# natir/yacrd

Measured on AMD Instinct MI355X. Metric: reads_per_sec_classified, higher is better.
Workload: dtype u32

## Files before the change

include/yacrd_engine_debug.h:

```cpp
#ifndef YACRD_ENGINE_DEBUG_H
#define YACRD_ENGINE_DEBUG_H

#include "yacrd_engine.h"

#define YACRD_F_FORCE_GENERAL 1u
#define YACRD_F_FORCE_LDS_SORT 2u
#define YACRD_F_WAVE_ONLY 8u
#define YACRD_F_NO_HALVES 16u
#define YACRD_F_NO_PREDICTION 64u
#define YACRD_F_NO_PREFILTER 256u
#define YACRD_F_COUNT_PREFILTERED 512u
#define YACRD_F_NO_DEFER 4096u
#define YACRD_F_ALWAYS_DEFER 8192u
#define YACRD_F_SCREEN_ITEMS_1 262144u
#define YACRD_F_SCREEN_ITEMS_2 524288u
#define YACRD_F_NO_FUSED_SCREEN 1048576u
#define YACRD_F_STREAM_SCREEN 65536u
#define YACRD_F_SCREEN_WIDE 2097152u

#ifdef __cplusplus
extern "C" {
#endif
int yacrd_debug_sort_pairs(yacrd_engine *e, uint64_t *keys, uint32_t *vals, uint64_t n, uint64_t key_bound);
uint64_t yacrd_debug_last_counters(const yacrd_engine *e, void *dst, uint64_t bytes);
int yacrd_debug_last_input_csr(yacrd_engine *e, uint64_t *n_reads, uint64_t *n_intervals, uint64_t *offsets, uint32_t *intervals,
                               uint32_t *lengths);
void yacrd_debug_peer_copy_counts(uint64_t out[3]);
void yacrd_debug_live_bytes(uint64_t out[2]);
#ifdef __cplusplus
}
#endif

#endif
```

yacrd_amd/__init__.py:

```python
from .engine import (
    Engine, EngineError, NeedsHostParser, Result, lib_path, load_library, build, partition_reads, run_partitioned, ingest_overlaps,
    NOT_BAD, CHIMERIC, NOT_COVERED, TYPE_NAMES, F_FORCE_GENERAL, F_FORCE_LDS_SORT, F_WAVE_ONLY, F_NO_HALVES, F_TIMING_FULL, F_NO_PREDICTION, F_NO_PREFILTER, F_COUNT_PREFILTERED, F_NO_TIMING, F_BLOCKING_WAIT, F_NO_DEFER, F_ALWAYS_DEFER, F_TIMING_SAMPLED, F_STREAM_SCREEN, F_SCREEN_ITEMS_1, F_SCREEN_ITEMS_2, F_NO_FUSED_SCREEN, F_SCREEN_WIDE, F_ONE_LAUNCH, run_device_batches, DeviceBatch,
    EXPORTED_SYMBOLS, CLASS_NAMES, CLASS_KERNELS, PinnedArray, Stream, StreamGroup, stream_device_of, HANDLE_ELSEWHERE, RecSink, OvlRec, OVL_REC_DTYPE, GzipWriter, ByteSink,
)
```

yacrd_amd/csrc/engine.hip:

```cpp
#include "engine_internal.h"

#include <time.h>

#include <algorithm>
#include <cstdio>
#include <cstdlib>
#include <cstring>
#include <string>
#include <thread>
#include <vector>

#include "device_common.h"
#include "plan_compact.h"
#include "sweep_big.h"
#include "sweep_wave.h"
#include "sweep_big_trim.h"
#include "sweep_general.h"
#include "sweep_lds.h"
#include "finish_compact.h"
#include "screen_wg.h"
#include "screen_stream.h"
#include "screen_big.h"
#include "one_batch.h"

// ... 85 lines not shown
            dl.shard_cap = (slabs / yk::kDeferShards + 1u) * (u32)yk::kMarkReads;
            HIP_TRY(e->dlist.reserve((size_t)yk::kDeferShards * dl.shard_cap * sizeof(u32)));
            dl.list = e->dlist.as<u32>();
            dl.count = reinterpret_cast<u32 *>(ca.scan_state + R.nb);
            if (e->compact_calls++)
                HIP_TRY(hipMemsetAsync(dl.count, 0, (size_t)yk::kDeferShards * yk::kDeferShardStride * sizeof(u32), e->stream));
            hipLaunchKernelGGL(yk::mark_list_kernel, dim3(slabs), dim3(yk::kMarkThreads), 0, e->stream, ca.sweep.counts, n_reads, dl);
            hipLaunchKernelGGL(yk::deferred_list_kernel, dim3((u32)e->num_cu * (u32)(YK_LIST_OCC * 256 / yk::kListThreads)), dim3(yk::kListThreads), 0,
                               e->stream, ca.sweep, dl);
        }
        hipLaunchKernelGGL(yk::scan_compact_kernel<4>, dim3((n_reads + 4 * yk::kScanThreads - 1) / (4 * yk::kScanThreads)), dim3(yk::kScanThreads), 0, e->stream, ca);
        return YACRD_OK;
    }
    hipLaunchKernelGGL(yk::finish_compact_kernel, dim3((n_reads + yk::kScanBlock - 1) / yk::kScanBlock), dim3(yk::kScanBlock), 0, e->stream, ca);
    return YACRD_OK;
}

int gather_reads(yacrd_engine *e, const u64 *d_off, const u32 *d_len, const u32 *d_list, u32 count,
                 hipStream_t stream, std::vector<yk::GatherOut> &out)
{
    HIP_TRY(e->gen_sizes.reserve((size_t)count * sizeof(yk::GatherOut)));
    hipLaunchKernelGGL(yk::gather_general_sizes_kernel, dim3((count + 255) / 256), dim3(256), 0,
                       stream, d_off, d_len, d_list, count, e->gen_sizes.as<yk::GatherOut>());
    out.resize(count);
    HIP_TRY(hipMemcpyAsync(out.data(), e->gen_sizes.p, (size_t)count * sizeof(yk::GatherOut),
                           hipMemcpyDeviceToHost, stream));
    HIP_TRY(hipStreamSynchronize(stream));
    for (const auto &g : out)
        if (g.n >= 0x7FFFFFFFull) return fail(YACRD_EINVAL, "a read has >= 2^31 - 1 intervals");
    return YACRD_OK;
}

int run_general_global(yacrd_engine *e, const u64 *d_off, const uint2 *d_iv, const u32 *d_len,
                       const u32 *d_list, u32 count, u32 cov, hipStream_t stream)
{
    std::vector<yk::GatherOut> info;
    int rc = gather_reads(e, d_off, d_len, d_list, count, stream, info);
    if (rc) return rc;
    HIP_TRY(e->gen_scratch_off.reserve((size_t)count * sizeof(u64)));
    std::vector<u64> offs(count);
    u64 tot = 0;
    for (u32 i = 0; i < count; i++) {
        offs[i] = tot;
        tot += 3 * info[i].n + 2;
    }
    HIP_TRY(e->gen_scratch.reserve((size_t)tot * sizeof(u64)));
    HIP_TRY(hipMemcpyAsync(e->gen_scratch_off.p, offs.data(), (size_t)count * sizeof(u64),
                           hipMemcpyHostToDevice, stream));
    HIP_TRY(hipStreamSynchronize(stream));
    yk::GeneralArgs ga;
    ga.off = d_off;
    ga.iv = d_iv;
    ga.len = d_len;
    ga.list = d_list;
    ga.scratch_off = e->gen_scratch_off.as<u64>();
    ga.scratch = e->gen_scratch.as<u64>();
    ga.cov = cov;
    ga.stage = e->stage.as<uint2>();
    ga.counts = e->counts.as<u32>();
    hipLaunchKernelGGL(yk::sweep_general_kernel, dim3(count), dim3(yk::kGenThreads), 0, stream, ga);
    return YACRD_OK;
}

int run_big_sort(yacrd_engine *e, const uint2 *d_iv, const std::vector<yk::GatherOut> &info, u32 cov,
                 hipStream_t stream, std::vector<u32> &redo)
{
    const u32 count = (u32)info.size();
    std::vector<yk::BigSeg> segs(count);
    std::vector<u32> chunk_seg;
    u64 key_off = 0;
    u32 max_P = 0;
    for (u32 i = 0; i < count; i++) {
        u64 P = yk::kBigC;
        while (P < 2 * info[i].n) P <<= 1;
        if (P > 0x80000000ull) return fail(YACRD_EINVAL, "a read has more than 2^30 intervals");
        yk::BigSeg &sg = segs[i];
        sg.key_off = key_off;
        sg.iv_off = info[i].iv_off;
        sg.P = (u32)P;
        sg.n = (u32)info[i].n;
        sg.len = info[i].len;
        sg.read = info[i].read;
        sg.chunk_off = (u32)chunk_seg.size();
        sg.pad = 0;
        for (u64 c = 0; c < P / yk::kBigC; c++) chunk_seg.push_back(i);
        key_off += P;
        max_P = std::max(max_P, (u32)P);
    }
    const size_t n_chunks = chunk_seg.size();
    if (n_chunks >= 0x7FFFFFFFull / (yk::kBigC / 2)) return fail(YACRD_EINVAL, "big path: too many keys");
    const size_t tab_bytes = (size_t)count * sizeof(yk::BigSeg) + n_chunks * sizeof(u32) +
                             9 * n_chunks * sizeof(u32) + (size_t)count * sizeof(u32) + 64;
    HIP_TRY(e->big_tab.reserve(tab_bytes));
    HIP_TRY(e->big_keys.reserve((size_t)key_off * sizeof(u32)));
    char *base = e->big_tab.as<char>();
    yk::BigArgs a;
    a.seg = reinterpret_cast<yk::BigSeg *>(base);
    u32 *w = reinterpret_cast<u32 *>(base + (size_t)count * sizeof(yk::BigSeg));
    a.chunk_seg = w;
    w += n_chunks;
    u32 **per_chunk[] = {&a.c_delta, &a.c_depth_in, &a.c_mf, &a.c_ml, &a.c_mf_in,
                         &a.c_ml_in, &a.c_cnt, &a.c_pos, &a.c_cand};
    for (u32 **pp : per_chunk) {
        *pp = w;
        w += n_chunks;
    }
    a.seg_bad = w;
    a.keys = e->big_keys.as<u32>();
    a.iv = d_iv;
    a.n_chunks = (u32)n_chunks;
    a.n_segs = count;
    a.cov = cov;
    a.stage = e->stage.as<uint2>();
    a.counts = e->counts.as<u32>();
    HIP_TRY(hipMemcpyAsync((void *)a.seg, segs.data(), (size_t)count * sizeof(yk::BigSeg),
                           hipMemcpyHostToDevice, stream));
    HIP_TRY(hipMemcpyAsync((void *)a.chunk_seg, chunk_seg.data(), n_chunks * sizeof(u32),
                           hipMemcpyHostToDevice, stream));
    HIP_TRY(hipMemsetAsync(a.seg_bad, 0, (size_t)count * sizeof(u32), stream));
    hipLaunchKernelGGL(yk::big_fill_kernel, dim3((u32)n_chunks), dim3(yk::kBigT), 0, stream, a);
    yk::launch_big(a, max_P, stream);
    std::vector<u32> bad(count);
    HIP_TRY(hipMemcpyAsync(bad.data(), a.seg_bad, (size_t)count * sizeof(u32), hipMemcpyDeviceToHost,
                           stream));
    HIP_TRY(hipStreamSynchronize(stream));
    HIP_TRY(hipGetLastError());
    for (u32 i = 0; i < count; i++)
        if (bad[i]) redo.push_back(info[i].read);
    return YACRD_OK;
}

int run_big(yacrd_engine *e, const u64 *d_off, const uint2 *d_iv, const u32 *d_len,
            const u32 *d_list, u32 count, u32 cov, hipStream_t stream)
{
    std::vector<yk::GatherOut> info;
    int rc = gather_reads(e, d_off, d_len, d_list, count, stream, info);
    if (rc) return rc;
    std::vector<u32> redo;

    if (!(e->flags & YACRD_F_NO_PREFILTER)) {
        std::vector<yk::BtSeg> bs(count);
        std::vector<u32> chunk_seg;
        for (u32 i = 0; i < count; i++) {
            yk::BtSeg &b = bs[i];
            b.iv_off = info[i].iv_off;
            b.n = (u32)info[i].n;
            b.len = info[i].len;
            b.read = info[i].read;
            b.chunk_off = (u32)chunk_seg.size();
            b.flags = 0;
            b.m_new = 0;
            b.n_zl = 0;
            b.pad = 0;
            for (u64 c = 0; c < (info[i].n + yk::kBtChunk - 1) / yk::kBtChunk; c++) chunk_seg.push_back(i);
        }
        const size_t n_chunks = chunk_seg.size();
        const size_t tab_words = (size_t)count * 3 * yk::kBtSeq;
        HIP_TRY(e->bt_tab.reserve((size_t)count * sizeof(yk::BtSeg) + n_chunks * sizeof(u32) + 64));
        HIP_TRY(e->bt_hist.reserve(tab_words * sizeof(u32)));
        HIP_TRY(e->bt_cur.reserve((2 * tab_words + (size_t)count * (3 * yk::kBtSeq / 32)) * sizeof(u32)));
        HIP_TRY(e->bt_keys.reserve((size_t)count * yk::kBtCap * sizeof(u32)));
        yk::BtArgs ba;
        ba.seg = e->bt_tab.as<yk::BtSeg>();
        ba.chunk_seg = reinterpret_cast<const u32 *>(e->bt_tab.as<char>() + (size_t)count * sizeof(yk::BtSeg));
        ba.iv = d_iv;
        ba.n_chunks = (u32)n_chunks;
        ba.n_segs = count;
        ba.cov = cov;
        ba.hist = e->bt_hist.as<u32>();
        ba.cur = e->bt_cur.as<u32>();
        ba.lim = e->bt_cur.as<u32>() + tab_words;
        ba.drop = e->bt_cur.as<u32>() + 2 * tab_words;
        ba.tkeys = e->bt_keys.as<u32>();
        ba.stage = e->stage.as<uint2>();
        ba.counts = e->counts.as<u32>();
        HIP_TRY(hipMemcpyAsync((void *)ba.seg, bs.data(), (size_t)count * sizeof(yk::BtSeg),
                               hipMemcpyHostToDevice, stream));
        HIP_TRY(hipMemcpyAsync((void *)ba.chunk_seg, chunk_seg.data(), n_chunks * sizeof(u32),
                               hipMemcpyHostToDevice, stream));
        HIP_TRY(hipMemsetAsync(ba.hist, 0, tab_words * sizeof(u32), stream));
        yk::Counters *ctr = e->ctrl2[e->ctrl_cur].as<yk::Counters>();
        u32 *rej = e->lists.as<u32>() + (size_t)(yk::CLS_COUNT + 2) * e->last_list_stride;
        hipLaunchKernelGGL(yk::bt_hist_kernel, dim3((u32)n_chunks), dim3(yk::kBtT), 0, stream, ba);
        hipLaunchKernelGGL(yk::bt_plan_kernel, dim3(count), dim3(yk::kBtT), 0, stream, ba);
        hipLaunchKernelGGL(yk::bt_scatter_kernel, dim3((u32)n_chunks), dim3(yk::kBtT), 0, stream, ba);
        hipLaunchKernelGGL(yk::bt_sweep_kernel, dim3(count), dim3(1024), 0, stream, ba, rej, &ctr->rej_big);
        HIP_TRY(hipMemcpyAsync(bs.data(), (void *)ba.seg, (size_t)count * sizeof(yk::BtSeg),
                               hipMemcpyDeviceToHost, stream));
        HIP_TRY(hipStreamSynchronize(stream));
        HIP_TRY(hipGetLastError());
        std::vector<yk::GatherOut> rest;
        for (u32 i = 0; i < count; i++) {
            if (bs[i].flags & yk::BT_TRIMMED) continue;
            if (bs[i].flags & yk::BT_BAD) redo.push_back(info[i].read);
            else rest.push_back(info[i]);
        }
        info.swap(rest);
        count = (u32)info.size();
    }
    if (count) {
        rc = run_big_sort(e, d_iv, info, cov, stream, redo);
        if (rc) return rc;
    }
    if (!redo.empty()) {
        HIP_TRY(e->big_redo.reserve(redo.size() * sizeof(u32)));
        HIP_TRY(hipMemcpyAsync(e->big_redo.p, redo.data(), redo.size() * sizeof(u32),
                               hipMemcpyHostToDevice, stream));
        HIP_TRY(hipStreamSynchronize(stream));
        rc = run_general_global(e, d_off, d_iv, d_len, e->big_redo.as<u32>(), (u32)redo.size(), cov, stream);
        if (rc) return rc;
    }
    return YACRD_OK;
}

int wait_for_stream(yacrd_engine *e)
{
    if (e->flags & YACRD_F_BLOCKING_WAIT) {
        HIP_TRY(hipEventRecord(e->ev_sync[EVS_DONE], e->stream));
        for (;;) {
            const hipError_t q = hipEventQuery(e->ev_sync[EVS_DONE]);
            if (q == hipSuccess) break;
            if (q != hipErrorNotReady) HIP_TRY(q);
            struct timespec ts = {0, 20000};
            nanosleep(&ts, nullptr);
        }
    } else {
        HIP_TRY(hipStreamSynchronize(e->stream));
    }
    HIP_TRY(hipGetLastError());
    return YACRD_OK;
}

int conclude_run(yacrd_engine *e, const Run &R, float extra_ms);
int finish_pending(yacrd_engine *e);


int reserve_buffers(yacrd_engine *e, Run &R)
{
    const u32 n_reads = R.n_reads;
    const uint64_t n_reads64 = R.n_reads64;
    R.ob_slabs = (n_reads + yk::kObSlab - 1) / yk::kObSlab;
    R.nb = R.one_launch ? 2 * R.ob_slabs : (n_reads + yk::kScanBlock - 1) / yk::kScanBlock;
    constexpr int kLists = yk::CLS_COUNT + 9;
    HIP_TRY(e->lists.reserve((size_t)kLists * n_reads * sizeof(u32)));
    const size_t shard_ctr_bytes = (!R.one_launch && n_reads64 >= split_min_reads()) ? (size_t)yk::kDeferShards * yk::kDeferShardStride * sizeof(u32) : 0;
    R.ctrl_bytes = (sizeof(yk::Counters) + (size_t)R.nb * sizeof(u64) + shard_ctr_bytes + 255) & ~(size_t)255;
    e->compact_calls = 0;
    e->ctrl_cur ^= 1;
    const int cur = e->ctrl_cur, other = cur ^ 1;
    for (int i = 0; i < 2; i++) {
        const void *before = e->ctrl2[i].p;
        HIP_TRY(e->ctrl2[i].reserve(R.ctrl_bytes));
        if (e->ctrl2[i].p != before) e->ctrl_clean[i] = 0;
    }
    HIP_TRY(e->stage.reserve((size_t)(R.n_iv + 2 * n_reads64) * sizeof(uint2)));
    HIP_TRY(e->counts.reserve((size_t)n_reads * sizeof(u32)));
    HIP_TRY(e->closed.reserve((size_t)n_reads * sizeof(uint2)));
    HIP_TRY(e->read_type.reserve((size_t)n_reads));
    if (e->bad_regions.cap < (size_t)(4 * n_reads64 + 1024) * sizeof(uint2))
        HIP_TRY(e->bad_regions.reserve((size_t)(4 * n_reads64 + 1024) * sizeof(uint2)));

    R.mrec_cap1 = (u32)std::min<u64>(n_reads64, R.n_iv / 513 + 1), R.mrec_cap2 = (u32)std::min<u64>(n_reads64, R.n_iv / 4097 + 1);
    HIP_TRY(e->mrec.reserve(((size_t)R.mrec_cap1 + R.mrec_cap2) * sizeof(uint4)));
    R.lists = e->lists.as<u32>();
    e->last_list_stride = n_reads;
    R.rej_small = R.list_of(yk::CLS_COUNT), R.rej_med = R.list_of(yk::CLS_COUNT + 1);
    R.rej_big = R.list_of(yk::CLS_COUNT + 2), R.over_med = R.list_of(yk::CLS_COUNT + 3);
    R.fb_med[0] = R.list_of(yk::CLS_COUNT + 4), R.fb_med[1] = R.list_of(yk::CLS_COUNT + 5);
    R.fb_big = R.list_of(yk::CLS_COUNT + 6);
    R.fb_stream[0] = R.list_of(yk::CLS_COUNT + 7), R.fb_stream[1] = R.list_of(yk::CLS_COUNT + 8);
    R.ctr = e->ctrl2[cur].as<yk::Counters>();
    R.base = base_sweep_args(e, R);

    if (e->ctrl_clean[cur] < R.ctrl_bytes) HIP_TRY(hipMemsetAsync(R.ctr, 0, R.ctrl_bytes, e->stream));
    e->ctrl_clean[cur] = 0;
    R.other_bytes = std::min<size_t>(e->ctrl2[other].cap, (size_t)1 << 30) & ~(size_t)3;
    return YACRD_OK;
}

int launch_one_batch(yacrd_engine *e, Run &R)
{
    const int other = e->ctrl_cur ^ 1;
    yk::OneBatchArgs oa;
    oa.c = compact_args(e, R);
    oa.slab_ctr = oa.c.scan_state + R.ob_slabs;
    oa.n_slabs = R.ob_slabs;
    oa.zero = e->ctrl2[other].as<u32>();
    oa.zero_words = (u32)(R.other_bytes / 4);
    e->h_ctr()->ob_unsupported = 0;
    e->h_ctr()->scan_ticket = 0;
    hipLaunchKernelGGL(yk::one_batch_kernel, dim3(((R.ob_slabs + 7) / 8) * 8 * (u32)(yk::kObSlab / yk::kObReads)), dim3(64), 0, e->stream, oa);
    e->ctrl_clean[other] = R.other_bytes;
    if (R.full) HIP_TRY(hipEventRecord(e->ev[EV_COMPACT], e->stream));
    return YACRD_OK;
}

int launch_plan(yacrd_engine *e, Run &R)
{
    const int other = e->ctrl_cur ^ 1;
    const u32 n_reads = R.n_reads;
    const u32 plan_mode = (u32)((e->flags & YACRD_F_FORCE_GENERAL) ? 1
                                : (e->flags & (YACRD_F_WAVE_ONLY | YACRD_F_FORCE_LDS_SORT)) ? 2
                                : (e->flags & YACRD_F_NO_HALVES) ? 3 : 0);
    if (n_reads < yk::kPlanSmallReads)
        hipLaunchKernelGGL((yk::plan_kernel<1, yk::kPlanSmallBlock>), dim3((n_reads + yk::kPlanSmallBlock - 1) / yk::kPlanSmallBlock),
                           dim3(yk::kPlanSmallBlock), 0, e->stream, R.d_off, n_reads, R.lists, R.ctr, plan_mode, e->ctrl2[other].as<u32>(), (u32)(R.other_bytes / 4), e->counts.as<u32>(), e->mrec.as<uint4>(), R.mrec_cap1, R.mrec_cap2);
    else
        hipLaunchKernelGGL(yk::plan_kernel<4>, dim3((n_reads + 4 * yk::kPlanBlock - 1) / (4 * yk::kPlanBlock)),
                           dim3(yk::kPlanBlock), 0, e->stream, R.d_off, n_reads, R.lists, R.ctr, plan_mode,
                           e->ctrl2[other].as<u32>(), (u32)(R.other_bytes / 4), e->counts.as<u32>(), e->mrec.as<uint4>(), R.mrec_cap1, R.mrec_cap2);
    e->ctrl_clean[other] = R.other_bytes;
    if (R.full) HIP_TRY(hipEventRecord(e->ev[EV_PLAN], e->stream));
    return YACRD_OK;
}

int size_launches(yacrd_engine *e, Run &R)
{
    const uint64_t n_reads64 = R.n_reads64;
    const bool big_predictable = !(e->flags & YACRD_F_NO_PREFILTER) && e->pred.fb_big == 0;
    R.predicted = e->pred_valid && e->pred_reads == n_reads64 && e->pred_iv == R.n_iv &&
                  (e->pred.n[yk::CLS_GENERAL] == 0 || big_predictable) &&
                  !(e->flags & (YACRD_F_FORCE_GENERAL | YACRD_F_NO_PREDICTION));
    LaunchSet &ls = R.ls;
    if (R.predicted) {
        for (int cls = 0; cls < yk::CLS_GENERAL; cls++) {
            const u64 p = e->pred.n[cls];
            const u64 cap = (cls <= yk::CLS_W16 && R.tight_grids) ? ((p + p / 8 + 64 + 15) & ~(u64)15)
                                                                 : n_reads64;
            ls.n[cls] = p ? (u32)std::min<u64>(cap, (n_reads64 + 15) & ~(u64)15) : 0;
            ls.hint[cls] = p ? (u32)std::min<u64>(p + p / 8 + 64, n_reads64) : 0;
            ls.iv[cls] = e->pred.iv[cls];
        }
        R.big_n = e->pred.n[yk::CLS_GENERAL], R.big_iv = e->pred.iv[yk::CLS_GENERAL];
    } else {
        HIP_TRY(hipMemcpyAsync(e->h_ctr(), R.ctr, sizeof(yk::Counters), hipMemcpyDeviceToHost, e->stream));
        HIP_TRY(hipStreamSynchronize(e->stream));
        R.c0 = *e->h_ctr();
        for (int cls = 0; cls < yk::CLS_GENERAL; cls++) {
            ls.n[cls] = R.c0.n[cls];
            ls.hint[cls] = R.c0.n[cls];
            ls.iv[cls] = R.c0.iv[cls];
        }
        R.big_n = R.c0.n[yk::CLS_GENERAL], R.big_iv = R.c0.iv[yk::CLS_GENERAL];
    }
    for (int cls = 0; cls < yk::CLS_GENERAL; cls++)
        if (ls.n[cls] && (R.dom_cls < 0 || ls.iv[cls] > ls.iv[R.dom_cls])) R.dom_cls = cls;
    return YACRD_OK;
}

hipError_t before_class(yacrd_engine *e, Run &R, int cls)
{
    if (!R.timing_on || !(R.full || cls == R.dom_cls)) return hipSuccess;
    if (R.n_cls_ev > 0 && R.full) {
        R.cls_b[cls] = R.n_cls_ev - 1;
        return hipSuccess;
    }
    R.cls_b[cls] = R.n_cls_ev;
    return hipEventRecord(e->ev_cls[R.n_cls_ev++], e->stream);
}
hipError_t mark_class(yacrd_engine *e, Run &R, int cls)
{
    if (!R.timing_on || !(R.full || cls == R.dom_cls)) return hipSuccess;
    R.cls_e[cls] = R.n_cls_ev;
    return hipEventRecord(e->ev_cls[R.n_cls_ev++], e->stream);
}

int launch_register_classes(yacrd_engine *e, Run &R, const LaunchSet &set, bool again)
{
    yk::Counters *ctr = R.ctr;
    const bool fuse = !(e->flags & YACRD_F_FORCE_LDS_SORT);
    if (fuse) {
        yk::FusedArgs fa;
        fa.base = R.base;
        const u64 fused_iv = set.iv[yk::CLS_R16] + set.iv[yk::CLS_H16];
        const bool defer = R.prefilter && !(e->flags & YACRD_F_NO_DEFER) &&
                           ((e->flags & YACRD_F_ALWAYS_DEFER) ||
                            (fused_iv >= defer_min_intervals() && e->nodefer_left == 0));
        const bool wide = defer && !(e->flags & YACRD_F_SCREEN_ITEMS_2) && ((e->flags & YACRD_F_SCREEN_WIDE) || e->wide_left > 0);
        const int items = !defer ? 1
                          : (wide || (e->flags & YACRD_F_SCREEN_ITEMS_1)) ? 1
                          : ((e->flags & YACRD_F_SCREEN_ITEMS_2) || fused_iv >= 40000000ull) ? 2 : 1;
        e->last_items = (uint32_t)items;
        e->last_wide = wide;
        if (!again) e->last_build = !defer ? 0 : wide ? 3 : items;
        fa.base.over_list = nullptr;
        fa.base.over_count = nullptr;
        fa.n_entries = 0;
        u32 blocks = 0;
        bool has_dom = false;
        for (int cls = yk::CLS_R2; cls <= yk::CLS_H16; cls++) {
            if (!set.n[cls]) continue;
            const u32 per = yk::sweep_group_reads_per_block(cls, defer ? yk::kDeferWaves : yk::kFusedWaves) *
                            (cls >= yk::CLS_R16 ? (u32)items : 1u);
            blocks += (set.n[cls] + per - 1) / per;
            fa.cls[fa.n_entries] = (u32)cls;
            fa.block_end[fa.n_entries] = blocks;
            fa.list[fa.n_entries] = R.list_of(cls);
            fa.list_n[fa.n_entries] = &ctr->n[cls];
            fa.first[fa.n_entries] = set.first[cls];
            fa.n_entries++;
            has_dom |= cls == R.dom_cls;
        }
        if (fa.n_entries) {
            const bool mark = R.timing_on && (R.full || has_dom);
            void (*kernel)(yk::FusedArgs) = yk::sweep_small_fused_kernel;
            u32 threads = 64 * yk::kFusedWaves;
            if (defer && items == 2) kernel = yk::sweep_small_fused_defer2_kernel, threads = 64;
            else if (defer && wide) kernel = yk::sweep_small_fused_defer_wide_kernel, threads = 64 * yk::kDeferWaves;
            else if (defer) kernel = yk::sweep_small_fused_defer_kernel, threads = 64 * yk::kDeferWaves;
            hipExtLaunchKernelGGL(kernel, dim3(blocks), dim3(threads), 0, e->stream, mark ? e->ev_cls[22] : (hipEvent_t) nullptr,
                                  mark ? e->ev_cls[23] : (hipEvent_t) nullptr, 0, fa);
            if (mark) R.fused_marked = true;
            if (defer && (set.n[yk::CLS_R16] || set.n[yk::CLS_H16])) R.screened = true;
        }
    }
    for (int cls = fuse ? yk::CLS_W2 : yk::CLS_R2; cls <= yk::CLS_W16; cls++) {
        if (!set.n[cls]) continue;
        HIP_TRY(before_class(e, R, cls));
        yk::SweepArgs sa = list_sweep_args(R, R.list_of(cls), &ctr->n[cls]);
        sa.first = set.first[cls];
        if (!fuse) {
            const u32 grid = (u32)std::min<uint64_t>(set.n[cls], (uint64_t)e->num_cu * 32);
            hipLaunchKernelGGL((yk::sweep_lds_kernel<64, (int)yk::kSmallEvents>), dim3(grid), dim3(64), 0, e->stream, sa);
        } else {
            switch (cls) {
            case yk::CLS_W2: yk::launch_sweep_group<64, 2>(sa, set.n[cls], e->stream); break;
            case yk::CLS_W4: yk::launch_sweep_group<64, 4>(sa, set.n[cls], e->stream); break;
            case yk::CLS_W8: yk::launch_sweep_group<64, 8>(sa, set.n[cls], e->stream); break;
            default: yk::launch_sweep_group<64, 16>(sa, set.n[cls], e->stream); break;
            }
        }
        HIP_TRY(mark_class(e, R, cls));
    }
    if (R.full && R.timing_on) HIP_TRY(hipEventRecord(e->ev[EV_SMALL], e->stream));
    return YACRD_OK;
}

int launch_workgroup_class_fused_screen(yacrd_engine *e, Run &R, const LaunchSet &set, int k, bool again)
{
    yk::Counters *ctr = R.ctr;
    const int cls = k == 0 ? yk::CLS_MED1 : yk::CLS_MED2;
    if (again) {
        HIP_TRY(hipMemsetAsync(&ctr->fb_stream[k], 0, sizeof(u32), e->stream));
        HIP_TRY(hipMemsetAsync(&ctr->fb_med[k], 0, sizeof(u32), e->stream));
    }
    {
        yk::SweepArgs ss = list_sweep_args(R, R.list_of(cls), &ctr->n[cls]);
        ss.over_list = R.fb_stream[k];
        ss.over_count = &ctr->fb_stream[k];
        const u32 want = std::max<u32>(set.hint[cls], 1u);
        if (e->flags & YACRD_F_STREAM_SCREEN) {
            hipLaunchKernelGGL(yk::screen_stream_kernel, dim3((u32)std::min<uint64_t>(want, (uint64_t)e->num_cu * 96)), dim3(64), 0, e->stream, ss);
        } else {
            ss.rec = e->mrec.as<uint4>() + (k == 0 ? 0u : R.mrec_cap1);
            hipLaunchKernelGGL(yk::screen_wg_kernel, dim3((u32)std::min<uint64_t>(want, (uint64_t)e->num_cu * 64)), dim3(yk::kWsT), 0, e->stream, ss);
        }
    }
    yk::ScreenFusedArgs fa;
    fa.sweep = list_sweep_args(R, R.fb_stream[k], &ctr->fb_stream[k]);
    fa.sweep.rej_list = k == 0 ? R.rej_med : R.rej_big;
    fa.sweep.rej_count = k == 0 ? &ctr->rej_med : &ctr->rej_big;
    fa.n_fallback = &ctr->fb_med[k];
    const u64 known = std::max<u32>(set.hint[cls], 1u);
    u64 share = 1;
    if (fused_share_override()) share = std::min<u64>(fused_share_override(), (u64)yk::kFusedShareMax);
    fa.share = (u32)share;
    const u32 gs = (u32)std::min<u64>(std::min<u64>((known + share - 1) / share, (u64)e->num_cu * 4) * fused_grid_mult(), 0x7FFFFFFFull);
    hipLaunchKernelGGL(yk::screen_wg_fused_kernel, dim3(gs), dim3(yk::kWsT), 0, e->stream, fa);
    if (k == 1) {
        yk::SweepArgs so = list_sweep_args(R, R.over_med, &ctr->over_med);
        so.rej_list = R.rej_big;
        so.rej_count = &ctr->rej_big;
        const u32 grid = (u32)std::min<uint64_t>(set.n[cls], (uint64_t)e->num_cu);
        hipLaunchKernelGGL((yk::sweep_lds_kernel<1024, (int)yk::kMedium2Events>), dim3(grid), dim3(1024), 0, e->stream, so);
    }
    return YACRD_OK;
}

int launch_workgroup_class_chain(yacrd_engine *e, Run &R, const LaunchSet &set, int k, bool again)
{
    yk::Counters *ctr = R.ctr;
    const int cls = k == 0 ? yk::CLS_MED1 : yk::CLS_MED2;
    const u32 *list = R.list_of(cls), *list_n = &ctr->n[cls];
    if (R.prefilter) {
        if (again) HIP_TRY(hipMemsetAsync(&ctr->fb_med[k], 0, sizeof(u32), e->stream));
        yk::SweepArgs ss = list_sweep_args(R, list, list_n);
        ss.over_list = R.fb_med[k];
        ss.over_count = &ctr->fb_med[k];
        const u32 gs = (u32)std::min<uint64_t>(set.n[cls], (uint64_t)e->num_cu * 4);
        hipLaunchKernelGGL(yk::screen_wg_kernel, dim3(gs), dim3(yk::kWsT), 0, e->stream, ss);
        list = R.fb_med[k], list_n = &ctr->fb_med[k];
    }
    yk::SweepArgs sa = list_sweep_args(R, list, list_n);
    sa.rej_list = k == 0 ? R.rej_med : R.rej_big;
    sa.rej_count = k == 0 ? &ctr->rej_med : &ctr->rej_big;
    if (k == 0) {
        const u32 grid = (u32)std::min<uint64_t>(set.n[cls], (uint64_t)e->num_cu * 4);
        hipLaunchKernelGGL((yk::sweep_lds_kernel<256, (int)yk::kMedium1Events>), dim3(grid), dim3(256), 0, e->stream, sa);
        return YACRD_OK;
    }
    yk::SweepArgs so = sa;
    if (R.prefilter) {
        const u32 g256 = (u32)std::min<uint64_t>(set.n[cls], (uint64_t)e->num_cu * 5);
        hipLaunchKernelGGL((yk::sweep_lds_kernel<256, (int)yk::kMedium1Events>), dim3(g256), dim3(256), 0, e->stream, sa);
        so.list = R.over_med;
        so.list_n = &ctr->over_med;
    }
    const u32 grid = (u32)std::min<uint64_t>(set.n[cls], (uint64_t)e->num_cu);
    hipLaunchKernelGGL((yk::sweep_lds_kernel<1024, (int)yk::kMedium2Events>), dim3(grid), dim3(1024), 0, e->stream, so);
    return YACRD_OK;
}

int launch_workgroup_classes(yacrd_engine *e, Run &R, const LaunchSet &set, bool again)
{
    const bool fused_screen = R.prefilter && !(e->flags & YACRD_F_NO_FUSED_SCREEN) && !e->fused_off && e->screen_fused_wgs_per_cu > 0;
    for (int k = 0; k < 2; k++) {
        const int cls = k == 0 ? yk::CLS_MED1 : yk::CLS_MED2;
        if (!set.n[cls]) continue;
        HIP_TRY(before_class(e, R, cls));
        const int rc = fused_screen ? launch_workgroup_class_fused_screen(e, R, set, k, again)
                                    : launch_workgroup_class_chain(e, R, set, k, again);
        if (rc) return rc;
        HIP_TRY(mark_class(e, R, cls));
    }
    if (R.full && R.timing_on) HIP_TRY(hipEventRecord(e->ev[EV_MED], e->stream));
    return YACRD_OK;
}

void launch_rejected_medium(yacrd_engine *e, Run &R, const LaunchSet &set)
{
    if (!set.n[yk::CLS_MED1]) return;
    yk::SweepArgs sa = list_sweep_args(R, R.rej_med, &R.ctr->rej_med);
    sa.rej_list = R.rej_big;
    sa.rej_count = &R.ctr->rej_big;
    hipLaunchKernelGGL((yk::sweep_general_lds_kernel<1024, 4096>), dim3(e->num_cu), dim3(1024), 0, e->stream, sa);
}

int launch_sweeps(yacrd_engine *e, Run &R, const LaunchSet &set, bool again = false)
{
    int rc = launch_register_classes(e, R, set, again);
    if (!rc) rc = launch_workgroup_classes(e, R, set, again);
    if (!rc) launch_rejected_medium(e, R, set);
    return rc;
}

int launch_device_wide_screen_on(yacrd_engine *e, Run &R, u32 count, u64 iv_big, hipStream_t hs)
{
    yk::Counters *ctr = R.ctr;
    if (e->flags & YACRD_F_FORCE_GENERAL)
        return run_general_global(e, R.d_off, R.d_iv, R.d_len, R.list_of(yk::CLS_GENERAL), count, R.cov, e->stream);
    if (!R.prefilter)
        return run_big(e, R.d_off, R.d_iv, R.d_len, R.list_of(yk::CLS_GENERAL), count, R.cov, e->stream);
    const u64 max_chunks = iv_big / yk::kBsChunk + count;
    if (max_chunks >= 0x7FFFFFFFull) return fail(YACRD_EINVAL, "too many intervals in reads beyond 16384");
    HIP_TRY(e->bs_seg.reserve((size_t)count * sizeof(yk::BsSeg)));
    HIP_TRY(e->bs_chunk.reserve((size_t)max_chunks * sizeof(u32)));
    HIP_TRY(e->bs_hist.reserve((size_t)count * 2 * yk::kBsBins * sizeof(u32)));
    yk::BsArgs ba;
    ba.off = R.d_off, ba.iv = R.d_iv, ba.len = R.d_len;
    ba.list = R.list_of(yk::CLS_GENERAL);
    ba.list_n = &ctr->n[yk::CLS_GENERAL];
    ba.seg = e->bs_seg.as<yk::BsSeg>();
    ba.chunk_seg = e->bs_chunk.as<u32>();
    ba.n_chunks = &ctr->bs_chunks;
    ba.hist = e->bs_hist.as<u32>();
    ba.max_chunks = (u32)max_chunks, ba.max_segs = count;
    ba.cov = R.cov, ba.count_healthy = R.prefilter == 2 ? 1u : 0u;
    ba.stage = R.base.stage, ba.counts = R.base.counts;
    ba.fb_list = R.fb_big, ba.fb_count = &ctr->fb_big;
    ba.ctr = ctr;
    if (R.big_screened) HIP_TRY(hipMemsetAsync(&ctr->fb_big, 0, sizeof(u32), hs));
    HIP_TRY(hipMemsetAsync(ba.hist, 0, (size_t)count * 2 * yk::kBsBins * sizeof(u32), hs));
    hipLaunchKernelGGL(yk::bs_setup_kernel, dim3(1), dim3(1024), 0, hs, ba);
    hipLaunchKernelGGL(yk::bs_minmax_kernel, dim3((u32)max_chunks), dim3(yk::kBsT), 0, hs, ba);
    hipLaunchKernelGGL(yk::bs_hist_kernel, dim3((u32)max_chunks), dim3(yk::kBsT), 0, hs, ba);
    hipLaunchKernelGGL(yk::bs_verdict_kernel, dim3(count), dim3(yk::kBsVT), 0, hs, ba);
    R.big_screened = true;
    return YACRD_OK;
}
int launch_device_wide_screen(yacrd_engine *e, Run &R)
{
    const bool can_fork = R.big_n != 0 && R.prefilter && !(e->flags & YACRD_F_FORCE_GENERAL);
    if (can_fork && e->side == nullptr) {
        if (e->streams.add(1)) e->side = e->streams[1];
        else (void)hipGetLastError();
    }
    R.big_beside = can_fork && e->side != nullptr;
    if (!R.big_beside) return YACRD_OK;
    HIP_TRY(hipEventRecord(e->ev_sync[EVS_FORK], e->stream));
    HIP_TRY(hipStreamWaitEvent(e->side, e->ev_sync[EVS_FORK], 0));
    const int rc = launch_device_wide_screen_on(e, R, R.big_n, R.big_iv, e->side);
    if (rc) return rc;
    HIP_TRY(hipEventRecord(e->ev_sync[EVS_JOIN], e->side));
    return YACRD_OK;
}
int join_device_wide_screen(yacrd_engine *e, Run &R)
{
    if (R.big_beside) HIP_TRY(hipStreamWaitEvent(e->stream, e->ev_sync[EVS_JOIN], 0));
    else if (R.big_n) return launch_device_wide_screen_on(e, R, R.big_n, R.big_iv, e->stream);
    return YACRD_OK;
}

void launch_rejected_small(yacrd_engine *e, Run &R)
{
    yk::SweepArgs sa = list_sweep_args(R, R.rej_small, &R.ctr->rej_small);
    sa.rej_list = R.rej_med;
    sa.rej_count = &R.ctr->rej_med;
    hipLaunchKernelGGL((yk::sweep_general_lds_kernel<256, 512>), dim3(e->num_cu * 2), dim3(256), 0, e->stream, sa);
}

int recover(yacrd_engine *e, Run &R, float &extra_ms)
{
    yk::Counters *ctr = R.ctr;
    int rc = YACRD_OK;
    bool redo = false;
    if (R.predicted) {
        R.c0 = *e->h_ctr();
        const yk::Counters &c0 = R.c0;
        LaunchSet missing{};
        bool any_missing = false;
        for (int cls = 0; cls < yk::CLS_GENERAL; cls++)
            if (c0.n[cls] > R.ls.n[cls]) {
                missing.first[cls] = (cls <= yk::CLS_W16 && R.tight_grids) ? R.ls.n[cls] : 0;
                missing.n[cls] = c0.n[cls] - missing.first[cls];
                missing.hint[cls] = missing.n[cls];
                any_missing = true;
            }
        const bool big_mismatch = c0.n[yk::CLS_GENERAL] != R.big_n || c0.iv[yk::CLS_GENERAL] != R.big_iv;
        if (any_missing || big_mismatch) {
            e->miss_pending = true;
            HIP_TRY(hipEventRecord(e->ev[EV_X0], e->stream));
            if (any_missing && (rc = launch_sweeps(e, R, missing, true))) return rc;
            if (big_mismatch && c0.n[yk::CLS_GENERAL] &&
                (rc = launch_device_wide_screen_on(e, R, c0.n[yk::CLS_GENERAL], c0.iv[yk::CLS_GENERAL], e->stream))) return rc;
            HIP_TRY(hipMemcpyAsync(e->h_ctr(), ctr, sizeof(yk::Counters), hipMemcpyDeviceToHost, e->stream));
            HIP_TRY(hipStreamSynchronize(e->stream));
            redo = true;
        }
    }
    u32 rej_small_done = 0;
    if (e->h_ctr()->rej_small) {
        if (!redo) HIP_TRY(hipEventRecord(e->ev[EV_X0], e->stream));
        launch_rejected_small(e, R);
        rej_small_done = e->h_ctr()->rej_small;
        redo = true;
    }
    if (R.big_screened && e->h_ctr()->fb_big) {
        if (!redo) HIP_TRY(hipEventRecord(e->ev[EV_X0], e->stream));
        rc = run_big(e, R.d_off, R.d_iv, R.d_len, R.fb_big, e->h_ctr()->fb_big, R.cov, e->stream);
        if (rc) return rc;
        HIP_TRY(hipMemcpyAsync(e->h_ctr(), ctr, sizeof(yk::Counters), hipMemcpyDeviceToHost, e->stream));
        HIP_TRY(hipStreamSynchronize(e->stream));
        redo = true;
    }
    const u32 n_rej_big = e->h_ctr()->rej_big;
    if (n_rej_big) {
        if (!redo) HIP_TRY(hipEventRecord(e->ev[EV_X0], e->stream));
        rc = run_general_global(e, R.d_off, R.d_iv, R.d_len, R.rej_big, n_rej_big, R.cov, e->stream);
        if (rc) return rc;
        redo = true;
    }
    for (int attempt = 0; attempt < 4; attempt++) {
        if (!redo && e->h_ctr()->rej_small > rej_small_done) {
            HIP_TRY(hipEventRecord(e->ev[EV_X0], e->stream));
            launch_rejected_small(e, R);
            rej_small_done = e->h_ctr()->rej_small;
            redo = true;
        }
        if (!redo) {
            if (!e->h_ctr()->region_overflow) break;
            HIP_TRY(e->bad_regions.reserve((size_t)(e->h_ctr()->total_regions + 16) * sizeof(uint2)));
            HIP_TRY(hipEventRecord(e->ev[EV_X0], e->stream));
        }
        redo = false;
        HIP_TRY(hipMemsetAsync(&ctr->region_overflow, 0, 3 * sizeof(u32), e->stream));
        HIP_TRY(hipMemsetAsync(ctr + 1, 0, (size_t)R.nb * sizeof(u64), e->stream));
        rc = launch_compact(e, R);
        if (rc) return rc;
        HIP_TRY(hipEventRecord(e->ev[EV_X1], e->stream));
        HIP_TRY(hipStreamSynchronize(e->stream));
        HIP_TRY(hipGetLastError());
        extra_ms += ev_ms(e->ev[EV_X0], e->ev[EV_X1]);
    }
    if (e->h_ctr()->region_overflow) return fail(YACRD_EINTERNAL, "bad_regions overflow persisted");
    if (e->h_ctr()->rej_small > rej_small_done) return fail(YACRD_EINTERNAL, "rejected reads persisted");
    return YACRD_OK;
}

}

namespace yke {
static int rerun_without_fused(yacrd_engine *e, const Run R)
{
    e->fused_off = true;
    e->pred_valid = false;
    const int rc = run_on_device(e, R.d_off, R.d_iv, R.d_len, R.n_reads64, R.n_iv, R.cov, R.not_cov, false);
    e->fused_off = false;
    return rc;
}

static int hand_over(yacrd_engine *e, const Run &R, bool defer)
{
    e->pending = Pending{true, R.one_launch, R};
    return defer ? YACRD_OK : finish_pending(e);
}

int run_on_device(yacrd_engine *e, const u64 *d_off, const uint2 *d_iv, const u32 *d_len,
                  uint64_t n_reads64, uint64_t n_iv, uint32_t cov, double not_cov, bool defer)
{
    if (n_reads64 >= 0xFFFFFFFFull) return fail(YACRD_EINVAL, "n_reads must be < 2^32 - 1");
    if (e->pending.active) return fail(YACRD_EINVAL, "a submitted batch is pending: yacrd_engine_wait first");
    e->has_result = false;
    e->resident.valid = e->input.valid = false;
    e->timing = yacrd_timing{};

    HIP_TRY(e->bad_offsets.reserve((n_reads64 + 1) * sizeof(u64)));
    if (n_reads64 == 0) {
        HIP_TRY(hipMemsetAsync(e->bad_offsets.p, 0, sizeof(u64), e->stream));
        HIP_TRY(hipStreamSynchronize(e->stream));
        e->last_reads = 0;
        e->last_regions = 0;
        e->has_result = true;
        return YACRD_OK;
    }

    Run R;
    R.d_off = d_off, R.d_iv = d_iv, R.d_len = d_len;
    R.n_reads64 = n_reads64, R.n_reads = (u32)n_reads64, R.n_iv = n_iv, R.cov = cov, R.not_cov = not_cov;
    R.full = (e->flags & YACRD_F_TIMING_FULL) != 0;
    R.tight_grids = !(e->flags & YACRD_F_FORCE_LDS_SORT);
    R.prefilter = (e->flags & YACRD_F_NO_PREFILTER) ? 0u : (e->flags & YACRD_F_COUNT_PREFILTERED) ? 2u : 1u;
    for (int i = 0; i < 12; i++) R.cls_b[i] = R.cls_e[i] = -1;
    const uint64_t ob_waiters = (n_reads64 + yk::kObSlab - 1) / yk::kObSlab * 7 / 8;
    R.one_launch = (e->flags & YACRD_F_ONE_LAUNCH) && !e->one_launch_off && n_reads64 < (uint64_t)yk::kObMaxReads &&
                   e->num_xcc == 8 && 2 * ob_waiters <= (uint64_t)e->num_cu * 4 * YK_OB_OCC &&
                   !(e->flags & (YACRD_F_FORCE_GENERAL | YACRD_F_WAVE_ONLY | YACRD_F_FORCE_LDS_SORT | YACRD_F_NO_HALVES |
                                 YACRD_F_NO_PREFILTER | YACRD_F_NO_DEFER));

    int rc = reserve_buffers(e, R);
    if (rc) return rc;
    if (R.full) HIP_TRY(hipEventRecord(e->ev[EV_START], e->stream));
    if (R.one_launch) {
        rc = launch_one_batch(e, R);
        return rc ? rc : hand_over(e, R, defer);
    }
    rc = launch_plan(e, R);
    if (!rc) rc = size_launches(e, R);
    if (rc) return rc;
    R.timing_on = !(e->flags & YACRD_F_NO_TIMING);
    if ((e->flags & YACRD_F_TIMING_SAMPLED) && !R.full && (e->run_seq++ % 8u) != 0) R.timing_on = false;
    struct MissGuard {
        yacrd_engine *e;
        bool before;
        ~MissGuard() { e->miss_pending = before; }
    } miss_guard{e, e->miss_pending};
    struct SideGuard {
        yacrd_engine *e;
        const Run &R;
        bool joined = false;
        ~SideGuard()
        {
            if (R.big_beside && !joined) (void)hipStreamSynchronize(e->side);
        }
    } side_guard{e, R};
    e->prev_build = e->last_build;
    e->last_build = -1;
    if (R.full) HIP_TRY(hipEventRecord(e->ev[EV_S0], e->stream));
    rc = launch_device_wide_screen(e, R);
    if (!rc) rc = launch_sweeps(e, R, R.ls);
    if (!rc) rc = join_device_wide_screen(e, R);
    if (rc) return rc;
    side_guard.joined = true;
    if (R.full) HIP_TRY(hipEventRecord(e->ev[EV_GEN], e->stream));
    rc = launch_compact(e, R);
    if (rc) return rc;
    if (R.full) HIP_TRY(hipEventRecord(e->ev[EV_COMPACT], e->stream));
    if (defer && R.predicted) return hand_over(e, R, defer);
    rc = wait_for_stream(e);
    if (rc) return rc;
    R.timing_on = false;
    if (e->h_ctr()->fused_gave_up && !e->fused_off) return rerun_without_fused(e, R);
    float extra_ms = 0.f;
    rc = recover(e, R, extra_ms);
    if (rc) return rc;
    return conclude_run(e, R, extra_ms);
}
}

namespace {

void fold_timing(yacrd_engine *e)
{
    const yacrd_timing &t = e->timing;
    yacrd_timing &ts = e->timing_sum;
    const yacrd_timing keep = ts;
    ts = t;
    ts.h2d_ms = keep.h2d_ms;
    ts.d2h_ms = keep.d2h_ms;
    ts.plan_ms = keep.plan_ms + t.plan_ms;
    ts.sweep_small_ms = keep.sweep_small_ms + t.sweep_small_ms;
    ts.sweep_medium_ms = keep.sweep_medium_ms + t.sweep_medium_ms;
    ts.sweep_general_ms = keep.sweep_general_ms + t.sweep_general_ms;
    ts.compact_ms = keep.compact_ms + t.compact_ms;
    ts.total_ms = keep.total_ms + t.total_ms;
    for (int i = 0; i < 12; i++) ts.class_ms[i] = keep.class_ms[i] + t.class_ms[i];
    ts.fused_ms = keep.fused_ms + t.fused_ms;
    ts.screened = keep.screened + t.screened;
    ts.one_launch = keep.one_launch + t.one_launch;
    ts.fused_reruns = keep.fused_reruns + t.fused_reruns;
    ts.screen_wide = keep.screen_wide + t.screen_wide;
    ts.predicted = keep.predicted + t.predicted;
    ts.prediction_misses = keep.prediction_misses + t.prediction_misses;
    ts.build_switches = keep.build_switches + t.build_switches;
    ts.sorting_build = keep.sorting_build + t.sorting_build;
    ts.timed_runs = keep.timed_runs + t.timed_runs;
    e->timing_runs++;
}

int conclude_run(yacrd_engine *e, const Run &R, float extra_ms)
{
    const bool full = R.full, predicted = R.predicted, screened = R.screened;
    const yk::Counters c1 = *e->h_ctr();
    const yk::Counters c0 = predicted ? c1 : R.c0;
    e->last_reads = R.n_reads;
    e->last_regions = c1.total_regions;
    e->has_result = true;
    e->pred = c1;
    e->pred_reads = R.n_reads64;
    e->pred_iv = R.n_iv;
    e->pred_valid = true;

    yacrd_timing &t = e->timing;
    t.plan_ms = t.sweep_small_ms = t.sweep_medium_ms = t.sweep_general_ms = t.compact_ms = 0.f;
    t.total_ms = 0.f;
    if (full) {
        t.plan_ms = ev_ms(e->ev[EV_START], e->ev[EV_PLAN]);
        t.sweep_small_ms = ev_ms(e->ev[EV_S0], e->ev[EV_SMALL]);
        t.sweep_medium_ms = ev_ms(e->ev[EV_SMALL], e->ev[EV_MED]);
        t.sweep_general_ms = ev_ms(e->ev[EV_MED], e->ev[EV_GEN]);
        t.compact_ms = ev_ms(e->ev[EV_GEN], e->ev[EV_COMPACT]);
        t.total_ms = (predicted ? ev_ms(e->ev[EV_START], e->ev[EV_COMPACT])
                                : t.plan_ms + ev_ms(e->ev[EV_S0], e->ev[EV_COMPACT])) + extra_ms;
    }
    t.n_small = 0;
    t.iv_small = 0;
    for (int cls = yk::CLS_R2; cls <= yk::CLS_W16; cls++) {
        t.n_small += c0.n[cls];
        t.iv_small += c0.iv[cls];
    }
    t.n_medium = (uint64_t)c0.n[yk::CLS_MED1] + c0.n[yk::CLS_MED2];
    t.n_general = (uint64_t)c0.n[yk::CLS_GENERAL] + c1.rej_small + c1.rej_med + c1.rej_big;
    t.iv_medium = c0.iv[yk::CLS_MED1] + c0.iv[yk::CLS_MED2];
    t.iv_general = c0.iv[yk::CLS_GENERAL];
    static_assert(yk::CLS_GENERAL == 11, "yacrd_timing.class_* follows the CLS_ order");
    for (int cls = 0; cls <= yk::CLS_GENERAL; cls++) {
        t.class_reads[cls] = c0.n[cls];
        t.class_intervals[cls] = c0.iv[cls];
        t.class_ms[cls] = 0.f;
        if (cls < yk::CLS_GENERAL && R.cls_b[cls] >= 0 && R.cls_e[cls] >= 0)
            t.class_ms[cls] = ev_ms(e->ev_cls[R.cls_b[cls]], e->ev_cls[R.cls_e[cls]]);
    }
    t.class_ms[yk::CLS_GENERAL] = (full && c0.n[yk::CLS_GENERAL]) ? t.sweep_general_ms : 0.f;
    t.fused_ms = 0.f;
    t.timed_runs = R.fused_marked ? 1u : 0u;
    for (int cls = 0; cls < yk::CLS_GENERAL; cls++)
        if (R.cls_b[cls] >= 0 && R.cls_e[cls] >= 0) t.timed_runs = 1u;
    t.deferred_reads = c1.deferred;
    t.deferred_intervals = c1.deferred_iv;
    if (screened) {
        const uint64_t looked_at = (uint64_t)c0.n[yk::CLS_R16] + c0.n[yk::CLS_H16];
        const bool can_widen = !e->last_wide && !(e->flags & YACRD_F_SCREEN_ITEMS_2);
        e->nodefer_left = (!(e->flags & YACRD_F_ALWAYS_DEFER) && !can_widen && 4 * (uint64_t)c1.deferred > looked_at) ? kProbeEvery - 1 : 0;
        if (!e->last_wide) e->wide_left = 10 * (uint64_t)c1.deferred > looked_at ? kProbeEvery - 1 : 0;
        else if (e->wide_left) e->wide_left--;
    } else if (e->nodefer_left) {
        e->nodefer_left--;
    }
    t.screened = screened ? 1u : 0u;
    t.screen_items = screened ? e->last_items : 0u;
    t.screen_wide = (screened && e->last_wide) ? 1u : 0u;
    t.fused_reruns = e->fused_off ? 1u : 0u;
    t.predicted = predicted ? 1u : 0u;
    t.prediction_misses = e->miss_pending ? 1u : 0u;
    t.build_switches = (e->last_build >= 0 && e->prev_build >= 0 && e->last_build != e->prev_build) ? 1u : 0u;
    t.sorting_build = e->last_build == 0 ? 1u : 0u;
    t.fused_reads = t.fused_intervals = 0;
    t.prefiltered_reads = c1.prefiltered;
    if (R.fused_marked) t.fused_ms = ev_ms(e->ev_cls[22], e->ev_cls[23]);
    if (!(e->flags & YACRD_F_FORCE_LDS_SORT)) {
        for (int cls = yk::CLS_R2; cls <= yk::CLS_H16; cls++) {
            t.fused_reads += c0.n[cls];
            t.fused_intervals += c0.iv[cls];
        }
    }

    fold_timing(e);
    return YACRD_OK;
}

int finish_pending(yacrd_engine *e)
{
    Pending &p = e->pending;
    if (!p.active) return YACRD_OK;
    p.active = false;
    const Run R = p.run;
    int rc = wait_for_stream(e);
    if (rc) return rc;
    if (p.one_launch) {
        const yk::Counters c1 = *e->h_ctr();
        if (c1.ob_unsupported || c1.rej_small || c1.region_overflow || c1.scan_ticket != R.ob_slabs) {
            if (c1.region_overflow) HIP_TRY(e->bad_regions.reserve((size_t)(c1.total_regions + 16) * sizeof(uint2)));
            e->one_launch_off = true;
            rc = run_on_device(e, R.d_off, R.d_iv, R.d_len, R.n_reads64, R.n_iv, R.cov, R.not_cov);
            e->one_launch_off = false;
            return rc;
        }
        e->last_reads = R.n_reads64;
        e->last_regions = c1.total_regions;
        e->has_result = true;
        yacrd_timing &t = e->timing;
        t = yacrd_timing{};
        if (R.full) t.total_ms = ev_ms(e->ev[EV_START], e->ev[EV_COMPACT]);
        t.n_small = R.n_reads64, t.iv_small = R.n_iv;
        t.deferred_reads = c1.deferred, t.deferred_intervals = c1.deferred_iv, t.prefiltered_reads = c1.prefiltered;
        t.screened = 1u, t.screen_items = (uint32_t)yk::kObItems, t.one_launch = 1u;
        fold_timing(e);
        return YACRD_OK;
    }
    const yk::Counters c = *e->h_ctr();
    if (c.fused_gave_up && !e->fused_off) return yke::rerun_without_fused(e, R);
    bool ok = !c.rej_small && c.n[yk::CLS_GENERAL] == R.big_n && c.iv[yk::CLS_GENERAL] == R.big_iv && !c.fb_big && !c.rej_big && !c.region_overflow;
    for (int cls = 0; cls < yk::CLS_GENERAL; cls++) ok = ok && c.n[cls] <= R.ls.n[cls];
    if (!ok) {
        e->pred_valid = false;
        e->miss_pending = true;
        const int rcm = run_on_device(e, R.d_off, R.d_iv, R.d_len, R.n_reads64, R.n_iv, R.cov, R.not_cov);
        e->miss_pending = false;
        return rcm;
    }
    return conclude_run(e, R, 0.f);
}

}

namespace yke {
int h2d(yacrd_engine *e, void *dst, const void *src, size_t bytes)
{
    if (!bytes) return YACRD_OK;
    hipPointerAttribute_t at;
    const bool pinned = hipPointerGetAttributes(&at, src) == hipSuccess && at.type == hipMemoryTypeHost;
    if (!pinned) (void)hipGetLastError();
    if (pinned || bytes < ((size_t)1 << 20)) {
        HIP_TRY(hipMemcpyAsync(dst, src, bytes, hipMemcpyHostToDevice, e->stream));
        return YACRD_OK;
    }
    constexpr size_t kPiece = yacrd_engine::kBounceBytes;
    for (size_t b = e->bounce_ev.v.size(); b < (size_t)yacrd_engine::kBounce; b++) {
        HIP_TRY(e->bounce[b].reserve(kPiece));
        if (!e->bounce_ev.add(1, hipEventDisableTiming)) {
            e->bounce[b].release();
            HIP_TRY(why_not_added());
        }
    }
    const size_t n_pieces = (bytes + kPiece - 1) / kPiece;
    const int T = (int)std::min<size_t>(yacrd_engine::kBounce / 2, n_pieces);
    std::vector<hipError_t> errs((size_t)T, hipSuccess);
    auto work = [&](int t) {
        if (hipSetDevice(e->device) != hipSuccess) {
            errs[t] = hipErrorInvalidDevice;
            return;
        }
        int turn = 0;
        for (size_t piece = (size_t)t; piece < n_pieces; piece += (size_t)T, turn ^= 1) {
            const int b = 2 * t + turn;
            if (e->bounce_busy[b]) {
                const hipError_t w = hipEventSynchronize(e->bounce_ev[b]);
                if (w != hipSuccess) errs[t] = w;
            }
            const size_t at2 = piece * kPiece, n = std::min(kPiece, bytes - at2);
            std::memcpy(e->bounce[b].p, (const char *)src + at2, n);
            hipError_t c = hipMemcpyAsync((char *)dst + at2, e->bounce[b].p, n, hipMemcpyHostToDevice, e->stream);
            if (c == hipSuccess) c = hipEventRecord(e->bounce_ev[b], e->stream);
            if (c != hipSuccess) errs[t] = c;
            e->bounce_busy[b] = true;
        }
    };
    {
        std::vector<std::thread> th;
        for (int t = 1; t < T; t++) th.emplace_back(work, t);
        work(0);
        for (auto &x : th) x.join();
    }
    for (hipError_t er : errs) HIP_TRY(er);
    return YACRD_OK;
}

int classify_on_device(yacrd_engine *e, const u64 *d_bad_offsets, const uint2 *d_bad_regions, const u32 *d_len, u32 n_reads, double not_cov,
                       uint8_t *d_read_type)
{
    if (n_reads)
        hipLaunchKernelGGL(yk::classify_csr_kernel, dim3((n_reads + 255u) / 256u), dim3(256), 0, e->stream, d_bad_offsets, d_bad_regions, d_len,
                           n_reads, not_cov, d_read_type);
    HIP_TRY(hipGetLastError());
    return YACRD_OK;
}

int fetch_result(yacrd_engine *e, yacrd_result *out)
{
    if (!out) return fail(YACRD_EINVAL, "out is null");
    std::memset(out, 0, sizeof(*out));
    if (e->pending.active) return fail(YACRD_EINVAL, "a submitted batch is pending: yacrd_engine_wait first");
    if (!e->has_result) return fail(YACRD_EINVAL, "no result to fetch");
    const uint64_t R = e->last_reads, G = e->last_regions;
    out->bad_offsets = (uint64_t *)std::malloc((size_t)(R + 1) * sizeof(uint64_t));
    out->bad_regions = (uint32_t *)std::malloc((size_t)(2 * G + 2) * sizeof(uint32_t));
    out->read_type = (uint8_t *)std::malloc((size_t)R + 1);
    if (!out->bad_offsets || !out->bad_regions || !out->read_type) {
        yacrd_result_free(out);
        return fail(YACRD_ENOMEM, "host allocation failed");
    }
    const size_t b_off = (size_t)(R + 1) * sizeof(uint64_t), b_reg = (size_t)G * sizeof(uint2), b_typ = (size_t)R;
    const size_t o_reg = (b_off + 63) & ~(size_t)63, o_typ = (o_reg + b_reg + 63) & ~(size_t)63;
    const size_t need = o_typ + b_typ + 64;
    bool staged = need <= ((size_t)1 << 30);
    if (staged && need > e->h_out.cap && e->h_out.reserve(need + need / 4) != hipSuccess) {
        (void)hipGetLastError();
        staged = false;
    }
    char *h = e->h_out.as<char>();
    void *t_off = staged ? (void *)h : (void *)out->bad_offsets;
    void *t_reg = staged ? (void *)(h + o_reg) : (void *)out->bad_regions;
    void *t_typ = staged ? (void *)(h + o_typ) : (void *)out->read_type;
    HIP_TRY(hipEventRecord(e->ev[EV_D2H0], e->stream));
    HIP_TRY(hipMemcpyAsync(t_off, e->bad_offsets.p, b_off, hipMemcpyDeviceToHost, e->stream));
    if (G) HIP_TRY(hipMemcpyAsync(t_reg, e->bad_regions.p, b_reg, hipMemcpyDeviceToHost, e->stream));
    if (R) HIP_TRY(hipMemcpyAsync(t_typ, e->read_type.p, b_typ, hipMemcpyDeviceToHost, e->stream));
    HIP_TRY(hipEventRecord(e->ev[EV_D2H1], e->stream));
    HIP_TRY(hipStreamSynchronize(e->stream));
    if (staged) {
        std::memcpy(out->bad_offsets, t_off, b_off);
        if (G) std::memcpy(out->bad_regions, t_reg, b_reg);
        if (R) std::memcpy(out->read_type, t_typ, b_typ);
    }
    e->timing.d2h_ms = ev_ms(e->ev[EV_D2H0], e->ev[EV_D2H1]);
    out->n_reads = R;
    out->n_regions = G;
    return YACRD_OK;
}
}

extern "C" {

int yacrd_abi_version(void) { return YACRD_ABI_VERSION; }

uint64_t yacrd_debug_last_counters(const yacrd_engine *e, void *dst, uint64_t bytes)
{
    if (e && dst && e->h_ctr()) std::memcpy(dst, e->h_ctr(), (size_t)std::min<uint64_t>(bytes, sizeof(yk::Counters)));
    return sizeof(yk::Counters);
}

int yacrd_debug_last_input_csr(yacrd_engine *e, uint64_t *n_reads, uint64_t *n_intervals, uint64_t *offsets, uint32_t *intervals,
                               uint32_t *lengths)
{
    if (!e || !n_reads || !n_intervals) return fail(YACRD_EINVAL, "null argument");
    if (e->pending.active || e->host_pending) return fail(YACRD_EINVAL, "the engine has a submitted batch pending");
    if (!e->input.valid) return fail(YACRD_EINVAL, "the engine's last call left no input CSR of its own");
    const uint64_t R = e->input.n_reads, I = e->input.n_iv;
    if (offsets && ((I && !intervals) || (R && !lengths))) return fail(YACRD_EINVAL, "null argument");
    if ((R && ((R + 1) * sizeof(u64) > e->in_off.cap || R * sizeof(u32) > e->in_len.cap)) || (I && I * sizeof(uint2) > e->in_iv.cap))
        return fail(YACRD_EINTERNAL, "the input CSR's record does not fit the engine's input buffers");
    *n_reads = R, *n_intervals = I;
    if (!offsets) return YACRD_OK;
    DeviceGuard guard(e->device);
    offsets[0] = 0;
    if (R) HIP_TRY(hipMemcpyAsync(offsets, e->in_off.p, (size_t)(R + 1) * sizeof(u64), hipMemcpyDeviceToHost, e->stream));
    if (I) HIP_TRY(hipMemcpyAsync(intervals, e->in_iv.p, (size_t)I * sizeof(uint2), hipMemcpyDeviceToHost, e->stream));
    if (R) HIP_TRY(hipMemcpyAsync(lengths, e->in_len.p, (size_t)R * sizeof(u32), hipMemcpyDeviceToHost, e->stream));
    HIP_TRY(hipStreamSynchronize(e->stream));
    return YACRD_OK;
}

void yacrd_debug_live_bytes(uint64_t out[2])
{
    out[0] = yke::live_bytes()[0].load();
    out[1] = yke::live_bytes()[1].load();
}

const char *yacrd_last_error(void) { return yke::err_slot().c_str(); }

int yacrd_engine_create(const yacrd_engine_cfg *cfg, yacrd_engine **out)
{
    if (!out) return fail(YACRD_EINVAL, "out is null");
    *out = nullptr;
    int count = 0;
    if (hipGetDeviceCount(&count) != hipSuccess || count == 0)
        return fail(YACRD_ENODEV, "no HIP device visible (libyacrd_hip needs an MI355X / gfx950)");
    int dev = cfg ? cfg->device_id : -1;
    if (dev < 0) HIP_TRY(hipGetDevice(&dev));
    if (dev >= count) return fail(YACRD_EINVAL, "device_id out of range");
    hipDeviceProp_t prop;
    HIP_TRY(hipGetDeviceProperties(&prop, dev));
    if (std::strncmp(prop.gcnArchName, "gfx950", 6) != 0)
        return fail(YACRD_ENODEV, std::string("device is ") + prop.gcnArchName +
                                      ", this library is built for gfx950 only");
    DeviceGuard guard(dev);
    yacrd_engine *e = new (std::nothrow) yacrd_engine();
    if (!e) return fail(YACRD_ENOMEM, "host allocation failed");
    e->device = dev;
    e->flags = cfg ? cfg->flags : 0;
    e->num_cu = prop.multiProcessorCount > 0 ? prop.multiProcessorCount : 256;
    {
        int xcc = 0;
        if (hipDeviceGetAttribute(&xcc, hipDeviceAttributeNumberOfXccs, dev) != hipSuccess) xcc = 0;
        (void)hipGetLastError();
        e->num_xcc = xcc;
    }
    {
        int per_cu = 0;
        if (hipOccupancyMaxActiveBlocksPerMultiprocessor(&per_cu, yk::screen_wg_fused_kernel, yk::kWsT, 0) == hipSuccess && per_cu > 0)
            e->screen_fused_wgs_per_cu = std::min(per_cu, 4);
        (void)hipGetLastError();
    }
    const bool made = e->streams.add(1) && e->ev.add(EV_COUNT) && e->ev_cls.add(24) &&
                      e->ev_sync.add(1, hipEventBlockingSync | hipEventDisableTiming) && e->ev_sync.add(2, hipEventDisableTiming);
    if (!made || e->h_ctr_mem.reserve(sizeof(yk::Counters)) != hipSuccess) {
        yacrd_engine_destroy(e);
        return fail(YACRD_ENODEV, std::string("engine setup: ") + hipGetErrorString(why_not_added()));
    }
    e->stream = e->streams[0];
    *out = e;
    return YACRD_OK;
}

int yacrd_engine_trim(yacrd_engine *e)
{
    if (!e) return fail(YACRD_EINVAL, "engine is null");
    if (e->pending.active || e->host_pending) return fail(YACRD_EINVAL, "the engine has a submitted batch pending");
    DeviceGuard guard(e->device);
    e->mirror.valid = false;
    e->resident.valid = e->input.valid = false;
    for (int k = 0; k < yacrd_engine::kSlots; k++)
        if (!(k == yacrd_engine::kGzip && e->gzip_busy)) e->drop_scratch(k);
    return YACRD_OK;
}

void yacrd_engine_destroy(yacrd_engine *e)
{
    if (!e) return;
    DeviceGuard guard(e->device);
    if (e->stream) (void)hipStreamSynchronize(e->stream);
    if (e->side) (void)hipStreamSynchronize(e->side);
    for (int k = 0; k < yacrd_engine::kSlots; k++) e->drop_scratch(k);
    delete e;
}

static void fill_device_result(const yacrd_engine *e, yacrd_device_result *out)
{
    if (!out) return;
    out->n_reads = e->last_reads;
    out->n_regions = e->last_regions;
    out->d_bad_offsets = e->bad_offsets.p;
    out->d_bad_regions = e->bad_regions.p;
    out->d_read_type = e->read_type.p;
}

int yacrd_engine_run_device(yacrd_engine *e, const void *d_offsets, const void *d_intervals,
                            const void *d_lengths, uint64_t n_reads, uint64_t n_intervals,
                            uint32_t coverage, double not_coverage, yacrd_device_result *out)
{
    if (!e) return fail(YACRD_EINVAL, "engine is null");
    e->resident.valid = e->input.valid = false;
    if (n_reads && (!d_offsets || !d_lengths)) return fail(YACRD_EINVAL, "null device input");
    if (n_intervals && !d_intervals) return fail(YACRD_EINVAL, "null device intervals");
    if (e->host_pending) return fail(YACRD_EINVAL, "a submitted batch is pending: collect it first");
    DeviceGuard guard(e->device);
    int rc = run_on_device(e, (const u64 *)d_offsets, (const uint2 *)d_intervals,
                           (const u32 *)d_lengths, n_reads, n_intervals, coverage, not_coverage);
    if (rc) return rc;
    fill_device_result(e, out);
    return YACRD_OK;
}

int yacrd_engine_submit_device(yacrd_engine *e, const void *d_offsets, const void *d_intervals,
                               const void *d_lengths, uint64_t n_reads, uint64_t n_intervals,
                               uint32_t coverage, double not_coverage)
{
    if (!e) return fail(YACRD_EINVAL, "engine is null");
    e->resident.valid = e->input.valid = false;
    if (n_reads && (!d_offsets || !d_lengths)) return fail(YACRD_EINVAL, "null device input");
    if (n_intervals && !d_intervals) return fail(YACRD_EINVAL, "null device intervals");
    if (e->host_pending) return fail(YACRD_EINVAL, "a submitted batch is pending: collect it first");
    DeviceGuard guard(e->device);
    return run_on_device(e, (const u64 *)d_offsets, (const uint2 *)d_intervals,
                         (const u32 *)d_lengths, n_reads, n_intervals, coverage, not_coverage, true);
}

int yacrd_engine_wait(yacrd_engine *e, yacrd_device_result *out)
{
    if (!e) return fail(YACRD_EINVAL, "engine is null");
    DeviceGuard guard(e->device);
    int rc = finish_pending(e);
    if (rc) return rc;
    if (!e->has_result) return fail(YACRD_EINVAL, "nothing was submitted");
    fill_device_result(e, out);
    return YACRD_OK;
}

int yacrd_engines_run_device_batches(yacrd_engine *const *engines, uint32_t n_engines,
                                     const yacrd_device_batch *batches, uint32_t n_batches,
                                     yacrd_batch_done_fn done, void *user, yacrd_device_result *last)
{
    if (!engines || n_engines == 0 || (!batches && n_batches)) return fail(YACRD_EINVAL, "bad argument");
    for (uint32_t j = 0; j < n_engines; j++)
        if (!engines[j]) return fail(YACRD_EINVAL, "engine is null");
    for (uint32_t j = 0; j < n_engines; j++) engines[j]->resident.valid = engines[j]->input.valid = false;
    std::vector<int64_t> inflight(n_engines, -1);
    yacrd_device_result res{};
    auto finish = [&](uint32_t j) -> int {
        int rc = yacrd_engine_wait(engines[j], &res);
        if (rc) return rc;
        const uint32_t b = (uint32_t)inflight[j];
        inflight[j] = -1;
        if (done && done(user, b, engines[j], &res)) return fail(YACRD_EINVAL, "the batch callback asked to stop");
        return YACRD_OK;
    };
    int rc = YACRD_OK;
    for (uint32_t i = 0; i < n_batches && rc == YACRD_OK; i++) {
        const uint32_t j = i % n_engines;
        if (inflight[j] >= 0) rc = finish(j);
        if (rc) break;
        const yacrd_device_batch &b = batches[i];
        rc = yacrd_engine_submit_device(engines[j], b.d_offsets, b.d_intervals, b.d_lengths, b.n_reads,
                                        b.n_intervals, b.coverage, b.not_coverage);
        if (rc == YACRD_OK) inflight[j] = i;
    }
    for (uint32_t k = 0; k < n_engines; k++) {
        uint32_t j = 0;
        int64_t lo = -1;
        for (uint32_t q = 0; q < n_engines; q++)
            if (inflight[q] >= 0 && (lo < 0 || inflight[q] < lo)) lo = inflight[q], j = q;
        if (lo < 0) break;
        const int rc2 = finish(j);
        if (rc == YACRD_OK) rc = rc2;
        inflight[j] = -1;
    }
    if (rc == YACRD_OK && last) *last = res;
    return rc;
}

static int stage_host_inputs(yacrd_engine *e, const uint64_t *offsets, const uint32_t *intervals,
                             const uint32_t *lengths, uint64_t n_reads, uint64_t *n_iv_out)
{
    if (n_reads && (!offsets || !lengths)) return fail(YACRD_EINVAL, "null input");
    const uint64_t n_iv = n_reads ? offsets[n_reads] : 0;
    if (n_reads && offsets[0] != 0) return fail(YACRD_EINVAL, "offsets[0] must be 0");
    for (uint64_t r = 0; r < n_reads; r++)
        if (offsets[r + 1] < offsets[r]) return fail(YACRD_EINVAL, "offsets must be non-decreasing");
    if (n_iv && !intervals) return fail(YACRD_EINVAL, "null intervals");
    HIP_TRY(e->in_off.reserve((size_t)(n_reads + 1) * sizeof(uint64_t)));
    HIP_TRY(e->in_iv.reserve((size_t)(n_iv + 1) * sizeof(uint2)));
    HIP_TRY(e->in_len.reserve((size_t)(n_reads + 1) * sizeof(uint32_t)));
    HIP_TRY(hipEventRecord(e->ev[EV_H2D0], e->stream));
    int rc = YACRD_OK;
    if (n_reads) {
        rc = h2d(e, e->in_off.p, offsets, (size_t)(n_reads + 1) * sizeof(uint64_t));
        if (!rc) rc = h2d(e, e->in_len.p, lengths, (size_t)n_reads * sizeof(uint32_t));
    }
    if (!rc && n_iv) rc = h2d(e, e->in_iv.p, intervals, (size_t)n_iv * sizeof(uint2));
    if (rc) return rc;
    HIP_TRY(hipEventRecord(e->ev[EV_H2D1], e->stream));
    *n_iv_out = n_iv;
    return YACRD_OK;
}

static int bring_home(yacrd_engine *e, yacrd_result *out)
{
    e->timing.h2d_ms = ev_ms(e->ev[EV_H2D0], e->ev[EV_H2D1]);
    e->timing_sum.h2d_ms += e->timing.h2d_ms;
    const int rc = fetch_result(e, out);
    if (rc) return rc;
    e->timing_sum.d2h_ms += e->timing.d2h_ms;
    e->input.valid = true;
    return YACRD_OK;
}

int yacrd_engine_run(yacrd_engine *e, const uint64_t *offsets, const uint32_t *intervals,
                     const uint32_t *lengths, uint64_t n_reads, uint32_t coverage,
                     double not_coverage, yacrd_result *out)
{
    if (!e) return fail(YACRD_EINVAL, "engine is null");
    e->resident.valid = e->input.valid = false;
    if (!out) return fail(YACRD_EINVAL, "out is null");
    std::memset(out, 0, sizeof(*out));
    if (e->pending.active) return fail(YACRD_EINVAL, "a submitted batch is pending: yacrd_engine_wait first");
    if (e->host_pending) return fail(YACRD_EINVAL, "a submitted batch is pending: collect it first");
    DeviceGuard guard(e->device);
    uint64_t n_iv = 0;
    int rc = stage_host_inputs(e, offsets, intervals, lengths, n_reads, &n_iv);
    if (rc) return rc;
    rc = run_on_device(e, e->in_off.as<u64>(), e->in_iv.as<uint2>(), e->in_len.as<u32>(), n_reads,
                       n_iv, coverage, not_coverage);
    if (rc) return rc;
    e->input.n_reads = n_reads, e->input.n_iv = n_iv;
    return bring_home(e, out);
}

int yacrd_engine_submit(yacrd_engine *e, const uint64_t *offsets, const uint32_t *intervals,
                        const uint32_t *lengths, uint64_t n_reads, uint32_t coverage,
                        double not_coverage)
{
    if (!e) return fail(YACRD_EINVAL, "engine is null");
    e->resident.valid = e->input.valid = false;
    if (e->pending.active || e->host_pending)
        return fail(YACRD_EINVAL, "a submitted batch is pending: collect it first");
    DeviceGuard guard(e->device);
    uint64_t n_iv = 0;
    int rc = stage_host_inputs(e, offsets, intervals, lengths, n_reads, &n_iv);
    if (rc) return rc;
    rc = run_on_device(e, e->in_off.as<u64>(), e->in_iv.as<uint2>(), e->in_len.as<u32>(), n_reads,
                       n_iv, coverage, not_coverage, true);
    if (rc) return rc;
    e->input.n_reads = n_reads, e->input.n_iv = n_iv;
    e->host_pending = true;
    return YACRD_OK;
}

int yacrd_engine_collect(yacrd_engine *e, yacrd_result *out)
{
    if (!e) return fail(YACRD_EINVAL, "engine is null");
    if (!out) return fail(YACRD_EINVAL, "out is null");
    std::memset(out, 0, sizeof(*out));
    if (!e->host_pending) return fail(YACRD_EINVAL, "nothing was submitted");
    e->host_pending = false;
    DeviceGuard guard(e->device);
    int rc = finish_pending(e);
    return rc ? rc : bring_home(e, out);
}

void *yacrd_pinned_alloc(size_t bytes)
{
    void *p = nullptr;
    if (hipHostMalloc(&p, bytes ? bytes : 1) != hipSuccess) {
        (void)hipGetLastError();
        yke::err_slot() = "hipHostMalloc failed";
        return nullptr;
    }
    return p;
}

void yacrd_pinned_free(void *p)
{
    if (p) (void)hipHostFree(p);
}

int yacrd_engine_fetch(yacrd_engine *e, yacrd_result *out)
{
    if (!e) return fail(YACRD_EINVAL, "engine is null");
    DeviceGuard guard(e->device);
    return fetch_result(e, out);
}

void yacrd_result_free(yacrd_result *r)
{
    if (!r) return;
    std::free(r->bad_offsets);
    std::free(r->bad_regions);
    std::free(r->read_type);
    std::memset(r, 0, sizeof(*r));
}

int yacrd_engine_last_timing(const yacrd_engine *e, yacrd_timing *t)
{
    if (!e || !t) return fail(YACRD_EINVAL, "null argument");
    *t = e->timing;
    return YACRD_OK;
}

int yacrd_engine_timing_total(yacrd_engine *e, yacrd_timing *sum, uint64_t *n_runs, int reset)
{
    if (!e) return fail(YACRD_EINVAL, "null argument");
    if (sum) *sum = e->timing_sum;
    if (n_runs) *n_runs = e->timing_runs;
    if (reset) {
// ... 149 lines not shown
```

yacrd_amd/csrc/engine_internal.h:

```cpp
#pragma once
#include "../../include/yacrd_engine_debug.h"

#include <hip/hip_runtime.h>
#include <hip/hip_ext.h>

#include <atomic>
#include <chrono>
#include <new>
#include <string>
#include <vector>

#include "bgzf_sizes.h"
#include "device_common.h"

namespace yif {
struct InfMember;
}

namespace yke {

std::string &err_slot();
inline int fail(int code, const std::string &msg)
{
    err_slot() = msg;
    return code;
}

#define HIP_TRY(expr)                                                                          \
    do {                                                                                       \
        hipError_t _e = (expr);                                                                \
        if (_e != hipSuccess)                                                                  \
            return yke::fail(_e == hipErrorOutOfMemory ? YACRD_ENOMEM : YACRD_ENODEV,          \
                             std::string(#expr) + ": " + hipGetErrorString(_e));              \
    } while (0)

inline std::atomic<uint64_t> *live_bytes()
{
    static std::atomic<uint64_t> held[2];
    return held;
}

template <class Mem>
struct OwnedBuf {
    void *p = nullptr;
    size_t cap = 0;
    OwnedBuf() = default;
    OwnedBuf(const OwnedBuf &) = delete;
    OwnedBuf &operator=(const OwnedBuf &) = delete;
    OwnedBuf(OwnedBuf &&o) noexcept : p(o.p), cap(o.cap) { o.p = nullptr, o.cap = 0; }
    OwnedBuf &operator=(OwnedBuf &&o) noexcept
    {
        if (this != &o) {
            release();
            p = o.p, cap = o.cap;
            o.p = nullptr, o.cap = 0;
        }
        return *this;
    }
    ~OwnedBuf() { release(); }
    hipError_t reserve_exact(size_t bytes)
    {
        if (bytes <= cap) return hipSuccess;
        release();
        const hipError_t e = Mem::alloc(&p, bytes);
        if (e == hipSuccess) live_bytes()[Mem::kCounter] += (cap = bytes);
        else p = nullptr;
        return e;
    }
    void release()
    {
        if (!p) return;
        (void)Mem::free(p);
        live_bytes()[Mem::kCounter] -= cap;
        p = nullptr;
        cap = 0;
    }
    template <class T>
    T *as() const
    {
        return reinterpret_cast<T *>(p);
    }
};
struct DevMem {
    static constexpr int kCounter = 0;
    static hipError_t alloc(void **p, size_t n) { return hipMalloc(p, n); }
    static hipError_t free(void *p) { return hipFree(p); }
};
struct PinMem {
    static constexpr int kCounter = 1;
    static hipError_t alloc(void **p, size_t n) { return hipHostMalloc(p, n); }
    static hipError_t free(void *p) { return hipHostFree(p); }
};

struct DevBuf : OwnedBuf<DevMem> {
    hipError_t reserve(size_t bytes)
    {
        if (bytes <= cap) return hipSuccess;
        return reserve_exact(bytes + bytes / 8 + 256) == hipSuccess ? hipSuccess : reserve_exact(bytes);
    }
};

struct PinBuf : OwnedBuf<PinMem> {
    hipError_t reserve(size_t bytes) { return reserve_exact(bytes); }
};

struct Events {
    std::vector<hipEvent_t> v;
    Events() = default;
    Events(const Events &) = delete;
    Events &operator=(const Events &) = delete;
    bool add(size_t n, unsigned flags = hipEventDefault)
    {
        for (; n; n--) {
            hipEvent_t x = nullptr;
            if (hipEventCreateWithFlags(&x, flags) != hipSuccess) return false;
            v.push_back(x);
        }
        return true;
    }
    hipEvent_t operator[](size_t i) const { return v[i]; }
    ~Events()
    {
        for (hipEvent_t x : v) (void)hipEventDestroy(x);
    }
};
struct Streams {
    std::vector<hipStream_t> v;
    Streams() = default;
    Streams(const Streams &) = delete;
    Streams &operator=(const Streams &) = delete;
    bool add(size_t n)
    {
        for (; n; n--) {
            hipStream_t x = nullptr;
            if (hipStreamCreateWithFlags(&x, hipStreamNonBlocking) != hipSuccess) return false;
            v.push_back(x);
        }
        return true;
    }
    hipStream_t operator[](size_t i) const { return v[i]; }
    void clear()
    {
        for (hipStream_t x : v) (void)hipStreamDestroy(x);
        v.clear();
    }
    ~Streams() { clear(); }
};

inline hipError_t why_not_added()
{
    const hipError_t e = hipGetLastError();
    return e != hipSuccess ? e : hipErrorUnknown;
}

enum { EV_START = 0, EV_PLAN, EV_S0, EV_SMALL, EV_MED, EV_GEN, EV_COMPACT, EV_X0, EV_X1, EV_H2D0, EV_H2D1, EV_D2H0, EV_D2H1, EV_COUNT };
enum { EVS_DONE = 0, EVS_FORK, EVS_JOIN, EVS_COUNT };

struct DeviceGuard {
    int prev = -1;
    explicit DeviceGuard(int dev)
    {
        if (hipGetDevice(&prev) != hipSuccess) prev = -1;
        if (prev != dev) (void)hipSetDevice(dev);
        else prev = -1;
    }
    ~DeviceGuard()
    {
        if (prev >= 0) (void)hipSetDevice(prev);
    }
};

inline double now_ms()
{
    return std::chrono::duration<double, std::milli>(std::chrono::steady_clock::now().time_since_epoch()).count();
}

inline float ev_ms(hipEvent_t a, hipEvent_t b)
{
    float ms = 0.f;
    if (hipEventElapsedTime(&ms, a, b) != hipSuccess) return 0.f;
    return ms;
}

}



struct LaunchSet {
    u32 n[12];
    u32 hint[12];
    u32 first[12];
    u64 iv[12];
};

struct Run {
    const u64 *d_off = nullptr;
    const uint2 *d_iv = nullptr;
    const u32 *d_len = nullptr;
    uint64_t n_reads64 = 0, n_iv = 0;
    u32 n_reads = 0;
    uint32_t cov = 0;
    double not_cov = 0;
    bool full = false;
    bool tight_grids = false;
    u32 prefilter = 0;
    bool one_launch = false;
    yk::Counters *ctr = nullptr;
    u32 nb = 0, ob_slabs = 0;
    size_t ctrl_bytes = 0, other_bytes = 0;
    u32 *lists = nullptr;
    u32 *rej_small = nullptr, *rej_med = nullptr, *rej_big = nullptr;
    u32 *over_med = nullptr;
    u32 *fb_med[2] = {}, *fb_big = nullptr, *fb_stream[2] = {};
    u32 *list_of(int cls) const { return lists + (size_t)cls * n_reads; }
    u32 mrec_cap1 = 0, mrec_cap2 = 0;
    yk::SweepArgs base{};
    bool predicted = false;
    yk::Counters c0{};
    LaunchSet ls{};
    u32 big_n = 0;
    u64 big_iv = 0;
    bool big_beside = false;
    int cls_b[12], cls_e[12];
    int n_cls_ev = 0, dom_cls = -1;
    bool timing_on = false;
    bool fused_marked = false, screened = false, big_screened = false;
};

struct Pending {
    bool active = false;
    bool one_launch = false;
    Run run;
};

struct yacrd_engine {
    Pending pending;
    int device = 0;
    uint32_t flags = 0;
    yke::Streams streams;
    hipStream_t stream = nullptr;
    hipStream_t side = nullptr;
    yke::Events ev;
    yke::Events ev_cls;
    yke::Events ev_sync;
    int num_cu = 256;
    bool fused_off = false;
    int num_xcc = 0;
    int screen_fused_wgs_per_cu = 0;

    yke::DevBuf in_off, in_iv, in_len;
    yke::DevBuf dlist;
    uint32_t compact_calls = 0;
    yke::DevBuf mrec;
    yke::DevBuf lists, ctrl2[2], stage, counts, closed, gen_sizes, gen_scratch_off, gen_scratch, big_tab, big_keys, big_redo, bt_tab, bt_hist, bt_cur, bt_keys, bs_seg, bs_chunk, bs_hist;
    size_t ctrl_clean[2] = {0, 0};
    int ctrl_cur = 0;
    yke::DevBuf bad_offsets, bad_regions, read_type;
    yke::PinBuf h_ctr_mem;
    yk::Counters *h_ctr() const { return h_ctr_mem.as<yk::Counters>(); }

    uint64_t last_reads = 0, last_regions = 0;
    size_t last_list_stride = 0;
    bool has_result = false;
    yk::Counters pred{};
    uint64_t pred_reads = 0, pred_iv = 0;
    bool pred_valid = false;
    yacrd_timing timing = {};
    yacrd_timing timing_sum = {};
    uint64_t timing_runs = 0;
    uint32_t run_seq = 0;
    uint32_t wide_left = 0;
    uint32_t last_items = 1;
    bool last_wide = false;
    bool one_launch_off = false;
    int last_build = -1, prev_build = -1;
    bool miss_pending = false;
    uint32_t nodefer_left = 0;
    static constexpr int kBounce = 12;
    static constexpr size_t kBounceBytes = (size_t)4 << 20;
    yke::Events bounce_ev;
    yke::PinBuf bounce[kBounce];
    bool bounce_busy[kBounce] = {};
    yke::PinBuf h_out;
    bool host_pending = false;
    yke::PinBuf paf_arena;
    struct {
        const unsigned char *p = nullptr;
        uint64_t n = 0, dev = 0, ino = 0;
        int64_t mtime_s = 0, mtime_ns = 0;
        bool valid = false;
    } mirror;
    struct {
        const unsigned char *names = nullptr;
        const u64 *name_off = nullptr;
        const u32 *lengths = nullptr;
        uint64_t n_reads = 0;
        bool valid = false;
    } resident;
    struct {
        uint64_t n_reads = 0, n_iv = 0;
        bool valid = false;
    } input;
    enum Slot { kPaf = 0, kEdit, kGzip, kReport, kReportWrite, kSeqEdit, kInflate, kSlots };
    struct {
        void *p = nullptr;
        void (*destroy)(void *) = nullptr;
    } scratch[kSlots];
    void drop_scratch(int k)
    {
        if (scratch[k].p) scratch[k].destroy(scratch[k].p);
        scratch[k].p = nullptr;
    }
    bool gzip_busy = false;
};


namespace yke {
template <class T>
T *scratch_of(yacrd_engine *e)
{
    auto &s = e->scratch[T::kScratchSlot];
    if (!s.p && (s.p = new (std::nothrow) T())) s.destroy = [](void *p) { delete static_cast<T *>(p); };
    return static_cast<T *>(s.p);
}
int run_on_device(yacrd_engine *e, const u64 *d_off, const uint2 *d_iv, const u32 *d_len,
                  uint64_t n_reads64, uint64_t n_iv, uint32_t cov, double not_cov, bool defer = false);
int classify_on_device(yacrd_engine *e, const u64 *d_bad_offsets, const uint2 *d_bad_regions, const u32 *d_len, u32 n_reads, double not_cov,
                       uint8_t *d_read_type);
int fetch_result(yacrd_engine *e, yacrd_result *out);
struct RecSlab {
    const yk::OvlRec *recs;
    uint64_t n;
};
int csr_from_records(yacrd_engine *e, const RecSlab *slabs, size_t n_slabs, const u32 *d_map, u64 n_handles, u64 n_reads,
                     DevBuf &cnt, DevBuf &part, DevBuf &err, hipEvent_t done, u64 *n_intervals = nullptr,
                     bool counted = false, u64 iv_bound = 0);
int scan_u32_to_u64(yacrd_engine *e, const u32 *in, u64 n, u64 *out, DevBuf &part, hipStream_t st = nullptr );
int h2d(yacrd_engine *e, void *dst, const void *src, size_t bytes);
struct GzDevice {
    const unsigned char *out[2] = {nullptr, nullptr};
    u64 max_blocks = 0;
};
int gzip_device_open(yacrd_engine *e, u64 max_blocks, GzDevice *g);
int gzip_device_encode(yacrd_engine *e, const GzDevice &g, hipStream_t st, const unsigned char *d_text, u64 n, bool last, int which,
                       hipEvent_t k0, hipEvent_t k1, volatile u64 *h_bytes, volatile u64 *h_stored);
void gzip_device_close(yacrd_engine *e);
struct InflateDevice {
    unsigned char *comp = nullptr;
    const yif::InfMember *members = nullptr;
    u32 *status = nullptr;
    u64 comp_bytes = 0, n_members = 0;
    bool fresh = false;
};
int inflate_device_open(yacrd_engine *e, u64 comp_bytes, const yif::InfMember *members, u64 n_members, InflateDevice *d);
int inflate_device_run(yacrd_engine *e, const InflateDevice &d, hipStream_t st, unsigned char *d_text, u64 text_bytes);
int inflate_not_taken(u32 status);
}
```

yacrd_amd/csrc/plan_compact.h:

```cpp
#pragma once
#include "device_common.h"

namespace yk {

constexpr int kPlanBlock = 1024;
constexpr u32 kPlanSmallReads = 400000;
#ifndef YK_PLAN_SMALL_BLOCK
#define YK_PLAN_SMALL_BLOCK 1024
#endif
constexpr int kPlanSmallBlock = YK_PLAN_SMALL_BLOCK;

template <int PER, int BLK = kPlanBlock>
__global__ __launch_bounds__(BLK) void plan_kernel(const u64 *off, u32 n_reads, u32 *lists,
                                                   Counters *ctr, u32 mode, u32 *zero,
                                                   u32 zero_words, u32 *counts, uint4 *mrec, u32 mrec_cap1, u32 mrec_cap2)
{
    constexpr int kPlanBlock = BLK;
    for (u32 i = blockIdx.x * kPlanBlock + threadIdx.x; i < zero_words; i += gridDim.x * kPlanBlock)
        zero[i] = 0;
    __shared__ u32 s_cnt[CLS_COUNT];
    __shared__ u32 s_base[CLS_COUNT];
    __shared__ unsigned long long s_iv[CLS_COUNT];
    if (threadIdx.x < CLS_COUNT) {
        s_cnt[threadIdx.x] = 0;
        s_iv[threadIdx.x] = 0;
    }
    __syncthreads();
    constexpr int kPlanPer = PER, kPlanReads = kPlanBlock * PER;
    u32 cls[kPlanPer], local[kPlanPer];
    u64 first[kPlanPer];
    u32 niv[kPlanPer];
    const u64 lt = (1ull << lane_id()) - 1ull;
#pragma unroll
    for (int k = 0; k < kPlanPer; k++) {
        const u32 r = blockIdx.x * (u32)kPlanReads + (u32)k * kPlanBlock + threadIdx.x;
        cls[k] = CLS_COUNT;
        local[k] = 0;
        u64 n = 0;
        first[k] = 0, niv[k] = 0;
        if (r < n_reads) {
            first[k] = off[r];
            n = off[r + 1] - first[k];
            niv[k] = (u32)n;
            const u64 m = 2 * n;
            u32 c;
            if (mode == 1) c = CLS_GENERAL;
            else if (mode != 2 && m <= 32) c = CLS_R2;
            else if (mode != 2 && m <= 64) c = CLS_R4;
            else if (mode != 2 && m <= 128) c = CLS_R8;
            else if (mode != 2 && m <= 256) c = CLS_R16;
            else if (mode == 0 && m <= 512) c = CLS_H16;
            else if (m <= 128) c = CLS_W2;
            else if (m <= 256) c = CLS_W4;
            else if (m <= 512) c = CLS_W8;
            else if (m <= kSmallEvents) c = CLS_W16;
            else if (m <= kMedium1Events) c = CLS_MED1;
            else if (m <= kMedium2Events) c = CLS_MED2;
            else c = CLS_GENERAL;
            cls[k] = c;
        }
        u64 todo = __builtin_amdgcn_ballot_w64(cls[k] != CLS_COUNT);
        while (todo) {
            const u32 c = (u32)__builtin_amdgcn_readlane((int)cls[k], (int)__builtin_ctzll(todo));
            const u64 mask = __builtin_amdgcn_ballot_w64(cls[k] == c);
            u64 iv = (cls[k] == c) ? n : 0;
#pragma unroll
            for (int d = 32; d > 0; d >>= 1) iv += __shfl_xor(iv, d, 64);
            u32 base = 0;
            if (lane_id() == (u32)__builtin_ctzll(mask)) {
                base = atomicAdd(&s_cnt[c], (u32)__builtin_popcountll(mask));
                atomicAdd(&s_iv[c], (unsigned long long)iv);
            }
            base = (u32)__builtin_amdgcn_readlane((int)base, (int)__builtin_ctzll(mask));
            if (cls[k] == c) local[k] = base + (u32)__builtin_popcountll(mask & lt);
            todo &= ~mask;
        }
    }
    __syncthreads();
    if (threadIdx.x < CLS_COUNT && s_cnt[threadIdx.x]) {
        s_base[threadIdx.x] = atomicAdd(&ctr->n[threadIdx.x], s_cnt[threadIdx.x]);
        atomicAdd((unsigned long long *)&ctr->iv[threadIdx.x], s_iv[threadIdx.x]);
    }
    __syncthreads();
#pragma unroll
    for (int k = 0; k < kPlanPer; k++) {
        const u32 r = blockIdx.x * (u32)kPlanReads + (u32)k * kPlanBlock + threadIdx.x;
        if (cls[k] != CLS_COUNT) {
            const u64 pos = s_base[cls[k]] + local[k];
            lists[(u64)cls[k] * n_reads + pos] = r;
            counts[r] = kClosedForm;
            if (mrec != nullptr && (cls[k] == CLS_MED1 || cls[k] == CLS_MED2)) {
                const u64 at = cls[k] == CLS_MED1 ? pos : (u64)mrec_cap1 + pos;
                if (pos < (cls[k] == CLS_MED1 ? mrec_cap1 : mrec_cap2))
                    mrec[at] = make_uint4((u32)first[k], (u32)(first[k] >> 32), niv[k], r);
            }
        }
    }
}

#ifndef YK_SCAN_BLOCK
#define YK_SCAN_BLOCK 1024
#endif
constexpr int kScanBlock = YK_SCAN_BLOCK;

__device__ __forceinline__ u32 classify(u32 bad, bool middle_gap, u32 len, double not_cov)
{
    if ((double)bad / (double)len > not_cov) return 2u;
    return middle_gap ? 1u : 0u;
}


__global__ __launch_bounds__(256) void classify_csr_kernel(const u64 *bad_offsets,
                                                           const uint2 *bad_regions, const u32 *len,
                                                           u32 n_reads, double not_cov,
                                                           uint8_t *read_type)
{
    const u32 r = blockIdx.x * 256u + threadIdx.x;
    if (r >= n_reads) return;
    const u64 a = bad_offsets[r], b = bad_offsets[r + 1];
    const u32 L = len[r];
    u32 bad = 0;
    bool middle = false;
    for (u64 k = a; k < b; k++) {
        const uint2 v = bad_regions[k];
        bad += v.y - v.x;
        middle |= (v.x != 0u) & (v.y != L);
    }
    read_type[r] = (uint8_t)classify(bad, middle, L, not_cov);
}

}
```

yacrd_amd/csrc/screen_reg.h:

```cpp
#pragma once
#include "device_common.h"
#include "wave_ops.h"

namespace yk {

#ifndef YK_SCREEN_WINDOW
#define YK_SCREEN_WINDOW 32
#endif
constexpr int kScreenWindow = YK_SCREEN_WINDOW;
constexpr int kScreenTabWords = (64 / 16) * (16 + 2 * kScreenWindow) * 4;
constexpr int kScreenTabWordsRows = (64 / 16) * (32 + 2 * kScreenWindow) * 4;
template <int WPB, int WORDS = kScreenTabWords>
__device__ __forceinline__ u32 *wave_screen_scratch()
{
    __shared__ __attribute__((aligned(16))) u32 s_tab[WPB][WORDS];
    return s_tab[threadIdx.x >> 6];
}

template <int LANES>
__device__ __forceinline__ bool group_any(u64 ballot)
{
    if (LANES == 64) return ballot != 0;
    return ((u32)(ballot >> (lane_id() & (u32)(64 - LANES))) & (u32)((1ull << (LANES & 63)) - 1ull)) != 0u;
}

struct HealthyRead {
    u32 a, b;
    i32 F, G;
};
#ifndef YK_SCREEN_SLIDES
#define YK_SCREEN_SLIDES 4
#endif
constexpr int kScreenSlides = YK_SCREEN_SLIDES;

template <int LANES, int WPB, bool SLID = false, int TABW = kScreenTabWords, int NB = LANES, int PAIRS = 4>
__device__ __forceinline__ bool healthy_screen(const uint4 (&v)[PAIRS], const bool (&real0)[PAIRS], const bool (&real1)[PAIRS],
                                               u32 len, i32 c, u32 pmin, u32 pmax, HealthyRead &hr, u32 P = 0, u32 Q = 0,
                                               u32 emin = 0, u32 smax = 0xFFFFFFFFu)
{
    constexpr int W = kScreenWindow, NBIN = 2 * W + NB, GROUPS = 64 / LANES, PER = W / LANES, ZPER = NBIN / LANES,
                  CPL = NB / LANES;
    constexpr u32 kEnd = 1u << 10, kField = kEnd - 1u;
    static_assert(W % LANES == 0 && PER >= 1 && W <= 64, "window bins per lane; a window index has six bits");
    static_assert(NB % LANES == 0 && NBIN % LANES == 0 && GROUPS * NBIN * 4 <= TABW, "scratch");
    static_assert(PAIRS * 2 * LANES <= 256, "a counter field has ten bits");
    const u32 lane = lane_id(), lig = lane & (u32)(LANES - 1), grp = lane / (u32)LANES;
    u32 *tab = wave_screen_scratch<WPB, TABW>() + grp * (u32)(NBIN * 4);
    uint4 *bins = reinterpret_cast<uint4 *>(tab);
    char *tb = reinterpret_cast<char *>(tab);

    const i32 bits = 32 - (i32)__builtin_clz(len | 1u) - ilog2c(NB) + (len != 0 ? 0 : -1);
    const u32 sh = (u32)max(bits, ilog2c(W));
    const u32 span = pmax - pmin, T = span - (u32)W;

#pragma unroll
    for (int q = 0; q < ZPER; q++) bins[lig + (u32)(LANES * q)] = make_uint4(0u, 0u, 0u, 0u);
    wave_lds_sync();

    const u32 cp = (lig & 3u) * 4u;
    u32 one = 1u, one_end = kEnd;
    if constexpr (!SLID) asm volatile("" : "+v"(one), "+v"(one_end));
    u32 ramp = 0;
    auto count = [&](u32 s, u32 e, bool real) {
        const u32 ds = s - pmin, dx = e - pmin;
        const u32 is = min(ds, (u32)W) + (ds >> sh);
        const u32 ie = (dx >> sh) + __builtin_elementwise_sub_sat(dx, T) + (u32)W;
        if constexpr (SLID) {
            const bool in_ramp = ds >= (u32)W && s < emin;
            ramp += (real && s >= pmin && in_ramp) ? 1u : 0u;
            if (real && s >= pmin && !in_ramp) atomicAdd(reinterpret_cast<u32 *>(tb + ((is << 4) + cp)), one);
            if (real && e <= pmax && !(e > smax && dx <= T)) atomicAdd(reinterpret_cast<u32 *>(tb + ((ie << 4) + cp)), one_end);
        } else if (real) {
            atomicAdd(reinterpret_cast<u32 *>(tb + ((is << 4) + cp)), one);
            atomicAdd(reinterpret_cast<u32 *>(tb + ((ie << 4) + cp)), one_end);
        }
    };
#pragma unroll
    for (int j = 0; j < PAIRS; j++) {
        count(v[j].x, v[j].y, real0[j]);
        count(v[j].z, v[j].w, real1[j]);
    }
    wave_lds_sync();

    u32 f[PER], fw = 0;
#pragma unroll
    for (int q = 0; q < PER; q++) {
        const u32 d = lig * (u32)PER + q;
        const u32 it = min((u32)(2 * W) - d + ((span - d) >> sh), (u32)(NBIN - 1));
        const uint4 h4 = bins[d], t4 = bins[it];
        f[q] = ((h4.x + h4.y + h4.z + h4.w) & kField) | ((t4.x + t4.y + t4.z + t4.w) & (kField << 10));
        fw += f[q];
    }
    u32 wb[CPL], w = 0;
#pragma unroll
    for (int q = 0; q < CPL; q++) {
        const uint4 c4 = bins[(u32)W + lig * (u32)CPL + q];
        wb[q] = (c4.x + c4.y + c4.z + c4.w) & ((kField << 10) | kField);
        w += wb[q];
    }
    const u32 fincl = gscan_add<LANES>(fw);
    u32 reached = 0;
    {
        const u32 k1 = (u32)min(c + 1, 0x1FF);
        u32 run = fincl - fw + (SLID ? ((512u - k1 + P) | ((512u - k1 + Q) << 10)) : (512u - k1) * (1u | kEnd));
#pragma unroll
        for (int q = 0; q < PER; q++) {
            run += f[q];
            reached += run & (0x200u | (0x200u << 10));
        }
    }
    const u32 cand = (((u32)PER - ((reached >> 9) & 7u)) << 20) | (((u32)PER - (reached >> 19)) << 26);
    const u32 wincl = gscan_add<LANES>(w | cand);
    u32 run = wincl - w, xl = 0xFFFFFFFFu;
#pragma unroll
    for (int q = 0; q < CPL; q++) {
        const u32 ex = run;
        run += wb[q];
        const i32 x = (i32)(ex & kField) - (i32)((run >> 10) & kField);
        xl = min(xl, (wb[q] & kField) != 0u ? (u32)(x + 0x10000) : 0xFFFFFFFFu);
    }
    const u32 xm = gscan_min<LANES>(xl);
    const i32 F = (i32)(fincl & kField) + (SLID ? (i32)P : 0), G = (i32)(fincl >> 10) + (SLID ? (i32)Q : 0);
    hr.F = F, hr.G = G;
    hr.a = pmin + ((wincl >> 20) & 63u);
    hr.b = pmax - (wincl >> 26);
    i32 open0 = F;
    if constexpr (SLID) open0 += (i32)gscan_add<LANES>(ramp);
    const bool deep = xm == 0xFFFFFFFFu || (i32)(xm - 0x10000u) + open0 > c;
    return deep && F > c && G > c;
}

struct VerdictsToGlobal {
    const SweepArgs &a;
    __device__ __forceinline__ void closed(u32 r, u32 ra, u32 rb, u32 len) const
    {
        if (ra != 0 || rb != len) a.closed[r] = make_uint2(ra, rb);
        else a.counts[r] = 0;
        if (a.prefilter == 2) atomicAdd(&a.ctr->prefiltered, 1u);
    }
    __device__ __forceinline__ void deferred(u32 r) const { a.counts[r] = kDeferredMark; }
};

template <int ITEMS>
struct ReadsKnown {
    u64 o[ITEMS];
    u32 n[ITEMS], len[ITEMS];
};

template <int LANES, int ITEMS, bool WIDE, int WPB = 1, int K = 16, int NB = LANES, bool NT = (ITEMS >= 2),
          int TABW = kScreenTabWords, class Sink>
__device__ __forceinline__ void screen_reads(const SweepArgs &a, const u32 (&r)[ITEMS], const bool (&active)[ITEMS], const Sink &sink,
                                             const ReadsKnown<ITEMS> *known = nullptr)
{
    static_assert(K % 4 == 0, "a lane takes its intervals in pairs");
    const u32 lane = lane_id(), lig = lane & (u32)(LANES - 1);
    const i32 c = (i32)min(a.cov, 0x3FFFFFFFu);
    u32 n[ITEMS], len[ITEMS];
    u64 o[ITEMS];
#pragma unroll
    for (int t = 0; t < ITEMS; t++) {
        o[t] = 0, n[t] = 0, len[t] = 0;
        if (known) {
            if (active[t]) o[t] = known->o[t], n[t] = known->n[t], len[t] = known->len[t];
        } else if (active[t]) {
            const ulonglong2 oo = load_extent(a.off + r[t]);
            o[t] = oo.x;
            n[t] = (u32)(oo.y - oo.x);
            len[t] = a.len[r[t]];
        }
    }
    uint4 v[ITEMS][K / 4];
#pragma unroll
    for (int t = 0; t < ITEMS; t++) {
        const bool two = n[t] >= 2u;
        const uint2 *src = two ? a.iv + o[t] : reinterpret_cast<const uint2 *>(a.off);
        const u32 last2 = two ? n[t] - 2u : 0u;
#pragma unroll
        for (int j = 0; j < K / 4; j++)
            v[t][j] = load_pair<NT>(src + min(2u * (lig + (u32)LANES * j), last2));
    }
#pragma unroll
    for (int t = 0; t < ITEMS; t++) {
        if (t > 0 && __builtin_amdgcn_ballot_w64(active[t]) == 0) break;
        const u32 len_c = min(len[t], kMaxKeyPos);
        u32 smin = v[t][0].x, emax = v[t][0].y, smax = v[t][0].x;
        i32 tmin = 0x7FFFFFFF;
#pragma unroll
        for (int j = 0; j < K / 4; j++) {
            smin = min(smin, min(v[t][j].x, v[t][j].z));
            smax = max(smax, max(v[t][j].x, v[t][j].z));
            emax = max(emax, max(v[t][j].y, v[t][j].w));
            tmin = min(tmin, min((i32)(v[t][j].y - v[t][j].x), (i32)(v[t][j].w - v[t][j].z)));
        }
        const int last_addr = (int)((lane | (u32)(LANES - 1)) << 2);
        const u32 pmin = (u32)__builtin_amdgcn_ds_bpermute(last_addr, (int)gscan_min<LANES>(smin));
        const u32 pmax = (u32)__builtin_amdgcn_ds_bpermute(last_addr, (int)gscan_max<LANES>(emax));
        const bool irregular = n[t] < 2u || pmax > len_c || smax > kMaxKeyPos || tmin < (i32)kScreenWindow;
        const bool girr = group_any<LANES>(__builtin_amdgcn_ballot_w64(irregular));
        const u32 n_eff = girr ? 0u : n[t];
        bool real0[K / 4], real1[K / 4];
#pragma unroll
        for (int j = 0; j < K / 4; j++) {
            const u32 i0 = 2u * (lig + (u32)LANES * j);
            real0[j] = i0 + 1u < n_eff;
            real1[j] = i0 < n_eff;
        }
        HealthyRead hr;
        bool healthy = healthy_screen<LANES, WPB, false, TABW, NB>(v[t], real0, real1, len[t], c, pmin, pmax, hr) && !girr;
        if constexpr (kScreenSlides > 0 && WIDE) {
            auto state_of = [&](bool nd, const HealthyRead &h) {
                return (nd ? 1u : 0u) | ((u32)min(max(h.F, 0), 1023) << 1) | ((u32)min(max(h.G, 0), 1023) << 11);
            };
            u32 st = state_of(!healthy && !girr && (i32)n[t] > c && (hr.F <= 3 * c + 6 || hr.G <= c), hr);
            if (__builtin_amdgcn_ballot_w64((st & 1u) != 0 && lig == (u32)(LANES - 1)) != 0) {
                u32 emin = v[t][0].y, smax2 = v[t][0].x;
#pragma unroll
                for (int j = 0; j < K / 4; j++) {
                    emin = min(emin, min(v[t][j].y, v[t][j].w));
                    smax2 = max(smax2, max(v[t][j].x, v[t][j].z));
                }
                const u32 gemin = (u32)__builtin_amdgcn_ds_bpermute(last_addr, (int)gscan_min<LANES>(emin));
                const u32 room_h = gemin - pmin;
                const u32 gsmax = (u32)__builtin_amdgcn_ds_bpermute(last_addr, (int)gscan_max<LANES>(smax2));
                const u32 room_t = pmax - gsmax;
                u32 ht = 0, PQ = 0;
#pragma unroll 1
                for (int slide = 0; slide < kScreenSlides; slide++) {
                    const u32 g = (u32)__builtin_amdgcn_ds_bpermute(last_addr, (int)st);
                    const bool gneed = (g & 1u) != 0;
                    const u32 gF = (g >> 1) & 1023u, gG = g >> 11;
                    if (gneed && (i32)gF <= c) ht += (u32)kScreenWindow, PQ = (PQ & 0xFFFF0000u) | gF;
                    if (gneed && (i32)gG <= c) ht += (u32)kScreenWindow << 16, PQ = (PQ & 0xFFFFu) | (gG << 16);
                    const u32 h0 = ht & 0xFFFFu, t0 = ht >> 16;
                    const bool go = gneed && room_h >= h0 + (u32)kScreenWindow && room_t >= t0 + (u32)kScreenWindow &&
                                    pmax - pmin >= h0 + t0 + 2u * (u32)kScreenWindow;
                    if (__builtin_amdgcn_ballot_w64(go) == 0) break;
                    bool r0[K / 4], r1[K / 4];
#pragma unroll
                    for (int j = 0; j < K / 4; j++) r0[j] = real0[j] && go, r1[j] = real1[j] && go;
                    wave_lds_sync();
                    HealthyRead h2;
                    const bool ok2 = healthy_screen<LANES, WPB, true, TABW, NB>(v[t], r0, r1, len[t], c, pmin + h0, pmax - t0, h2, PQ & 0xFFFFu, PQ >> 16, gemin, gsmax);
                    st = go ? state_of(!ok2 && (h2.F <= c || h2.G <= c), h2) : 0u;
                    if (go) healthy = ok2, hr.a = h2.a, hr.b = h2.b, hr.F = h2.F, hr.G = h2.G;
                }
            }
        }
        if (lig == (u32)(LANES - 1) && active[t]) {
            if (healthy || (!girr && (i32)n[t] <= c)) {
                const u32 ra = (i32)n[t] <= c ? len[t] : hr.a, rb = (i32)n[t] <= c ? len[t] : hr.b;
                sink.closed(r[t], ra, rb, len[t]);
            } else {
                sink.deferred(r[t]);
            }
        }
        if (t + 1 < ITEMS) wave_lds_sync();
    }
}

template <int LANES, int ITEMS, bool WIDE = false, int K = 16, int NB = LANES, bool NT = (ITEMS >= 2), int TABW = kScreenTabWords>
__device__ __forceinline__ void screen_block(const SweepArgs &a, u32 block)
{
    constexpr u32 GROUPS = 64 / LANES;
    const u32 grp = lane_id() / (u32)LANES;
    const u32 list_n = *a.list_n;
    const u32 idx0 = a.first + block * (u32)ITEMS * GROUPS;
    if (idx0 >= list_n) return;
    u32 r[ITEMS];
    bool active[ITEMS];
#pragma unroll
    for (int t = 0; t < ITEMS; t++) {
        const u32 idx = idx0 + (u32)t * GROUPS + grp;
        active[t] = idx < list_n;
        r[t] = active[t] ? a.list[idx] : 0u;
    }
    screen_reads<LANES, ITEMS, WIDE, 1, K, NB, NT, TABW>(a, r, active, VerdictsToGlobal{a});
}

}
```

yacrd_amd/csrc/sweep_wave.h:

```cpp
#pragma once
#include <type_traits>

#include "device_common.h"
#include "screen_reg.h"
#include "wave_ops.h"

namespace yk {

constexpr u32 kPadKey = 0xFFFFFFFEu;

template <int LANES, int K>
__device__ __forceinline__ void sweep_group_keys(u32 (&x)[K], u32 m, u32 len, i32 c,
                                                 bool active, u32 r, u64 badmask, u64 zmask,
                                                 bool zl_check, const SweepArgs &a,
                                                 const LaneConst &lc)
{
    const u32 lane = lane_id(), lig = lane & (u32)(LANES - 1);
    auto slot_of = [&]() {
        u32 rr = r;
        asm volatile("" : "+v"(rr));
        return a.stage + (a.off[rr] + 2 * (u64)rr);
    };

    bitonic_sort<LANES, K, 2>(x, lc);
// ... 11 lines not shown
                                         : ((u32)(badmask >> (lane & 48u)) & 0xFFFFu) != 0;

    u32 n_starts = 0;
#pragma unroll
    for (int q = 0; q < K; q++) n_starts += x[q] & 1u;
    const u32 delta = 2u * n_starts - (u32)K;
    const u32 dincl = gscan_add<LANES>(delta);
    const i32 depth_in = (i32)(dincl - delta);

    const u32 tail_base = m - lig * (u32)K;
    const u32 len_key = len > kMaxKeyPos ? 0xFFFFFFFFu : (len << kKeyShift);
    u32 mf_incl, ml_incl, mf_in, ml_in;
    u32 cnt = 0, fb = 0, fe = 0, cand = kNoKey;
    auto passes = [&](auto zl_tag) {
        constexpr bool ZL = decltype(zl_tag)::value;
        u32 mf = 0, ml = 0;
        i32 dd = depth_in;
#pragma unroll
        for (int q = 0; q < K; q++) {
            const u32 key = x[q], bit = key & 1u;
            const bool is_s = bit != 0, gt = dd > c + q;
            ml = (is_s && !gt) ? key : ml;
            if (ZL) mf = (!is_s && gt) ? max(mf, key ^ 2u) : mf;
            else mf = (!is_s && gt) ? key : mf;
            dd += (i32)(bit << 1);
        }
        if (!ZL) mf = mf ? (mf ^ 2u) : 0u;
        mf_incl = gscan_max<LANES>(mf);
        ml_incl = gscan_max<LANES>(ml);
        mf_in = max(gshift_up1<LANES>(mf_incl), kNoFlag);
        ml_in = gshift_up1<LANES>(ml_incl);

        u32 tc = ZL ? mf_in : (mf_in ^ 2u);
        u32 cml = ml_in;
        dd = depth_in;
#pragma unroll
        for (int q = 0; q < K; q++) {
            const u32 key = x[q], bit = key & 1u;
            const bool is_s = bit != 0, gt = dd > c + q;
            const bool fl = !is_s && gt, low = is_s && !gt;
            const bool eff = ZL ? (fl && (key ^ 2u) > tc) : fl;
            const u32 begin = ZL ? (tc ^ 2u) : tc;
            const bool close = eff && cml > begin;
            cnt += close ? 1u : 0u;
            fb = close ? begin : fb;
            fe = close ? cml : fe;
            const bool tail = fl && ((u32)dd == tail_base) && key >= len_key;
            cand = min(cand, tail ? (key >> kKeyShift) : kNoKey);
            tc = eff ? (ZL ? (key ^ 2u) : key) : tc;
            cml = low ? key : cml;
            dd += (i32)(bit << 1);
        }
    };
    if (zmask == 0) passes(std::false_type{});
    else passes(std::true_type{});
    i32 d;

    const bool live = active && !group_bad;
    u32 g_closed = 0;
    if (__builtin_amdgcn_ballot_w64(cnt != 0) != 0) {
        const u32 cincl = gscan_add<LANES>(cnt);
        g_closed = cincl;
        u32 pos = cincl - cnt;
        if (live && cnt == 1) {
            slot_of()[pos] = make_uint2(fb >> kKeyShift, fe >> kKeyShift);
        } else if (live && cnt > 1) {
            uint2 *slot = slot_of();
            u32 tc = mf_in, cml = ml_in;
            d = depth_in;
#pragma unroll
            for (int q = 0; q < K; q++) {
                const u32 key = x[q];
                const bool is_s = (key & 1u) != 0, gt = d > c;
                const bool fl = !is_s && gt, low = is_s && !gt;
                const bool eff = fl && (key ^ 2u) > tc;
                if (eff && cml > (tc ^ 2u))
                    slot[pos++] = make_uint2((tc ^ 2u) >> kKeyShift, cml >> kKeyShift);
                tc = eff ? (key ^ 2u) : tc;
                cml = low ? key : cml;
                d += is_s ? 1 : -1;
            }
        }
    }
    u32 min_ge = kNoKey;
    if (__builtin_amdgcn_ballot_w64(cand != kNoKey) != 0) min_ge = gscan_min<LANES>(cand);
    if (lig == LANES - 1 && active) {
        if (group_bad) {
            a.rej_list[atomicAdd(a.rej_count, 1u)] = r;
            a.counts[r] = 0;
        } else {
            a.counts[r] = finish_read(slot_of(), g_closed, mf_incl ? (mf_incl ^ 2u) : 0u, ml_incl, min_ge, len);
        }
    }
}


constexpr int kFilterTabWords = 304, kFilterKeyWords = 512;
template <int WPB>
__device__ __forceinline__ u32 *wave_filter_scratch()
{
    __shared__ __attribute__((aligned(16))) u32 s_scratch[WPB][kFilterTabWords + kFilterKeyWords];
    return s_scratch[threadIdx.x >> 6];
}

template <int LANES, int K, int WPB>
__device__ __forceinline__ bool prefilter(const u32 (&x)[K], u32 n, u32 len, i32 c, u32 (&y)[K / 2],
                                          u32 &m_out)
{
    static_assert(K == 16, "a lane reads its K/2 = 8 compacted keys as two 16-byte vectors");
    constexpr int NB = LANES, CAP = LANES * K / 2, GROUPS = 64 / LANES;
    static_assert(GROUPS * (NB + 1) * 4 <= kFilterTabWords && GROUPS * CAP <= kFilterKeyWords, "scratch");
    const u32 lane = lane_id(), lig = lane & (u32)(LANES - 1), grp = lane / (u32)LANES;
    u32 *scratch = wave_filter_scratch<WPB>();
    u32 *tab = scratch + grp * (u32)((NB + 1) * 4);
    u32 *keys = scratch + kFilterTabWords + grp * (u32)CAP;
    uint4 *my_bin = reinterpret_cast<uint4 *>(tab) + lig;
    uint4 *my_keys = reinterpret_cast<uint4 *>(keys) + lig * 2u;

    const i32 bits = 32 - (i32)__builtin_clz(len | 1u) - ilog2c(NB) + (len != 0 ? 0 : -1);
    const u32 sh = (u32)max(bits, 0), ksh = sh + kKeyShift;

    *my_bin = make_uint4(0u, 0u, 0u, 0u);
    my_keys[0] = make_uint4(kPadKey, kPadKey, kPadKey, kPadKey);
    my_keys[1] = make_uint4(kPadKey, kPadKey, kPadKey, kPadKey);
    wave_lds_sync();
    u32 *cell0 = tab + (lig & 3u);
    u32 *pad_cell = cell0 + NB * 4;
    u32 *cell[K];
#pragma unroll
    for (int q = 0; q < K; q++) {
        const bool real = lig + (u32)LANES * (q / 2) < n;
        u32 *p = cell0 + (x[q] >> ksh) * 4u;
        cell[q] = real ? p : pad_cell;
        atomicAdd(cell[q], (q & 1) ? 0x10000u : 1u);
    }
    wave_lds_sync();
    const uint4 w4 = *my_bin;
    const u32 w = w4.x + w4.y + w4.z + w4.w;
    const u32 incl = gscan_add<LANES>(w);
    const i32 S = (i32)(w & 0xFFFFu), E = (i32)(w >> 16);
    const i32 cs = (i32)(incl & 0xFFFFu), ce = (i32)(incl >> 16);
    const i32 depth_after = cs - ce, depth_at = depth_after - (S - E);
    const bool safe = (cs - S) - ce > c && lig < (len >> sh);
    const u64 sball = __builtin_amdgcn_ballot_w64(safe);
    if (sball == 0) return false;
    const u64 smask = LANES == 64 ? sball
                                  : (sball >> (lane & (u32)(64 - LANES))) & ((1ull << (LANES & 63)) - 1ull);
    const bool head = safe && (((smask << 1) >> lig) & 1ull) == 0;
    const bool tail = safe && (((smask >> 1) >> lig) & 1ull) == 0;
    const u32 hv = gscan_max<LANES>(head ? (((lig + 1u) << 16) | (u32)depth_at) : 0u);
    const i32 net = tail ? depth_after - (i32)(hv & 0xFFFFu) : 0;
    const u32 nsyn = min((u32)(net < 0 ? -net : net), (u32)CAP + 1u);
    const u32 synkey = (((hv >> 16) - 1u) << ksh) | (net > 0 ? 3u : 0u);

    const u32 mine = safe ? nsyn : (u32)(S + E);
    const u32 rincl = gscan_add<LANES>(mine);
    const u32 m = (u32)__builtin_amdgcn_ds_bpermute((int)((lane | (u32)(LANES - 1)) << 2), (int)rincl);
    if (__builtin_amdgcn_ballot_w64(m > (u32)CAP) != 0) return false;
    const u32 base = rincl - mine;
    {
        uint4 b4;
        b4.x = base;
        b4.y = b4.x + (w4.x & 0xFFFFu) + (w4.x >> 16);
        b4.z = b4.y + (w4.y & 0xFFFFu) + (w4.y >> 16);
        b4.w = b4.z + (w4.z & 0xFFFFu) + (w4.z >> 16);
        *my_bin = safe ? make_uint4(CAP, CAP, CAP, CAP) : b4;
        if (lig < 4u) tab[NB * 4 + lig] = (u32)CAP;
    }
#pragma unroll 1
    for (u32 t = 0; t < nsyn; t++) keys[base + t] = synkey;
    wave_lds_sync();
#pragma unroll
    for (int q0 = 0; q0 < K; q0 += 8) {
        u32 pos[8];
#pragma unroll
        for (int q = 0; q < 8; q++) pos[q] = atomicAdd(cell[q0 + q], 1u);
#pragma unroll
        for (int q = 0; q < 8; q++) {
            if (pos[q] < (u32)CAP) keys[pos[q]] = x[q0 + q];
        }
    }
    wave_lds_sync();
    const uint4 lo = my_keys[0], hi = my_keys[1];
    y[0] = lo.x, y[1] = lo.y, y[2] = lo.z, y[3] = lo.w;
    y[4] = hi.x, y[5] = hi.y, y[6] = hi.z, y[7] = hi.w;
    m_out = m;
    return true;
}

template <int LANES, int K, int WPB = 4>
__device__ __forceinline__ void sweep_group_read(const uint2 *__restrict__ iv, u32 n, u32 len,
                                                 u32 cov, bool active, u32 r,
                                                 const SweepArgs &a, const LaneConst &lc)
{
    const u32 lane = lane_id(), lig = lane & (u32)(LANES - 1);
    const i32 c = (i32)min(cov, 0x3FFFFFFFu);

    u32 x[K];
    u32 bad = 0, nz = 0;
    bool plain;
    {
        const uint2 *src = n ? iv : reinterpret_cast<const uint2 *>(a.off);
        const u32 last = n ? n - 1u : 0u;
        uint2 v[K / 2];
#pragma unroll
        for (int j = 0; j < K / 2; j++) v[j] = src[min(lig + (u32)LANES * j, last)];
        const u32 len_c = min(len, kMaxKeyPos);
        u32 irregular = 0;
#pragma unroll
        for (int j = 0; j < K / 2; j++) {
            const bool real = lig + (u32)LANES * j < n;
            irregular |= (real && (v[j].x >= v[j].y || v[j].y > len_c)) ? 1u : 0u;
            x[2 * j] = real ? ((v[j].x << kKeyShift) | 3u) : kPadKey;
            x[2 * j + 1] = real ? (v[j].y << kKeyShift) : kPadKey;
        }
        plain = __builtin_amdgcn_ballot_w64(irregular != 0) == 0;
        if (!plain) {
#pragma unroll
            for (int j = 0; j < K / 2; j++) {
                u32 ks, ke, b = 0, z = 0;
                make_event_keys(v[j], ks, ke, b, z);
                const bool real = lig + (u32)LANES * j < n;
                x[2 * j] = real ? ks : kPadKey;
                x[2 * j + 1] = real ? ke : kPadKey;
                bad |= real ? b : 0u;
                nz += real ? z : 0u;
            }
        }
    }
    const u64 badmask = __builtin_amdgcn_ballot_w64(bad != 0);
    const u64 zmask = __builtin_amdgcn_ballot_w64(nz != 0);
    if (LANES == 64 && badmask != 0) {
        if (lig == LANES - 1 && active) {
            a.rej_list[atomicAdd(a.rej_count, 1u)] = r;
            a.counts[r] = 0;
        }
        return;
    }
    const bool zl_check = (zmask & (zmask - 1)) != 0 || __builtin_amdgcn_ballot_w64(nz > 2) != 0;

    if constexpr (K == 16) {
        if (a.prefilter && plain) {
            u32 y[K / 2], mf;
            if (prefilter<LANES, K, WPB>(x, n, len, c, y, mf)) {
                if (a.prefilter == 2 && lig == 0 && active) atomicAdd(&a.ctr->prefiltered, 1u);
                sweep_group_keys<LANES, K / 2>(y, mf, len, c, active, r, badmask, zmask, zl_check, a, lc);
                return;
            }
        }
    }
    sweep_group_keys<LANES, K>(x, 2 * n, len, c, active, r, badmask, zmask, zl_check, a, lc);
}

template <int LANES, int K, int WPB = 4>
__device__ __forceinline__ void sweep_group_block(const SweepArgs &a, u32 block)
{
    const u32 lane = lane_id();
    const LaneConst lc = make_lane_const(lane);

    constexpr u32 GROUPS = 64 / LANES;
    const u32 list_n = *a.list_n;
    const u32 wave = block * (u32)WPB + (threadIdx.x >> 6);
    if (a.first + wave * GROUPS >= list_n) return;
    const u32 idx = a.first + wave * GROUPS + lane / (u32)LANES;
    const bool active = idx < list_n;
    u32 r = 0, n = 0, len = 0;
    u64 o = 0;
    if (active) {
        r = a.list[idx];
        o = a.off[r];
        n = (u32)(a.off[r + 1] - o);
        len = a.len[r];
    }
    sweep_group_read<LANES, K, WPB>(a.iv + o, n, len, a.cov, active, r, a, lc);
}

template <int LANES, int K>
__global__ __launch_bounds__(256) void sweep_group_kernel(SweepArgs a)
{
    sweep_group_block<LANES, K>(a, blockIdx.x);
}

template <int LANES, int K>
inline void launch_sweep_group(const SweepArgs &sa, u32 n_reads, hipStream_t stream)
{
    constexpr u32 per_block = 4u * (64 / LANES);
    const u32 grid = (n_reads + per_block - 1) / per_block;
    hipLaunchKernelGGL((sweep_group_kernel<LANES, K>), dim3(grid ? grid : 1), dim3(256), 0, stream, sa);
}

#ifndef YK_DEFER_OCC
#define YK_DEFER_OCC 6
#endif
constexpr int kFusedWaves = 4, kDeferWaves = 1, kDeferOcc = YK_DEFER_OCC;
static_assert(kDeferWaves == 1, "screen_block indexes list entries by workgroup: one wavefront each");
struct FusedArgs {
    SweepArgs base;
    u32 n_entries;
    u32 cls[5];
    u32 block_end[5];
    u32 first[5];
    const u32 *list[5];
    const u32 *list_n[5];
};

template <bool DEFER, int WPB, int ITEMS = 1, bool WIDE = false>
__device__ __forceinline__ void sweep_small_fused_body(const FusedArgs &f)
{
    u32 g = blockIdx.x;
    {
        const u32 nb = gridDim.x, x = g & 7u, q = nb >> 3, rem = nb & 7u;
        g = x * q + min(x, rem) + (g >> 3);
    }
    u32 e = 0, first = 0;
    while (e + 1 < f.n_entries && g >= f.block_end[e]) {
        first = f.block_end[e];
        e++;
    }
    SweepArgs a = f.base;
    a.list = f.list[e];
    a.list_n = f.list_n[e];
    a.first = f.first[e];
    const u32 b = g - first;
    constexpr bool ROWS = DEFER && ITEMS == 2 && !WIDE;
    constexpr int TABW = ROWS ? kScreenTabWordsRows : kScreenTabWords;
    switch (f.cls[e]) {
    case CLS_R2: sweep_group_block<16, 2, WPB>(a, b); break;
    case CLS_R4: sweep_group_block<16, 4, WPB>(a, b); break;
    case CLS_R8: sweep_group_block<16, 8, WPB>(a, b); break;
    case CLS_R16:
        if constexpr (DEFER) screen_block<16, ITEMS, WIDE, 16, 16, (ITEMS >= 2), TABW>(a, b);
        else sweep_group_block<16, 16, WPB>(a, b);
        break;
    default:
        if constexpr (ROWS) screen_block<16, 1, false, 32, 32, true, TABW>(a, b);
        else if constexpr (DEFER) screen_block<32, ITEMS, WIDE>(a, b);
        else sweep_group_block<32, 16, WPB>(a, b);
        break;
    }
}
__global__ __launch_bounds__(64 * kDeferWaves, kDeferOcc) void sweep_small_fused_defer_kernel(FusedArgs f)
{
    sweep_small_fused_body<true, kDeferWaves>(f);
}
__global__ __launch_bounds__(64 * kDeferWaves, kDeferOcc) void sweep_small_fused_defer_wide_kernel(FusedArgs f)
{
    sweep_small_fused_body<true, kDeferWaves, 1, true>(f);
}
#ifndef YK_DEFER2_OCC
#define YK_DEFER2_OCC YK_DEFER_OCC
#endif
__global__ __launch_bounds__(64, YK_DEFER2_OCC) void sweep_small_fused_defer2_kernel(FusedArgs f)
{
    sweep_small_fused_body<true, 1, 2>(f);
}
__global__ __launch_bounds__(64 * kFusedWaves, 5) void sweep_small_fused_kernel(FusedArgs f)
{
    sweep_small_fused_body<false, kFusedWaves>(f);
}

inline u32 sweep_group_reads_per_block(int cls, int waves = 4)
{
    return ((cls <= CLS_R16) ? 4u : (cls == CLS_H16) ? 2u : 1u) * (u32)waves;
}

}
```

yacrd_amd/engine.py:

```python
import ctypes
import os
import subprocess
from collections import namedtuple

import numpy as np

_HERE = os.path.dirname(os.path.abspath(__file__))
_LIB = os.path.join(_HERE, "lib", "libyacrd_hip.so")

NOT_BAD, CHIMERIC, NOT_COVERED = 0, 1, 2
TYPE_NAMES = {NOT_BAD: "NotBad", CHIMERIC: "Chimeric", NOT_COVERED: "NotCovered"}
F_FORCE_GENERAL = 1
F_FORCE_LDS_SORT = 2
F_WAVE_ONLY = 8
F_NO_HALVES = 16
F_TIMING_FULL = 32
F_NO_PREDICTION = 64
F_NO_PREFILTER = 256
F_COUNT_PREFILTERED = 512
F_NO_TIMING = 1024
F_BLOCKING_WAIT = 2048
F_NO_DEFER = 4096
F_ALWAYS_DEFER = 8192
F_TIMING_SAMPLED = 32768
F_STREAM_SCREEN = 65536
F_SCREEN_ITEMS_1 = 262144
F_SCREEN_ITEMS_2 = 524288
F_NO_FUSED_SCREEN = 1048576
F_SCREEN_WIDE = 2097152
F_ONE_LAUNCH = 4194304

EXPORTED_SYMBOLS = [
    "yacrd_abi_version", "yacrd_last_error", "yacrd_engine_create", "yacrd_engine_destroy",
    "yacrd_engine_run", "yacrd_result_free", "yacrd_engine_run_device", "yacrd_engine_fetch",
    "yacrd_engine_last_timing", "yacrd_partition_reads", "yacrd_engine_classify",
    "yacrd_engines_run_partitioned", "yacrd_engine_timing_total", "yacrd_engine_event_overhead", "yacrd_engine_submit_device", "yacrd_engine_wait", "yacrd_engines_run_device_batches",
    "yacrd_engine_submit", "yacrd_engine_collect", "yacrd_pinned_alloc", "yacrd_pinned_free",
    "yacrd_stream_open", "yacrd_stream_sink", "yacrd_stream_acquire", "yacrd_stream_commit",
    "yacrd_stream_finish", "yacrd_stream_last_stats", "yacrd_stream_reset", "yacrd_stream_close",
    "yacrd_engine_ingest_paf", "yacrd_engine_ingest_overlaps", "yacrd_engine_ingest_overlaps_mem", "yacrd_engines_ingest_overlaps",
    "yacrd_engines_ingest_overlaps_mem", "yacrd_reads_free", "yacrd_engine_trim",
    "yacrd_engine_ingest_report", "yacrd_engine_ingest_report_mem", "yacrd_engine_write_report", "yacrd_engine_write_report_mem",
    "yacrd_engine_edit_overlaps", "yacrd_engine_edit_overlaps_mem", "yacrd_edit_text_free",
    "yacrd_engine_edit_overlaps_gzip_mem", "yacrd_engine_edit_overlaps_gzip_file",
    "yacrd_engine_edit_fastq", "yacrd_engine_edit_fastq_mem", "yacrd_engine_edit_fastq_gzip_mem", "yacrd_engine_edit_fastq_gzip_file",
    "yacrd_engine_edit_fasta", "yacrd_engine_edit_fasta_mem", "yacrd_engine_edit_fasta_gzip_mem", "yacrd_engine_edit_fasta_gzip_file",
    "yacrd_engine_gunzip_mem", "yacrd_engine_edit_fastq_bgzf_mem", "yacrd_engine_edit_fastq_bgzf_file",
    "yacrd_engine_edit_fasta_bgzf_mem", "yacrd_engine_edit_fasta_bgzf_file",
    "yacrd_engine_gzip_mem", "yacrd_gzip_writer_open", "yacrd_gzip_writer_write", "yacrd_gzip_writer_sink", "yacrd_gzip_writer_close",
    "yacrd_gzip_writer_abort",
    "yacrd_stream_device_of", "yacrd_stream_group_open", "yacrd_stream_group_sink", "yacrd_stream_group_finish",
    "yacrd_stream_group_last_stats", "yacrd_stream_group_reset", "yacrd_stream_group_close",
]


class EngineError(RuntimeError):
    pass


class NeedsHostParser(EngineError):
    """yacrd_engine_ingest_paf returned YACRD_EFALLBACK: the input is for the host parser."""


E_FALLBACK = 5


class _Reads(ctypes.Structure):
    _fields_ = [("n_reads", ctypes.c_uint64), ("n_records", ctypes.c_uint64),
                ("lengths", ctypes.POINTER(ctypes.c_uint32)), ("name_off", ctypes.POINTER(ctypes.c_uint64)),
                ("names", ctypes.POINTER(ctypes.c_char))]


class _ReportTable(ctypes.Structure):
    _fields_ = [("n_reads", ctypes.c_uint64)] + \
               [(n, ctypes.c_void_p) for n in ("name_off", "names", "lengths", "bad_offsets", "bad_regions", "read_type")]


class _ReportWriteStats(ctypes.Structure):
    _fields_ = [(n, ctypes.c_uint64) for n in ("n_reads", "n_regions", "text_bytes")] + \
               [(n, ctypes.c_float) for n in ("up_ms", "kernel_ms", "out_ms")] + [("resident", ctypes.c_uint32)]


class _IngestStats(ctypes.Structure):
    _fields_ = [("text_bytes", ctypes.c_uint64), ("n_records", ctypes.c_uint64), ("n_reads", ctypes.c_uint64)] + \
               [(n, ctypes.c_float) for n in ("text_ms", "parse_ms", "build_ms", "run_ms", "d2h_ms")]


class _TypeTable(ctypes.Structure):
    _fields_ = [("n_reads", ctypes.c_uint64), ("name_off", ctypes.c_void_p), ("names", ctypes.c_void_p), ("read_type", ctypes.c_void_p)]


class _EditStats(ctypes.Structure):
    _fields_ = [(n, ctypes.c_uint64) for n in ("text_bytes", "kept_bytes", "n_lines", "n_kept")] + \
               [(n, ctypes.c_float) for n in ("text_ms", "table_ms", "kernel_ms", "out_ms")] + [("mirror_reused", ctypes.c_uint32)]


class _SeqEditStats(ctypes.Structure):
    _fields_ = [(n, ctypes.c_uint64) for n in ("text_bytes", "out_bytes", "n_records", "n_out_records")] + \
               [(n, ctypes.c_float) for n in ("text_ms", "table_ms", "kernel_ms", "out_ms")]


class _GzipStats(ctypes.Structure):
    _fields_ = [("in_bytes", ctypes.c_uint64), ("out_bytes", ctypes.c_uint64), ("n_members", ctypes.c_uint64), ("n_stored", ctypes.c_uint64),
                ("h2d_ms", ctypes.c_float), ("kernel_ms", ctypes.c_float), ("d2h_ms", ctypes.c_float), ("write_ms", ctypes.c_float)]


class _GunzipStats(ctypes.Structure):
    _fields_ = [(n, ctypes.c_uint64) for n in ("in_bytes", "out_bytes", "n_members")] + \
               [(n, ctypes.c_float) for n in ("walk_ms", "h2d_ms", "kernel_ms", "d2h_ms")]


from .host import ByteSink


class _Cfg(ctypes.Structure):
    _fields_ = [("device_id", ctypes.c_int32), ("flags", ctypes.c_uint32)]


class _Result(ctypes.Structure):
    _fields_ = [("n_reads", ctypes.c_uint64), ("n_regions", ctypes.c_uint64),
                ("bad_offsets", ctypes.POINTER(ctypes.c_uint64)),
                ("bad_regions", ctypes.POINTER(ctypes.c_uint32)),
                ("read_type", ctypes.POINTER(ctypes.c_uint8))]


class _DevResult(ctypes.Structure):
    _fields_ = [("n_reads", ctypes.c_uint64), ("n_regions", ctypes.c_uint64),
                ("d_bad_offsets", ctypes.c_void_p), ("d_bad_regions", ctypes.c_void_p),
                ("d_read_type", ctypes.c_void_p)]


class DeviceBatch(ctypes.Structure):
    _fields_ = [("d_offsets", ctypes.c_void_p), ("d_intervals", ctypes.c_void_p), ("d_lengths", ctypes.c_void_p),
                ("n_reads", ctypes.c_uint64), ("n_intervals", ctypes.c_uint64), ("coverage", ctypes.c_uint32),
                ("not_coverage", ctypes.c_double)]


BATCH_DONE = ctypes.CFUNCTYPE(ctypes.c_int, ctypes.c_void_p, ctypes.c_uint32, ctypes.c_void_p,
                              ctypes.POINTER(_DevResult))


class _Timing(ctypes.Structure):
    _fields_ = [(n, ctypes.c_float) for n in
                ("h2d_ms", "plan_ms", "sweep_small_ms", "sweep_medium_ms", "sweep_general_ms",
                 "compact_ms", "d2h_ms", "total_ms")] + \
               [(n, ctypes.c_uint64) for n in
                ("n_small", "n_medium", "n_general", "iv_small", "iv_medium", "iv_general")] + \
               [("class_ms", ctypes.c_float * 12), ("class_reads", ctypes.c_uint64 * 12),
                ("class_intervals", ctypes.c_uint64 * 12), ("fused_ms", ctypes.c_float),
                ("fused_reads", ctypes.c_uint64), ("fused_intervals", ctypes.c_uint64),
                ("prefiltered_reads", ctypes.c_uint64), ("deferred_reads", ctypes.c_uint64),
                ("deferred_intervals", ctypes.c_uint64), ("screened", ctypes.c_uint32),
                ("timed_runs", ctypes.c_uint32), ("screen_items", ctypes.c_uint32), ("screen_wide", ctypes.c_uint32),
                ("one_launch", ctypes.c_uint32), ("fused_reruns", ctypes.c_uint32),
                ("predicted", ctypes.c_uint32), ("prediction_misses", ctypes.c_uint32),
                ("build_switches", ctypes.c_uint32), ("sorting_build", ctypes.c_uint32)]

CLASS_NAMES = "R2,R4,R8,R16,H16,W2,W4,W8,W16,M1,M2,BIG".split(",")
CLASS_KERNELS = {
    "R2": "sweep_small_fused_kernel", "R4": "sweep_small_fused_kernel", "R8": "sweep_small_fused_kernel",
    "R16": "sweep_small_fused_kernel", "H16": "sweep_small_fused_kernel",
    "W2": "sweep_group_kernel<64, 2>", "W4": "sweep_group_kernel<64, 4>", "W8": "sweep_group_kernel<64, 8>",
    "W16": "sweep_group_kernel<64, 16>",
    "M1": "screen_wg_kernel + screen_wg_fused_kernel over what it leaves",
    "M2": "screen_wg_kernel + screen_wg_fused_kernel over what it leaves (+ sweep_lds_kernel<1024, 32768> over what exceeds 16 384 events)",
    "BIG": "bs_setup / bs_minmax / bs_hist / bs_verdict (screen_big.h)",
}


class _StreamStats(ctypes.Structure):
    _fields_ = [("n_records", ctypes.c_uint64), ("h2d_bytes", ctypes.c_uint64),
                ("h2d_busy_ms", ctypes.c_float), ("build_ms", ctypes.c_float),
                ("run_ms", ctypes.c_float), ("d2h_ms", ctypes.c_float)]


class OvlRec(ctypes.Structure):
    _fields_ = [(n, ctypes.c_uint32) for n in ("a", "b", "sa", "ea", "sb", "eb")]


_ACQUIRE = ctypes.CFUNCTYPE(ctypes.c_int, ctypes.c_void_p, ctypes.POINTER(ctypes.POINTER(OvlRec)),
                            ctypes.POINTER(ctypes.c_uint64))
_COMMIT = ctypes.CFUNCTYPE(ctypes.c_int, ctypes.c_void_p, ctypes.POINTER(OvlRec), ctypes.c_uint64)


class RecSink(ctypes.Structure):
    _fields_ = [("ctx", ctypes.c_void_p), ("acquire", _ACQUIRE), ("commit", _COMMIT)]


OVL_REC_DTYPE = np.dtype([(n, np.uint32) for n in ("a", "b", "sa", "ea", "sb", "eb")])

Result = namedtuple("Result", "bad_offsets bad_regions read_type")

_lib = None


def lib_path():
    return _LIB


def build(force=False):
    cmd = ["make", "-s", "-C", os.path.join(_HERE, "csrc")]
    if force:
        cmd.append("-B")
    subprocess.check_call(cmd)
    return _LIB


def _share_hip_runtime_with_torch():
    if os.environ.get("YACRD_HIP_RUNTIME", "") == "system":
        return None
    import importlib.util
    import sys
    try:
        if "torch" in sys.modules:
            tdir = os.path.dirname(sys.modules["torch"].__file__)
        else:
            spec = importlib.util.find_spec("torch")
            if spec is None or not spec.origin:
                return None
            tdir = os.path.dirname(spec.origin)
    except (ImportError, ValueError):
        return None
    cand = os.path.join(tdir, "lib", "libamdhip64.so")
    if not os.path.exists(cand):
        return None
    try:
        ctypes.CDLL(cand, mode=ctypes.RTLD_GLOBAL)
    except OSError:
        return None
    return cand


def peer_copy_counts():
    lib = load_library()
    out = (ctypes.c_uint64 * 3)()
    lib.yacrd_debug_peer_copy_counts.restype = None
    lib.yacrd_debug_peer_copy_counts(out)
    return [int(x) for x in out]


def live_bytes():
    lib = load_library()
    out = (ctypes.c_uint64 * 2)()
    lib.yacrd_debug_live_bytes.restype = None
    lib.yacrd_debug_live_bytes(out)
    return (int(out[0]), int(out[1]))


def load_library():
    global _lib
    if _lib is not None:
        return _lib
    if not os.path.exists(_LIB):
        raise EngineError("%s is missing: run `python -c 'import __graft_entry__ as g; g.build()'` "
                          "(there is no CPU fallback)" % _LIB)
    _share_hip_runtime_with_torch()
    lib = ctypes.CDLL(_LIB)
    u64p, u32p, u8p = (ctypes.POINTER(t) for t in (ctypes.c_uint64, ctypes.c_uint32, ctypes.c_uint8))
    lib.yacrd_abi_version.restype = ctypes.c_int
    lib.yacrd_last_error.restype = ctypes.c_char_p
    lib.yacrd_engine_create.argtypes = [ctypes.POINTER(_Cfg), ctypes.POINTER(ctypes.c_void_p)]
    lib.yacrd_engine_destroy.argtypes = [ctypes.c_void_p]
    lib.yacrd_engine_destroy.restype = None
    lib.yacrd_engine_run.argtypes = [ctypes.c_void_p, u64p, u32p, u32p, ctypes.c_uint64,
                                     ctypes.c_uint32, ctypes.c_double, ctypes.POINTER(_Result)]
    lib.yacrd_result_free.argtypes = [ctypes.POINTER(_Result)]
    lib.yacrd_result_free.restype = None
    lib.yacrd_engine_run_device.argtypes = [ctypes.c_void_p, ctypes.c_void_p, ctypes.c_void_p,
                                            ctypes.c_void_p, ctypes.c_uint64, ctypes.c_uint64,
                                            ctypes.c_uint32, ctypes.c_double,
                                            ctypes.POINTER(_DevResult)]
    lib.yacrd_engine_submit_device.argtypes = [ctypes.c_void_p, ctypes.c_void_p, ctypes.c_void_p,
                                               ctypes.c_void_p, ctypes.c_uint64, ctypes.c_uint64,
                                               ctypes.c_uint32, ctypes.c_double]
    lib.yacrd_engine_wait.argtypes = [ctypes.c_void_p, ctypes.POINTER(_DevResult)]
    lib.yacrd_engines_run_device_batches.argtypes = [ctypes.POINTER(ctypes.c_void_p), ctypes.c_uint32,
                                                     ctypes.POINTER(DeviceBatch), ctypes.c_uint32, BATCH_DONE,
                                                     ctypes.c_void_p, ctypes.POINTER(_DevResult)]
    lib.yacrd_engine_fetch.argtypes = [ctypes.c_void_p, ctypes.POINTER(_Result)]
    lib.yacrd_engine_ingest_paf.argtypes = [ctypes.c_void_p, ctypes.c_char_p, ctypes.c_int, ctypes.c_uint32, ctypes.c_double,
                                            ctypes.POINTER(_Result), ctypes.POINTER(_Reads), ctypes.POINTER(_IngestStats)]
    lib.yacrd_engine_ingest_overlaps.argtypes = [ctypes.c_void_p, ctypes.c_char_p, ctypes.c_int, ctypes.c_int, ctypes.c_uint32,
                                                 ctypes.c_double, ctypes.POINTER(_Result), ctypes.POINTER(_Reads),
                                                 ctypes.POINTER(_IngestStats)]
    lib.yacrd_engine_ingest_overlaps_mem.argtypes = [ctypes.c_void_p, ctypes.c_void_p, ctypes.c_uint64, ctypes.c_int, ctypes.c_int,
                                                     ctypes.c_uint32, ctypes.c_double, ctypes.POINTER(_Result), ctypes.POINTER(_Reads),
                                                     ctypes.POINTER(_IngestStats)]
    lib.yacrd_engines_ingest_overlaps.argtypes = [ctypes.POINTER(ctypes.c_void_p), ctypes.c_uint32, ctypes.c_char_p, ctypes.c_int,
                                                  ctypes.c_int, ctypes.c_uint32, ctypes.c_double, ctypes.POINTER(_Result),
                                                  ctypes.POINTER(_Reads), ctypes.POINTER(_IngestStats)]
    lib.yacrd_engines_ingest_overlaps_mem.argtypes = [ctypes.POINTER(ctypes.c_void_p), ctypes.c_uint32, ctypes.c_void_p, ctypes.c_uint64,
                                                      ctypes.c_int, ctypes.c_int, ctypes.c_uint32, ctypes.c_double,
                                                      ctypes.POINTER(_Result), ctypes.POINTER(_Reads), ctypes.POINTER(_IngestStats)]
    lib.yacrd_engine_ingest_report.argtypes = [ctypes.c_void_p, ctypes.c_char_p, ctypes.c_int, ctypes.c_double, ctypes.POINTER(_Result),
                                               ctypes.POINTER(_Reads), ctypes.POINTER(_IngestStats)]
    lib.yacrd_engine_ingest_report_mem.argtypes = [ctypes.c_void_p, ctypes.c_void_p, ctypes.c_uint64, ctypes.c_int, ctypes.c_double,
                                                   ctypes.POINTER(_Result), ctypes.POINTER(_Reads), ctypes.POINTER(_IngestStats)]
    lib.yacrd_engine_write_report.argtypes = [ctypes.c_void_p, ctypes.POINTER(_ReportTable), ctypes.c_char_p,
                                              ctypes.POINTER(_ReportWriteStats)]
    lib.yacrd_engine_write_report_mem.argtypes = [ctypes.c_void_p, ctypes.POINTER(_ReportTable), ctypes.POINTER(ctypes.c_void_p),
                                                  ctypes.POINTER(ctypes.c_uint64), ctypes.POINTER(_ReportWriteStats)]
    lib.yacrd_debug_sort_pairs.argtypes = [ctypes.c_void_p, ctypes.c_void_p, ctypes.c_void_p, ctypes.c_uint64, ctypes.c_uint64]
    lib.yacrd_engine_trim.argtypes = [ctypes.c_void_p]
    lib.yacrd_engine_edit_overlaps.argtypes = [ctypes.c_void_p, ctypes.c_int, ctypes.c_char_p, ctypes.c_char_p, ctypes.c_int, ctypes.c_int,
                                               ctypes.POINTER(_TypeTable), ctypes.POINTER(_EditStats)]
    lib.yacrd_engine_edit_overlaps_mem.argtypes = [ctypes.c_void_p, ctypes.c_int, ctypes.c_void_p, ctypes.c_uint64, ctypes.c_int,
                                                   ctypes.POINTER(_TypeTable), ctypes.POINTER(ctypes.c_void_p),
                                                   ctypes.POINTER(ctypes.c_uint64), ctypes.POINTER(_EditStats)]
    lib.yacrd_engine_edit_overlaps_gzip_mem.argtypes = [ctypes.c_void_p, ctypes.c_int, ctypes.c_void_p, ctypes.c_uint64, ctypes.c_int,
                                                        ctypes.POINTER(_TypeTable), ctypes.POINTER(ctypes.c_void_p),
                                                        ctypes.POINTER(ctypes.c_uint64), ctypes.POINTER(_EditStats), ctypes.POINTER(_GzipStats)]
    lib.yacrd_engine_edit_overlaps_gzip_file.argtypes = [ctypes.c_void_p, ctypes.c_int, ctypes.c_void_p, ctypes.c_uint64, ctypes.c_int,
                                                         ctypes.POINTER(_TypeTable), ctypes.c_char_p, ctypes.POINTER(_EditStats),
                                                         ctypes.POINTER(_GzipStats)]
    lib.yacrd_edit_text_free.argtypes = [ctypes.c_void_p]
    lib.yacrd_engine_edit_fastq.argtypes = [ctypes.c_void_p, ctypes.c_int, ctypes.c_char_p, ctypes.c_char_p, ctypes.c_int,
                                            ctypes.POINTER(_ReportTable), ctypes.POINTER(_SeqEditStats)]
    lib.yacrd_engine_edit_fastq_mem.argtypes = [ctypes.c_void_p, ctypes.c_int, ctypes.c_void_p, ctypes.c_uint64, ctypes.POINTER(_ReportTable),
                                                ctypes.POINTER(ctypes.c_void_p), ctypes.POINTER(ctypes.c_uint64),
                                                ctypes.POINTER(_SeqEditStats)]
    lib.yacrd_engine_edit_fastq_gzip_mem.argtypes = [ctypes.c_void_p, ctypes.c_int, ctypes.c_void_p, ctypes.c_uint64,
                                                     ctypes.POINTER(_ReportTable), ctypes.POINTER(ctypes.c_void_p),
                                                     ctypes.POINTER(ctypes.c_uint64), ctypes.POINTER(_SeqEditStats),
                                                     ctypes.POINTER(_GzipStats)]
    lib.yacrd_engine_edit_fastq_gzip_file.argtypes = [ctypes.c_void_p, ctypes.c_int, ctypes.c_void_p, ctypes.c_uint64,
                                                      ctypes.POINTER(_ReportTable), ctypes.c_char_p, ctypes.POINTER(_SeqEditStats),
                                                      ctypes.POINTER(_GzipStats)]
    for fq, fa in ((getattr(lib, "yacrd_engine_edit_fastq" + form), getattr(lib, "yacrd_engine_edit_fasta" + form))
                   for form in ("", "_mem", "_gzip_mem", "_gzip_file")):
        fa.argtypes = fq.argtypes
    lib.yacrd_edit_text_free.restype = None
    lib.yacrd_engine_gunzip_mem.argtypes = [ctypes.c_void_p, ctypes.c_void_p, ctypes.c_uint64, ctypes.POINTER(ctypes.c_void_p),
# ... 37 lines not shown
    lib.yacrd_stream_sink.argtypes = [ctypes.c_void_p, ctypes.POINTER(RecSink)]
    lib.yacrd_stream_acquire.argtypes = [ctypes.c_void_p, ctypes.POINTER(ctypes.POINTER(OvlRec)),
                                         ctypes.POINTER(ctypes.c_uint64)]
    lib.yacrd_stream_commit.argtypes = [ctypes.c_void_p, ctypes.POINTER(OvlRec), ctypes.c_uint64]
    lib.yacrd_stream_finish.argtypes = [ctypes.c_void_p, u32p, ctypes.c_uint64, u32p, ctypes.c_uint64,
                                        ctypes.c_uint32, ctypes.c_double, ctypes.POINTER(_Result)]
    lib.yacrd_stream_last_stats.argtypes = [ctypes.c_void_p, ctypes.POINTER(_StreamStats)]
    lib.yacrd_stream_close.argtypes = [ctypes.c_void_p]
    lib.yacrd_stream_close.restype = None
    lib.yacrd_stream_device_of.argtypes = [ctypes.c_uint32, ctypes.c_uint32]
    lib.yacrd_stream_device_of.restype = ctypes.c_uint32
    lib.yacrd_stream_group_open.argtypes = [ctypes.POINTER(ctypes.c_void_p), ctypes.c_uint32, ctypes.c_uint64,
                                            ctypes.c_uint32, ctypes.POINTER(ctypes.c_void_p)]
    lib.yacrd_stream_group_sink.argtypes = [ctypes.c_void_p, ctypes.POINTER(RecSink)]
    lib.yacrd_stream_group_finish.argtypes = lib.yacrd_stream_finish.argtypes
    lib.yacrd_stream_group_last_stats.argtypes = [ctypes.c_void_p, ctypes.c_uint32, ctypes.POINTER(_StreamStats),
                                                  ctypes.POINTER(ctypes.c_uint64)]
    lib.yacrd_stream_group_reset.argtypes = [ctypes.c_void_p]
    lib.yacrd_stream_group_close.argtypes = [ctypes.c_void_p]
    lib.yacrd_stream_group_close.restype = None
    _lib = lib
    return lib


def _check(lib, rc):
    if rc != 0:
        raise EngineError("yacrd engine error %d: %s" % (rc, lib.yacrd_last_error().decode()))


def _ptr(a, t):
    return a.ctypes.data_as(ctypes.POINTER(t))


def _take(lib, res):
    R, G = int(res.n_reads), int(res.n_regions)
    bo = np.ctypeslib.as_array(res.bad_offsets, shape=(R + 1,)).copy()
    br = (np.ctypeslib.as_array(res.bad_regions, shape=(2 * G,)).copy().reshape(-1, 2)
          if G else np.zeros((0, 2), dtype=np.uint32))
    rt = np.ctypeslib.as_array(res.read_type, shape=(R,)).copy() if R else np.zeros(0, np.uint8)
    lib.yacrd_result_free(ctypes.byref(res))
    return Result(bo, br, rt)


def partition_reads(offsets, n_parts):
    lib = load_library()
    offsets = np.ascontiguousarray(offsets, dtype=np.uint64)
    cuts = np.zeros(n_parts + 1, dtype=np.uint64)
    _check(lib, lib.yacrd_partition_reads(_ptr(offsets, ctypes.c_uint64), offsets.shape[0] - 1,
                                          n_parts, _ptr(cuts, ctypes.c_uint64)))
    return cuts


def run_partitioned(engines, offsets, intervals, lengths, coverage, not_coverage):
    lib = load_library()
    offsets = np.ascontiguousarray(offsets, dtype=np.uint64)
    intervals = np.ascontiguousarray(intervals, dtype=np.uint32).reshape(-1)
    lengths = np.ascontiguousarray(lengths, dtype=np.uint32)
    if intervals.size == 0:
        intervals = np.zeros(2, dtype=np.uint32)
    handles = (ctypes.c_void_p * len(engines))(*[e._h for e in engines])
    res = _Result()
    _check(lib, lib.yacrd_engines_run_partitioned(
        handles, len(engines), _ptr(offsets, ctypes.c_uint64), _ptr(intervals, ctypes.c_uint32),
        _ptr(lengths, ctypes.c_uint32), offsets.shape[0] - 1, min(int(coverage), 0xFFFFFFFF),
        float(not_coverage), ctypes.byref(res)))
    return _take(lib, res)


def ingest_overlaps(engines, source, coverage, not_coverage, n_threads=0, fmt=1):
    lib = load_library()
    handles = (ctypes.c_void_p * len(engines))(*[e._h for e in engines])
    res, rd, st = _Result(), _Reads(), _IngestStats()
    cov = min(int(coverage), 0xFFFFFFFF)
    if isinstance(source, (str, os.PathLike)):
        rc = lib.yacrd_engines_ingest_overlaps(handles, len(engines), os.fsencode(source), int(fmt), int(n_threads), cov,
                                               float(not_coverage), ctypes.byref(res), ctypes.byref(rd), ctypes.byref(st))
    else:
        if isinstance(source, tuple):
            addr, n, keep = int(source[0]), int(source[1]), None
        else:
            keep = ctypes.create_string_buffer(bytes(source), len(source))
            addr, n = ctypes.addressof(keep), len(source)
        rc = lib.yacrd_engines_ingest_overlaps_mem(handles, len(engines), addr, n, int(fmt), int(n_threads), cov, float(not_coverage),
                                                   ctypes.byref(res), ctypes.byref(rd), ctypes.byref(st))
        del keep
    return engines[0]._ingested(rc, res, rd, st)


def run_device_batches(engines, batches, done=None):
    lib = load_library()
    arr = (DeviceBatch * len(batches))()
    for i, b in enumerate(batches):
        arr[i] = DeviceBatch(b[0], b[1], b[2], b[3], b[4], min(int(b[5]), 0xFFFFFFFF), float(b[6]))
    handles = (ctypes.c_void_p * len(engines))(*[e._h for e in engines])
    by_handle = {e._h.value: e for e in engines}
    cb = BATCH_DONE(lambda user, i, h, res: 1 if done(i, by_handle[h]) else 0) if done else BATCH_DONE()
    out = _DevResult()
    _check(lib, lib.yacrd_engines_run_device_batches(handles, len(engines), arr, len(batches), cb, None,
                                                     ctypes.byref(out)))
    return out


class Engine:

    def __init__(self, device_id=-1, flags=0):
        self._lib = load_library()
        self._h = ctypes.c_void_p()
        self.device_id = device_id
        cfg = _Cfg(device_id, flags)
        _check(self._lib, self._lib.yacrd_engine_create(ctypes.byref(cfg), ctypes.byref(self._h)))

    def close(self):
        if self._h:
            self._lib.yacrd_engine_destroy(self._h)
            self._h = ctypes.c_void_p()

    def __del__(self):
        try:
            self.close()
        except Exception:
            pass

    def __enter__(self):
        return self

    def __exit__(self, *a):
        self.close()

    def run(self, offsets, intervals, lengths, coverage, not_coverage):
        offsets = np.ascontiguousarray(offsets, dtype=np.uint64)
        intervals = np.ascontiguousarray(intervals, dtype=np.uint32).reshape(-1)
        lengths = np.asarray(lengths)
        if lengths.size and int(lengths.max()) > 0xFFFFFFFF:
            raise EngineError("read length >= 2^32 is not supported by the engine ABI")
        lengths = np.ascontiguousarray(lengths, dtype=np.uint32)
        n_reads = offsets.shape[0] - 1
        if lengths.shape[0] != n_reads or intervals.shape[0] != 2 * int(offsets[-1]):
            raise EngineError("malformed CSR")
        res = _Result()
        _check(self._lib, self._lib.yacrd_engine_run(
            self._h, _ptr(offsets, ctypes.c_uint64), _ptr(intervals, ctypes.c_uint32),
            _ptr(lengths, ctypes.c_uint32), n_reads, min(int(coverage), 0xFFFFFFFF),
            float(not_coverage), ctypes.byref(res)))
        return _take(self._lib, res)

    def run_device(self, d_offsets, d_intervals, d_lengths, n_reads, n_intervals, coverage,
                   not_coverage):
        out = _DevResult()
        _check(self._lib, self._lib.yacrd_engine_run_device(
            self._h, d_offsets, d_intervals, d_lengths, n_reads, n_intervals,
            min(int(coverage), 0xFFFFFFFF), float(not_coverage), ctypes.byref(out)))
        return out

    def submit_device(self, d_offsets, d_intervals, d_lengths, n_reads, n_intervals, coverage,
                      not_coverage):
        _check(self._lib, self._lib.yacrd_engine_submit_device(
            self._h, d_offsets, d_intervals, d_lengths, n_reads, n_intervals,
            min(int(coverage), 0xFFFFFFFF), float(not_coverage)))

    def wait(self):
        out = _DevResult()
        _check(self._lib, self._lib.yacrd_engine_wait(self._h, ctypes.byref(out)))
        return out

    def ingest_paf(self, path, coverage, not_coverage, n_threads=0, fmt=1):
        res, rd, st = _Result(), _Reads(), _IngestStats()
        rc = self._lib.yacrd_engine_ingest_overlaps(self._h, os.fsencode(path), int(fmt), int(n_threads),
                                                    min(int(coverage), 0xFFFFFFFF), float(not_coverage), ctypes.byref(res),
                                                    ctypes.byref(rd), ctypes.byref(st))
        return self._ingested(rc, res, rd, st)

    def ingest_text(self, text, coverage, not_coverage, n_threads=0, fmt=1):
        res, rd, st = _Result(), _Reads(), _IngestStats()
        if isinstance(text, tuple):
            addr, n = int(text[0]), int(text[1])
            keep = None
        else:
            keep = ctypes.create_string_buffer(bytes(text), len(text))
            addr, n = ctypes.addressof(keep), len(text)
        rc = self._lib.yacrd_engine_ingest_overlaps_mem(self._h, addr, n, int(fmt), int(n_threads), min(int(coverage), 0xFFFFFFFF),
                                                        float(not_coverage), ctypes.byref(res), ctypes.byref(rd), ctypes.byref(st))
        del keep
        return self._ingested(rc, res, rd, st)

    def ingest_report(self, path_or_bytes, not_coverage, n_threads=0):
        res, rd, st = _Result(), _Reads(), _IngestStats()
        if isinstance(path_or_bytes, (str, os.PathLike)):
            rc = self._lib.yacrd_engine_ingest_report(self._h, os.fsencode(path_or_bytes), int(n_threads), float(not_coverage),
                                                      ctypes.byref(res), ctypes.byref(rd), ctypes.byref(st))
            return self._ingested(rc, res, rd, st)
        if isinstance(path_or_bytes, tuple):
            addr, n = int(path_or_bytes[0]), int(path_or_bytes[1])
            keep = None
        else:
            keep = ctypes.create_string_buffer(bytes(path_or_bytes), len(path_or_bytes))
            addr, n = ctypes.addressof(keep), len(path_or_bytes)
        rc = self._lib.yacrd_engine_ingest_report_mem(self._h, addr, n, int(n_threads), float(not_coverage), ctypes.byref(res),
                                                      ctypes.byref(rd), ctypes.byref(st))
        del keep
        return self._ingested(rc, res, rd, st)

    def _ingested(self, rc, res, rd, st):
        if rc == E_FALLBACK:
            raise NeedsHostParser(self._lib.yacrd_last_error().decode())
        _check(self._lib, rc)
        R = int(rd.n_reads)
        lengths = np.ctypeslib.as_array(rd.lengths, shape=(R,)).copy() if R else np.zeros(0, np.uint32)
        off = np.ctypeslib.as_array(rd.name_off, shape=(R + 1,)).copy()
        blob = ctypes.string_at(rd.names, int(off[-1])) if R else b""
        names = [blob[int(off[i]):int(off[i + 1])].decode("utf-8", "surrogateescape") for i in range(R)]
        stats = {n: getattr(st, n) for n, _ in _IngestStats._fields_}
        self._lib.yacrd_reads_free(ctypes.byref(rd))
        return _take(self._lib, res), names, lengths, stats

    def _report_table(self, names, lengths, result):
        if names is None and lengths is None and result is None:
            return None, None
        if names is None or lengths is None or result is None:
            raise ValueError("names, lengths and result: all three, or none for the table the last ingest left on the device")
        blobs = [n if isinstance(n, bytes) else n.encode("utf-8", "surrogateescape") for n in names]
        R = len(blobs)
        off = np.zeros(R + 1, np.uint64)
        if blobs:
            off[1:] = np.cumsum([len(b) for b in blobs], dtype=np.uint64)
        blob = ctypes.create_string_buffer(b"".join(blobs), int(off[-1]) + 1)
        lens = np.ascontiguousarray(lengths, dtype=np.uint32)
        bo = np.ascontiguousarray(result.bad_offsets, dtype=np.uint64)
        br = np.ascontiguousarray(result.bad_regions, dtype=np.uint32).reshape(-1)
        rt = np.ascontiguousarray(result.read_type, dtype=np.uint8)
        if lens.shape != (R,) or bo.shape != (R + 1,) or rt.shape != (R,) or (R and br.size != 2 * int(bo[-1])):
            raise ValueError("the report table's arrays do not fit one another")
        if br.size == 0:
            br = np.zeros(2, np.uint32)
        if R == 0:
            lens, rt = np.zeros(1, np.uint32), np.zeros(1, np.uint8)
        t = _ReportTable(R, off.ctypes.data, ctypes.addressof(blob), lens.ctypes.data, bo.ctypes.data, br.ctypes.data, rt.ctypes.data)
        return ctypes.byref(t), (t, off, blob, lens, bo, br, rt)

    def _report_written(self, rc, st):
        if rc == E_FALLBACK:
            raise NeedsHostParser(self._lib.yacrd_last_error().decode())
        _check(self._lib, rc)
        self.report_write_stats = {n: getattr(st, n) for n, _ in _ReportWriteStats._fields_}
        return self.report_write_stats

    def write_report(self, out_path, names=None, lengths=None, result=None):
        t, keep = self._report_table(names, lengths, result)
        st = _ReportWriteStats()
        rc = self._lib.yacrd_engine_write_report(self._h, t, os.fsencode(out_path), ctypes.byref(st))
        del keep
        return self._report_written(rc, st)

    def report_text(self, names=None, lengths=None, result=None):
        t, keep = self._report_table(names, lengths, result)
        st = _ReportWriteStats()
        out, n_out = ctypes.c_void_p(), ctypes.c_uint64()
        rc = self._lib.yacrd_engine_write_report_mem(self._h, t, ctypes.byref(out), ctypes.byref(n_out), ctypes.byref(st))
        del keep
        self._report_written(rc, st)
        try:
            return ctypes.string_at(out.value, int(n_out.value)) if n_out.value else b""
        finally:
            self._lib.yacrd_edit_text_free(out)

    def debug_sort_pairs(self, keys, vals, key_bound):
        keys = np.array(keys, dtype=np.uint64)
        vals = np.array(vals, dtype=np.uint32)
        _check(self._lib, self._lib.yacrd_debug_sort_pairs(self._h, keys.ctypes.data, vals.ctypes.data, keys.shape[0], int(key_bound)))
        return keys, vals

    def debug_input_csr(self):
        f = self._lib.yacrd_debug_last_input_csr
        f.argtypes = [ctypes.c_void_p, ctypes.POINTER(ctypes.c_uint64), ctypes.POINTER(ctypes.c_uint64), ctypes.c_void_p,
                      ctypes.c_void_p, ctypes.c_void_p]
        R, I = ctypes.c_uint64(), ctypes.c_uint64()
        rc = f(self._h, ctypes.byref(R), ctypes.byref(I), None, None, None)
        if rc == 1:
            return None
        _check(self._lib, rc)
        off = np.zeros(R.value + 1, dtype=np.uint64)
        iv = np.zeros((I.value, 2), dtype=np.uint32)
        ln = np.zeros(R.value, dtype=np.uint32)
        _check(self._lib, f(self._h, ctypes.byref(R), ctypes.byref(I), off.ctypes.data, iv.ctypes.data, ln.ctypes.data))
        return off, iv, ln

    def debug_counters(self):
        class _Counters(ctypes.Structure):
            _fields_ = [("n", ctypes.c_uint32 * 16), ("iv", ctypes.c_uint64 * 16), ("rej_small", ctypes.c_uint32),
                        ("rej_med", ctypes.c_uint32), ("rej_big", ctypes.c_uint32), ("region_overflow", ctypes.c_uint32),
                        ("scan_ticket", ctypes.c_uint32), ("ob_unsupported", ctypes.c_uint32), ("prefiltered", ctypes.c_uint32),
                        ("over_med", ctypes.c_uint32), ("fb_med", ctypes.c_uint32 * 2), ("fb_big", ctypes.c_uint32),
                        ("fbq_head", ctypes.c_uint32 * 2), ("fbq_done", ctypes.c_uint32 * 2), ("bs_chunks", ctypes.c_uint32),
                        ("fused_gave_up", ctypes.c_uint32), ("total_regions", ctypes.c_uint64)]
        c = _Counters()
        self._lib.yacrd_debug_last_counters.restype = ctypes.c_uint64
        self._lib.yacrd_debug_last_counters.argtypes = [ctypes.c_void_p, ctypes.c_void_p, ctypes.c_uint64]
        self._lib.yacrd_debug_last_counters(self._h, ctypes.byref(c), ctypes.sizeof(c))
        out = {}
        for n, _ in _Counters._fields_:
            v = getattr(c, n)
            out[n] = list(v) if hasattr(v, "__len__") else int(v)
        return out

    def _type_table(self, names, read_type):
        blobs = [n if isinstance(n, bytes) else n.encode("utf-8", "surrogateescape") for n in names]
        off = np.zeros(len(blobs) + 1, np.uint64)
        if blobs:
            off[1:] = np.cumsum([len(b) for b in blobs], dtype=np.uint64)
        blob = ctypes.create_string_buffer(b"".join(blobs), int(off[-1]) + 1)
        types = np.ascontiguousarray(read_type, dtype=np.uint8)
        if types.shape != (len(blobs),):
            raise ValueError("read_type: one type per name")
        tt = _TypeTable(len(blobs), off.ctypes.data, ctypes.addressof(blob), types.ctypes.data)
        return tt, (off, blob, types)

    def _edited(self, rc, st):
        if rc == E_FALLBACK:
            raise NeedsHostParser(self._lib.yacrd_last_error().decode())
        _check(self._lib, rc)
        self.edit_stats = {n: getattr(st, n) for n, _ in _EditStats._fields_}
        return self.edit_stats

    def edit_overlaps(self, op, src, out_path, names, read_type, fmt=0, n_threads=0):
        tt, keep = self._type_table(names, read_type)
        st = _EditStats()
        rc = self._lib.yacrd_engine_edit_overlaps(self._h, int(op), os.fsencode(src), os.fsencode(out_path), int(fmt), int(n_threads),
                                                  ctypes.byref(tt), ctypes.byref(st))
        del keep
        return self._edited(rc, st)

    def edit_overlaps_text(self, op, text, names, read_type, fmt):
        tt, keep = self._type_table(names, read_type)
        st = _EditStats()
        buf = ctypes.create_string_buffer(bytes(text), len(text) + 1)
        out, n_out = ctypes.c_void_p(), ctypes.c_uint64()
        rc = self._lib.yacrd_engine_edit_overlaps_mem(self._h, int(op), ctypes.addressof(buf), len(text), int(fmt), ctypes.byref(tt),
                                                      ctypes.byref(out), ctypes.byref(n_out), ctypes.byref(st))
        del keep
        self._edited(rc, st)
        try:
            return ctypes.string_at(out.value, int(n_out.value)) if n_out.value else b""
        finally:
            self._lib.yacrd_edit_text_free(out)

    def edit_overlaps_gzip(self, op, text, names, read_type, fmt, out_path=None):
        tt, keep = self._type_table(names, read_type)
        st, gs = _EditStats(), _GzipStats()
        buf = np.frombuffer(text, dtype=np.uint8)
        n = int(buf.size)
        addr = ctypes.c_void_p(buf.ctypes.data if n else None)
        out, n_out = ctypes.c_void_p(), ctypes.c_uint64()
        if out_path is None:
            rc = self._lib.yacrd_engine_edit_overlaps_gzip_mem(self._h, int(op), addr, n, int(fmt), ctypes.byref(tt),
                                                               ctypes.byref(out), ctypes.byref(n_out), ctypes.byref(st), ctypes.byref(gs))
        else:
            rc = self._lib.yacrd_engine_edit_overlaps_gzip_file(self._h, int(op), addr, n, int(fmt), ctypes.byref(tt),
                                                                os.fsencode(out_path), ctypes.byref(st), ctypes.byref(gs))
        del keep, buf
        self._edited(rc, st)
        self.gzip_stats = {f: getattr(gs, f) for f, _ in _GzipStats._fields_}
        if out_path is not None:
            return self.edit_stats, self.gzip_stats
        try:
            return ctypes.string_at(out.value, int(n_out.value))
        finally:
            self._lib.yacrd_edit_text_free(out)

    def _seq_table(self, names, lengths, result):
        if isinstance(result, (tuple, list)) and not hasattr(result, "bad_offsets"):
            bo, br, rt = result

            class _R:
                bad_offsets, bad_regions, read_type = bo, br, rt
            result = _R
        if len(names) == 0:
            result = type("_E", (), {"bad_offsets": np.zeros(1, np.uint64), "bad_regions": np.zeros(0, np.uint32),
                                     "read_type": np.zeros(0, np.uint8)})
        return self._report_table(names, lengths, result)

    def _seq_edited(self, rc, st):
        if rc == E_FALLBACK:
            raise NeedsHostParser(self._lib.yacrd_last_error().decode())
        _check(self._lib, rc)
        self.seq_edit_stats = {n: getattr(st, n) for n, _ in _SeqEditStats._fields_}
        return self.seq_edit_stats

    def edit_fastq(self, op, src, out_path, names, lengths, result, n_threads=0):
        return self._edit_seq_file("fastq", op, src, out_path, names, lengths, result, n_threads)

    def edit_fastq_text(self, op, text, names, lengths, result):
        return self._edit_seq_text("fastq", op, text, names, lengths, result)

    def edit_fastq_gzip(self, op, text, names, lengths, result, out_path=None):
        return self._edit_seq_gzip("fastq", op, text, names, lengths, result, out_path)

    def edit_fasta(self, op, src, out_path, names, lengths, result, n_threads=0):
        return self._edit_seq_file("fasta", op, src, out_path, names, lengths, result, n_threads)

    def edit_fasta_text(self, op, text, names, lengths, result):
        return self._edit_seq_text("fasta", op, text, names, lengths, result)

    def edit_fasta_gzip(self, op, text, names, lengths, result, out_path=None):
        return self._edit_seq_gzip("fasta", op, text, names, lengths, result, out_path)

    def _edit_seq_file(self, fmt, op, src, out_path, names, lengths, result, n_threads):
        t, keep = self._seq_table(names, lengths, result)
        st = _SeqEditStats()
        rc = getattr(self._lib, "yacrd_engine_edit_" + fmt)(self._h, int(op), os.fsencode(src), os.fsencode(out_path), int(n_threads), t,
                                                            ctypes.byref(st))
        del keep
        return self._seq_edited(rc, st)

    def _edit_seq_text(self, fmt, op, text, names, lengths, result):
        t, keep = self._seq_table(names, lengths, result)
        st = _SeqEditStats()
        buf = np.frombuffer(text, dtype=np.uint8)
        n = int(buf.size)
        out, n_out = ctypes.c_void_p(), ctypes.c_uint64()
        rc = getattr(self._lib, "yacrd_engine_edit_%s_mem" % fmt)(self._h, int(op), ctypes.c_void_p(buf.ctypes.data if n else None), n, t,
                                                                  ctypes.byref(out), ctypes.byref(n_out), ctypes.byref(st))
        del keep, buf
        self._seq_edited(rc, st)
        try:
            return ctypes.string_at(out.value, int(n_out.value)) if n_out.value else b""
        finally:
            self._lib.yacrd_edit_text_free(out)

    def edit_fastq_bgzf(self, op, blob, names, lengths, result, out_path=None):
        return self._edit_seq_gzip("fastq", op, blob, names, lengths, result, out_path, bgzf=True)

    def edit_fasta_bgzf(self, op, blob, names, lengths, result, out_path=None):
        return self._edit_seq_gzip("fasta", op, blob, names, lengths, result, out_path, bgzf=True)

    def gunzip(self, data):
        buf = np.frombuffer(data, dtype=np.uint8)
        n = int(buf.size)
        st = _GunzipStats()
        out, n_out = ctypes.c_void_p(), ctypes.c_uint64()
        rc = self._lib.yacrd_engine_gunzip_mem(self._h, ctypes.c_void_p(buf.ctypes.data if n else None), n, ctypes.byref(out), ctypes.byref(n_out),
                                               ctypes.byref(st))
        del buf
        if rc == E_FALLBACK:
            raise NeedsHostParser(self._lib.yacrd_last_error().decode())
        _check(self._lib, rc)
        self.gunzip_stats = {f: getattr(st, f) for f, _ in _GunzipStats._fields_}
        try:
            return ctypes.string_at(out.value, int(n_out.value)) if n_out.value else b""
        finally:
            self._lib.yacrd_edit_text_free(out)

    def _edit_seq_gzip(self, fmt, op, text, names, lengths, result, out_path, bgzf=False):
        t, keep = self._seq_table(names, lengths, result)
        st, gs, us = _SeqEditStats(), _GzipStats(), _GunzipStats()
        more = (ctypes.byref(us),) if bgzf else ()
        kind = "bgzf" if bgzf else "gzip"
        buf = np.frombuffer(text, dtype=np.uint8)
        n = int(buf.size)
        addr = ctypes.c_void_p(buf.ctypes.data if n else None)
        out, n_out = ctypes.c_void_p(), ctypes.c_uint64()
        if out_path is None:
            rc = getattr(self._lib, "yacrd_engine_edit_%s_%s_mem" % (fmt, kind))(self._h, int(op), addr, n, t, ctypes.byref(out), ctypes.byref(n_out),
                                                                                 ctypes.byref(st), ctypes.byref(gs), *more)
        else:
            rc = getattr(self._lib, "yacrd_engine_edit_%s_%s_file" % (fmt, kind))(self._h, int(op), addr, n, t, os.fsencode(out_path), ctypes.byref(st),
                                                                                  ctypes.byref(gs), *more)
        del keep, buf
        self._seq_edited(rc, st)
        if bgzf:
            self.gunzip_stats = {f: getattr(us, f) for f, _ in _GunzipStats._fields_}
        self.gzip_stats = {f: getattr(gs, f) for f, _ in _GzipStats._fields_}
        if out_path is not None:
            return self.seq_edit_stats, self.gzip_stats
        try:
            return ctypes.string_at(out.value, int(n_out.value))
        finally:
            self._lib.yacrd_edit_text_free(out)

    def gzip(self, data):
        data = bytes(data)
        st = _GzipStats()
        out, n_out = ctypes.c_void_p(), ctypes.c_uint64()
        buf = ctypes.create_string_buffer(data, len(data) + 1)
        _check(self._lib, self._lib.yacrd_engine_gzip_mem(self._h, ctypes.addressof(buf), len(data), ctypes.byref(out), ctypes.byref(n_out),
                                                          ctypes.byref(st)))
        self.gzip_stats = {f: getattr(st, f) for f, _ in _GzipStats._fields_}
        try:
            return ctypes.string_at(out.value, int(n_out.value))
        finally:
            self._lib.yacrd_edit_text_free(out)

    def gzip_writer(self, out_path, segment_bytes=0, n_buffers=0):
        return GzipWriter(self, out_path, segment_bytes, n_buffers)

    def trim(self):
        _check(self._lib, self._lib.yacrd_engine_trim(self._h))

    def fetch(self):
        res = _Result()
        _check(self._lib, self._lib.yacrd_engine_fetch(self._h, ctypes.byref(res)))
        return _take(self._lib, res)

    def timing(self):
        t = _Timing()
        _check(self._lib, self._lib.yacrd_engine_last_timing(self._h, ctypes.byref(t)))
        out = {}
        for n, _ in _Timing._fields_:
            v = getattr(t, n)
            out[n] = list(v) if n.startswith("class_") else v
        return out

    def event_overhead_ms(self):
        ms = ctypes.c_float()
        _check(self._lib, self._lib.yacrd_engine_event_overhead(self._h, ctypes.byref(ms)))
        return float(ms.value)

    def timing_total(self, reset=False):
        t = _Timing()
        n = ctypes.c_uint64()
        _check(self._lib, self._lib.yacrd_engine_timing_total(self._h, ctypes.byref(t),
                                                              ctypes.byref(n), 1 if reset else 0))
        out = {}
        for name, _ in _Timing._fields_:
            v = getattr(t, name)
            out[name] = list(v) if name.startswith("class_") else v
        return out, int(n.value)

    def submit(self, offsets, intervals, lengths, coverage, not_coverage):
        n_reads = offsets.shape[0] - 1
        self._keep = (offsets, intervals, lengths)
        _check(self._lib, self._lib.yacrd_engine_submit(
            self._h, _ptr(offsets, ctypes.c_uint64), _ptr(intervals.reshape(-1), ctypes.c_uint32),
            _ptr(lengths, ctypes.c_uint32), n_reads, min(int(coverage), 0xFFFFFFFF),
            float(not_coverage)))

    def collect(self):
        res = _Result()
        _check(self._lib, self._lib.yacrd_engine_collect(self._h, ctypes.byref(res)))
        self._keep = None
        return _take(self._lib, res)

    def classify(self, bad_offsets, bad_regions, lengths, not_coverage):
        bad_offsets = np.ascontiguousarray(bad_offsets, dtype=np.uint64)
        bad_regions = np.ascontiguousarray(bad_regions, dtype=np.uint32).reshape(-1)
        lengths = np.ascontiguousarray(lengths, dtype=np.uint32)
        n_reads = lengths.shape[0]
        out = np.zeros(max(n_reads, 1), dtype=np.uint8)
        if bad_regions.size == 0:
            bad_regions = np.zeros(2, dtype=np.uint32)
        _check(self._lib, self._lib.yacrd_engine_classify(
            self._h, _ptr(bad_offsets, ctypes.c_uint64), _ptr(bad_regions, ctypes.c_uint32),
            _ptr(lengths, ctypes.c_uint32), n_reads, float(not_coverage),
            _ptr(out, ctypes.c_uint8)))
        return out[:n_reads]


class GzipWriter:

    def __init__(self, engine, out_path, segment_bytes=0, n_buffers=0):
        self._lib = engine._lib
        self._engine = engine
        self._h = ctypes.c_void_p()
        self.stats = None
        _check(self._lib, self._lib.yacrd_gzip_writer_open(engine._h, os.fsencode(out_path), int(segment_bytes), int(n_buffers),
                                                           ctypes.byref(self._h)))

    def write(self, data):
        data = bytes(data)
        if not self._h:
            raise EngineError("the gzip writer is closed")
        _check(self._lib, self._lib.yacrd_gzip_writer_write(self._h, data, len(data)))
        return len(data)

    def sink(self):
        s = ByteSink()
        _check(self._lib, self._lib.yacrd_gzip_writer_sink(self._h, ctypes.byref(s)))
        return s

    def close(self):
        if not self._h:
            return self.stats
        h, self._h = self._h, ctypes.c_void_p()
        st = _GzipStats()
        _check(self._lib, self._lib.yacrd_gzip_writer_close(h, ctypes.byref(st)))
        self.stats = {f: getattr(st, f) for f, _ in _GzipStats._fields_}
        return self.stats

    def abort(self):
        if self._h:
            h, self._h = self._h, ctypes.c_void_p()
            self._lib.yacrd_gzip_writer_abort(h)

    def __del__(self):
        try:
            self.abort()
        except Exception:
            pass

    def __enter__(self):
        return self

    def __exit__(self, exc_type, exc, tb):
        if exc_type is None:
            self.close()
        else:
            self.abort()
        return False
# ... 177 lines not shown
```

Measured before the change: 3.126 billion.

## Screen H16 reads directly from offsets, overlapping plan on a side stream

Adds a direct screening path for inputs dominated by the 129-256 interval class. The H16 screen kernel reads offsets straight from the CSR instead of waiting for the plan kernel to build class lists. It runs on the main stream while plan and the other register classes run concurrently on a side stream, joined afterwards by events. This removes the plan-to-screen dependency, so plan latency overlaps with the dominant screen. The cost is a full-grid scan in which every read is checked for membership, extra stream and event sync, and more complex timing bookkeeping.

```diff
diff --git a/include/yacrd_engine_debug.h b/include/yacrd_engine_debug.h
--- a/include/yacrd_engine_debug.h
+++ b/include/yacrd_engine_debug.h
@@ -17,6 +17,8 @@
 #define YACRD_F_NO_FUSED_SCREEN 1048576u
 #define YACRD_F_STREAM_SCREEN 65536u
 #define YACRD_F_SCREEN_WIDE 2097152u
+#define YACRD_F_SCREEN_DIRECT 8388608u
+#define YACRD_F_NO_SCREEN_DIRECT 16777216u
 
 #ifdef __cplusplus
 extern "C" {
@@ -27,6 +29,7 @@
                                uint32_t *lengths);
 void yacrd_debug_peer_copy_counts(uint64_t out[3]);
 void yacrd_debug_live_bytes(uint64_t out[2]);
+uint64_t yacrd_debug_direct_runs(const yacrd_engine *e);
 #ifdef __cplusplus
 }
 #endif
diff --git a/yacrd_amd/__init__.py b/yacrd_amd/__init__.py
--- a/yacrd_amd/__init__.py
+++ b/yacrd_amd/__init__.py
@@ -1,5 +1,5 @@
 from .engine import (
     Engine, EngineError, NeedsHostParser, Result, lib_path, load_library, build, partition_reads, run_partitioned, ingest_overlaps,
-    NOT_BAD, CHIMERIC, NOT_COVERED, TYPE_NAMES, F_FORCE_GENERAL, F_FORCE_LDS_SORT, F_WAVE_ONLY, F_NO_HALVES, F_TIMING_FULL, F_NO_PREDICTION, F_NO_PREFILTER, F_COUNT_PREFILTERED, F_NO_TIMING, F_BLOCKING_WAIT, F_NO_DEFER, F_ALWAYS_DEFER, F_TIMING_SAMPLED, F_STREAM_SCREEN, F_SCREEN_ITEMS_1, F_SCREEN_ITEMS_2, F_NO_FUSED_SCREEN, F_SCREEN_WIDE, F_ONE_LAUNCH, run_device_batches, DeviceBatch,
+    NOT_BAD, CHIMERIC, NOT_COVERED, TYPE_NAMES, F_FORCE_GENERAL, F_FORCE_LDS_SORT, F_WAVE_ONLY, F_NO_HALVES, F_TIMING_FULL, F_NO_PREDICTION, F_NO_PREFILTER, F_COUNT_PREFILTERED, F_NO_TIMING, F_BLOCKING_WAIT, F_NO_DEFER, F_ALWAYS_DEFER, F_TIMING_SAMPLED, F_STREAM_SCREEN, F_SCREEN_ITEMS_1, F_SCREEN_ITEMS_2, F_NO_FUSED_SCREEN, F_SCREEN_WIDE, F_ONE_LAUNCH, F_SCREEN_DIRECT, F_NO_SCREEN_DIRECT, DEBUG_SYMBOLS, run_device_batches, DeviceBatch,
     EXPORTED_SYMBOLS, CLASS_NAMES, CLASS_KERNELS, PinnedArray, Stream, StreamGroup, stream_device_of, HANDLE_ELSEWHERE, RecSink, OvlRec, OVL_REC_DTYPE, GzipWriter, ByteSink,
 )
diff --git a/yacrd_amd/csrc/engine.hip b/yacrd_amd/csrc/engine.hip
--- a/yacrd_amd/csrc/engine.hip
+++ b/yacrd_amd/csrc/engine.hip
@@ -411,6 +411,16 @@
     const u32 plan_mode = (u32)((e->flags & YACRD_F_FORCE_GENERAL) ? 1
                                 : (e->flags & (YACRD_F_WAVE_ONLY | YACRD_F_FORCE_LDS_SORT)) ? 2
                                 : (e->flags & YACRD_F_NO_HALVES) ? 3 : 0);
+    if (R.direct) {
+        constexpr u32 per_wg = (u32)(yk::kPlanSidePer * yk::kPlanSideBlock);
+        if (R.full) HIP_TRY(hipEventRecord(e->ev[EV_PLAN0], e->side));
+        hipLaunchKernelGGL((yk::plan_kernel<yk::kPlanSidePer, yk::kPlanSideBlock>), dim3((n_reads + per_wg - 1) / per_wg), dim3(yk::kPlanSideBlock), 0, e->side,
+                           R.d_off, n_reads, R.lists, R.ctr, plan_mode | yk::kPlanDirect, e->ctrl2[other].as<u32>(), (u32)(R.other_bytes / 4),
+                           e->counts.as<u32>(), e->mrec.as<uint4>(), R.mrec_cap1, R.mrec_cap2);
+        e->ctrl_clean[other] = R.other_bytes;
+        if (R.full) HIP_TRY(hipEventRecord(e->ev[EV_PLAN], e->side));
+        return YACRD_OK;
+    }
     if (n_reads < yk::kPlanSmallReads)
         hipLaunchKernelGGL((yk::plan_kernel<1, yk::kPlanSmallBlock>), dim3((n_reads + yk::kPlanSmallBlock - 1) / yk::kPlanSmallBlock),
                            dim3(yk::kPlanSmallBlock), 0, e->stream, R.d_off, n_reads, R.lists, R.ctr, plan_mode, e->ctrl2[other].as<u32>(), (u32)(R.other_bytes / 4), e->counts.as<u32>(), e->mrec.as<uint4>(), R.mrec_cap1, R.mrec_cap2);
@@ -423,13 +433,49 @@
     return YACRD_OK;
 }
 
+bool prediction_holds(const yacrd_engine *e, const Run &R)
+{
+    const bool big_predictable = !(e->flags & YACRD_F_NO_PREFILTER) && e->pred.fb_big == 0;
+    return e->pred_valid && e->pred_reads == R.n_reads64 && e->pred_iv == R.n_iv &&
+           (e->pred.n[yk::CLS_GENERAL] == 0 || big_predictable) &&
+           !(e->flags & (YACRD_F_FORCE_GENERAL | YACRD_F_NO_PREDICTION));
+}
+
+bool choose_direct(yacrd_engine *e, const Run &R)
+{
+    const uint32_t f = e->flags;
+    if (f & YACRD_F_NO_SCREEN_DIRECT) return false;
+    if (f & (YACRD_F_FORCE_GENERAL | YACRD_F_WAVE_ONLY | YACRD_F_FORCE_LDS_SORT | YACRD_F_NO_HALVES | YACRD_F_NO_PREFILTER |
+             YACRD_F_COUNT_PREFILTERED | YACRD_F_NO_DEFER | YACRD_F_SCREEN_ITEMS_1 | YACRD_F_SCREEN_WIDE))
+        return false;
+    const bool forced = (f & YACRD_F_SCREEN_DIRECT) != 0;
+    if (!forced) {
+        if (!(f & YACRD_F_ALWAYS_DEFER) && e->nodefer_left != 0) return false;
+        if (!(f & YACRD_F_SCREEN_ITEMS_2) && e->wide_left != 0) return false;
+        if (R.n_reads64 < (uint64_t)yk::kPlanSmallReads) return false;
+        if (R.predicted) {
+            const yk::Counters &p = e->pred;
+            const u64 fused_iv = p.iv[yk::CLS_R16] + p.iv[yk::CLS_H16];
+            if (!(f & YACRD_F_SCREEN_ITEMS_2) && fused_iv < 40000000ull) return false;
+            if (!(f & YACRD_F_ALWAYS_DEFER) && fused_iv < defer_min_intervals()) return false;
+            if (8 * (u64)p.n[yk::CLS_H16] < 7 * R.n_reads64) return false;
+            if (p.n[yk::CLS_MED1] || p.n[yk::CLS_MED2] || p.n[yk::CLS_GENERAL]) return false;
+        } else {
+            if (!(f & YACRD_F_SCREEN_ITEMS_2) && R.n_iv < 40000000ull) return false;
+            if (!(f & YACRD_F_ALWAYS_DEFER) && R.n_iv < defer_min_intervals()) return false;
+            if (!(R.n_iv > 128 * R.n_reads64 && R.n_iv <= 256 * R.n_reads64)) return false;
+        }
+    }
+    if (e->side == nullptr) {
+        if (e->streams.add(1)) e->side = e->streams[1];
+        else (void)hipGetLastError();
+    }
+    return e->side != nullptr;
+}
+
 int size_launches(yacrd_engine *e, Run &R)
 {
     const uint64_t n_reads64 = R.n_reads64;
-    const bool big_predictable = !(e->flags & YACRD_F_NO_PREFILTER) && e->pred.fb_big == 0;
-    R.predicted = e->pred_valid && e->pred_reads == n_reads64 && e->pred_iv == R.n_iv &&
-                  (e->pred.n[yk::CLS_GENERAL] == 0 || big_predictable) &&
-                  !(e->flags & (YACRD_F_FORCE_GENERAL | YACRD_F_NO_PREDICTION));
     LaunchSet &ls = R.ls;
     if (R.predicted) {
         for (int cls = 0; cls < yk::CLS_GENERAL; cls++) {
@@ -442,8 +488,9 @@
         }
         R.big_n = e->pred.n[yk::CLS_GENERAL], R.big_iv = e->pred.iv[yk::CLS_GENERAL];
     } else {
-        HIP_TRY(hipMemcpyAsync(e->h_ctr(), R.ctr, sizeof(yk::Counters), hipMemcpyDeviceToHost, e->stream));
-        HIP_TRY(hipStreamSynchronize(e->stream));
+        const hipStream_t hs = R.direct ? e->side : e->stream;
+        HIP_TRY(hipMemcpyAsync(e->h_ctr(), R.ctr, sizeof(yk::Counters), hipMemcpyDeviceToHost, hs));
+        HIP_TRY(hipStreamSynchronize(hs));
         R.c0 = *e->h_ctr();
         for (int cls = 0; cls < yk::CLS_GENERAL; cls++) {
             ls.n[cls] = R.c0.n[cls];
@@ -452,53 +499,61 @@
         }
         R.big_n = R.c0.n[yk::CLS_GENERAL], R.big_iv = R.c0.iv[yk::CLS_GENERAL];
     }
+    if (R.direct) {
+        ls.n[yk::CLS_H16] = (u32)std::min<u64>((n_reads64 + 15) & ~(u64)15, 0xFFFFFFFFull);
+        ls.hint[yk::CLS_H16] = R.n_reads;
+    }
     for (int cls = 0; cls < yk::CLS_GENERAL; cls++)
         if (ls.n[cls] && (R.dom_cls < 0 || ls.iv[cls] > ls.iv[R.dom_cls])) R.dom_cls = cls;
     return YACRD_OK;
 }
 
-hipError_t before_class(yacrd_engine *e, Run &R, int cls)
+hipError_t before_class(yacrd_engine *e, Run &R, int cls, hipStream_t hs)
 {
     if (!R.timing_on || !(R.full || cls == R.dom_cls)) return hipSuccess;
-    if (R.n_cls_ev > 0 && R.full) {
+    if (R.n_cls_ev > 0 && R.full && R.cls_ev_stream == hs) {
         R.cls_b[cls] = R.n_cls_ev - 1;
         return hipSuccess;
     }
     R.cls_b[cls] = R.n_cls_ev;
-    return hipEventRecord(e->ev_cls[R.n_cls_ev++], e->stream);
-}
-hipError_t mark_class(yacrd_engine *e, Run &R, int cls)
+    R.cls_ev_stream = hs;
+    return hipEventRecord(e->ev_cls[R.n_cls_ev++], hs);
+}
+hipError_t mark_class(yacrd_engine *e, Run &R, int cls, hipStream_t hs)
 {
     if (!R.timing_on || !(R.full || cls == R.dom_cls)) return hipSuccess;
     R.cls_e[cls] = R.n_cls_ev;
-    return hipEventRecord(e->ev_cls[R.n_cls_ev++], e->stream);
+    R.cls_ev_stream = hs;
+    return hipEventRecord(e->ev_cls[R.n_cls_ev++], hs);
 }
 
 int launch_register_classes(yacrd_engine *e, Run &R, const LaunchSet &set, bool again)
 {
     yk::Counters *ctr = R.ctr;
     const bool fuse = !(e->flags & YACRD_F_FORCE_LDS_SORT);
+    const hipStream_t hs = (R.direct && !again) ? e->side : e->stream;
     if (fuse) {
         yk::FusedArgs fa;
         fa.base = R.base;
         const u64 fused_iv = set.iv[yk::CLS_R16] + set.iv[yk::CLS_H16];
-        const bool defer = R.prefilter && !(e->flags & YACRD_F_NO_DEFER) &&
-                           ((e->flags & YACRD_F_ALWAYS_DEFER) ||
-                            (fused_iv >= defer_min_intervals() && e->nodefer_left == 0));
-        const bool wide = defer && !(e->flags & YACRD_F_SCREEN_ITEMS_2) && ((e->flags & YACRD_F_SCREEN_WIDE) || e->wide_left > 0);
+        const bool defer = R.direct || (R.prefilter && !(e->flags & YACRD_F_NO_DEFER) &&
+                                        ((e->flags & YACRD_F_ALWAYS_DEFER) ||
+                                         (fused_iv >= defer_min_intervals() && e->nodefer_left == 0)));
+        const bool wide = defer && !R.direct && !(e->flags & YACRD_F_SCREEN_ITEMS_2) && ((e->flags & YACRD_F_SCREEN_WIDE) || e->wide_left > 0);
         const int items = !defer ? 1
                           : (wide || (e->flags & YACRD_F_SCREEN_ITEMS_1)) ? 1
-                          : ((e->flags & YACRD_F_SCREEN_ITEMS_2) || fused_iv >= 40000000ull) ? 2 : 1;
+                          : (R.direct || (e->flags & YACRD_F_SCREEN_ITEMS_2) || fused_iv >= 40000000ull) ? 2 : 1;
         e->last_items = (uint32_t)items;
         e->last_wide = wide;
         if (!again) e->last_build = !defer ? 0 : wide ? 3 : items;
         fa.base.over_list = nullptr;
         fa.base.over_count = nullptr;
         fa.n_entries = 0;
+        fa.direct = 0, fa.n_reads = R.n_reads;
         u32 blocks = 0;
         bool has_dom = false;
         for (int cls = yk::CLS_R2; cls <= yk::CLS_H16; cls++) {
-            if (!set.n[cls]) continue;
+            if (!set.n[cls] || (R.direct && cls == yk::CLS_H16)) continue;
             const u32 per = yk::sweep_group_reads_per_block(cls, defer ? yk::kDeferWaves : yk::kFusedWaves) *
                             (cls >= yk::CLS_R16 ? (u32)items : 1u);
             blocks += (set.n[cls] + per - 1) / per;
@@ -511,13 +566,13 @@
             has_dom |= cls == R.dom_cls;
         }
         if (fa.n_entries) {
-            const bool mark = R.timing_on && (R.full || has_dom);
+            const bool mark = R.timing_on && (R.full || has_dom) && !R.direct;
             void (*kernel)(yk::FusedArgs) = yk::sweep_small_fused_kernel;
             u32 threads = 64 * yk::kFusedWaves;
             if (defer && items == 2) kernel = yk::sweep_small_fused_defer2_kernel, threads = 64;
             else if (defer && wide) kernel = yk::sweep_small_fused_defer_wide_kernel, threads = 64 * yk::kDeferWaves;
             else if (defer) kernel = yk::sweep_small_fused_defer_kernel, threads = 64 * yk::kDeferWaves;
-            hipExtLaunchKernelGGL(kernel, dim3(blocks), dim3(threads), 0, e->stream, mark ? e->ev_cls[22] : (hipEvent_t) nullptr,
+            hipExtLaunchKernelGGL(kernel, dim3(blocks), dim3(threads), 0, hs, mark ? e->ev_cls[22] : (hipEvent_t) nullptr,
                                   mark ? e->ev_cls[23] : (hipEvent_t) nullptr, 0, fa);
             if (mark) R.fused_marked = true;
             if (defer && (set.n[yk::CLS_R16] || set.n[yk::CLS_H16])) R.screened = true;
@@ -525,24 +580,46 @@
     }
     for (int cls = fuse ? yk::CLS_W2 : yk::CLS_R2; cls <= yk::CLS_W16; cls++) {
         if (!set.n[cls]) continue;
-        HIP_TRY(before_class(e, R, cls));
+        HIP_TRY(before_class(e, R, cls, hs));
         yk::SweepArgs sa = list_sweep_args(R, R.list_of(cls), &ctr->n[cls]);
         sa.first = set.first[cls];
         if (!fuse) {
             const u32 grid = (u32)std::min<uint64_t>(set.n[cls], (uint64_t)e->num_cu * 32);
-            hipLaunchKernelGGL((yk::sweep_lds_kernel<64, (int)yk::kSmallEvents>), dim3(grid), dim3(64), 0, e->stream, sa);
+            hipLaunchKernelGGL((yk::sweep_lds_kernel<64, (int)yk::kSmallEvents>), dim3(grid), dim3(64), 0, hs, sa);
         } else {
             switch (cls) {
-            case yk::CLS_W2: yk::launch_sweep_group<64, 2>(sa, set.n[cls], e->stream); break;
-            case yk::CLS_W4: yk::launch_sweep_group<64, 4>(sa, set.n[cls], e->stream); break;
-            case yk::CLS_W8: yk::launch_sweep_group<64, 8>(sa, set.n[cls], e->stream); break;
-            default: yk::launch_sweep_group<64, 16>(sa, set.n[cls], e->stream); break;
+            case yk::CLS_W2: yk::launch_sweep_group<64, 2>(sa, set.n[cls], hs); break;
+            case yk::CLS_W4: yk::launch_sweep_group<64, 4>(sa, set.n[cls], hs); break;
+            case yk::CLS_W8: yk::launch_sweep_group<64, 8>(sa, set.n[cls], hs); break;
+            default: yk::launch_sweep_group<64, 16>(sa, set.n[cls], hs); break;
             }
         }
-        HIP_TRY(mark_class(e, R, cls));
-    }
-    if (R.full && R.timing_on) HIP_TRY(hipEventRecord(e->ev[EV_SMALL], e->stream));
-    return YACRD_OK;
+        HIP_TRY(mark_class(e, R, cls, hs));
+    }
+    if (R.full && R.timing_on && hs == e->stream) HIP_TRY(hipEventRecord(e->ev[EV_SMALL], e->stream));
+    return YACRD_OK;
+}
+
+void launch_direct_screen(yacrd_engine *e, Run &R)
+{
+    yk::FusedArgs fa;
+    fa.base = R.base;
+    fa.base.over_list = nullptr;
+    fa.base.over_count = nullptr;
+    fa.n_entries = 1;
+    fa.cls[0] = (u32)yk::CLS_H16;
+    fa.block_end[0] = R.n_reads / 4u + (R.n_reads % 4u ? 1u : 0u);
+    fa.first[0] = 0;
+    fa.list[0] = nullptr;
+    fa.list_n[0] = nullptr;
+    fa.direct = 1, fa.n_reads = R.n_reads;
+    const bool mark = R.timing_on;
+    hipExtLaunchKernelGGL(yk::sweep_small_fused_defer2_kernel, dim3(fa.block_end[0]), dim3(64), 0, e->stream, mark ? e->ev_cls[22] : (hipEvent_t) nullptr,
+                          mark ? e->ev_cls[23] : (hipEvent_t) nullptr, 0, fa);
+    if (mark) R.fused_marked = true;
+    R.screened = true;
+    e->last_items = 2, e->last_wide = false, e->last_build = 2;
+    e->direct_runs++;
 }
 
 int launch_workgroup_class_fused_screen(yacrd_engine *e, Run &R, const LaunchSet &set, int k, bool again)
@@ -626,11 +703,11 @@
     for (int k = 0; k < 2; k++) {
         const int cls = k == 0 ? yk::CLS_MED1 : yk::CLS_MED2;
         if (!set.n[cls]) continue;
-        HIP_TRY(before_class(e, R, cls));
+        HIP_TRY(before_class(e, R, cls, e->stream));
         const int rc = fused_screen ? launch_workgroup_class_fused_screen(e, R, set, k, again)
                                     : launch_workgroup_class_chain(e, R, set, k, again);
         if (rc) return rc;
-        HIP_TRY(mark_class(e, R, cls));
+        HIP_TRY(mark_class(e, R, cls, e->stream));
     }
     if (R.full && R.timing_on) HIP_TRY(hipEventRecord(e->ev[EV_MED], e->stream));
     return YACRD_OK;
@@ -689,7 +766,7 @@
 }
 int launch_device_wide_screen(yacrd_engine *e, Run &R)
 {
-    const bool can_fork = R.big_n != 0 && R.prefilter && !(e->flags & YACRD_F_FORCE_GENERAL);
+    const bool can_fork = R.big_n != 0 && R.prefilter && !(e->flags & YACRD_F_FORCE_GENERAL) && !R.direct;
     if (can_fork && e->side == nullptr) {
         if (e->streams.add(1)) e->side = e->streams[1];
         else (void)hipGetLastError();
@@ -853,11 +930,10 @@
         rc = launch_one_batch(e, R);
         return rc ? rc : hand_over(e, R, defer);
     }
-    rc = launch_plan(e, R);
-    if (!rc) rc = size_launches(e, R);
-    if (rc) return rc;
     R.timing_on = !(e->flags & YACRD_F_NO_TIMING);
     if ((e->flags & YACRD_F_TIMING_SAMPLED) && !R.full && (e->run_seq++ % 8u) != 0) R.timing_on = false;
+    R.predicted = prediction_holds(e, R);
+    R.direct = choose_direct(e, R);
     struct MissGuard {
         yacrd_engine *e;
         bool before;
@@ -869,17 +945,39 @@
         bool joined = false;
         ~SideGuard()
         {
-            if (R.big_beside && !joined) (void)hipStreamSynchronize(e->side);
+            if ((R.big_beside || R.direct) && !joined) (void)hipStreamSynchronize(e->side);
         }
     } side_guard{e, R};
     e->prev_build = e->last_build;
     e->last_build = -1;
-    if (R.full) HIP_TRY(hipEventRecord(e->ev[EV_S0], e->stream));
-    rc = launch_device_wide_screen(e, R);
-    if (!rc) rc = launch_sweeps(e, R, R.ls);
-    if (!rc) rc = join_device_wide_screen(e, R);
-    if (rc) return rc;
-    side_guard.joined = true;
+    if (R.direct) {
+        HIP_TRY(hipEventRecord(e->ev_sync[EVS_FORK], e->stream));
+        if (R.full) HIP_TRY(hipEventRecord(e->ev[EV_S0], e->stream));
+        launch_direct_screen(e, R);
+        HIP_TRY(hipStreamWaitEvent(e->side, e->ev_sync[EVS_FORK], 0));
+        rc = launch_plan(e, R);
+        if (!rc) rc = size_launches(e, R);
+        if (!rc) rc = launch_register_classes(e, R, R.ls, false);
+        if (rc) return rc;
+        HIP_TRY(hipEventRecord(e->ev_sync[EVS_JOIN], e->side));
+        HIP_TRY(hipStreamWaitEvent(e->stream, e->ev_sync[EVS_JOIN], 0));
+        side_guard.joined = true;
+        if (R.full && R.timing_on) HIP_TRY(hipEventRecord(e->ev[EV_SMALL], e->stream));
+        rc = launch_workgroup_classes(e, R, R.ls, false);
+        if (!rc) launch_rejected_medium(e, R, R.ls);
+        if (!rc) rc = join_device_wide_screen(e, R);
+        if (rc) return rc;
+    } else {
+        rc = launch_plan(e, R);
+        if (!rc) rc = size_launches(e, R);
+        if (rc) return rc;
+        if (R.full) HIP_TRY(hipEventRecord(e->ev[EV_S0], e->stream));
+        rc = launch_device_wide_screen(e, R);
+        if (!rc) rc = launch_sweeps(e, R, R.ls);
+        if (!rc) rc = join_device_wide_screen(e, R);
+        if (rc) return rc;
+        side_guard.joined = true;
+    }
     if (R.full) HIP_TRY(hipEventRecord(e->ev[EV_GEN], e->stream));
     rc = launch_compact(e, R);
     if (rc) return rc;
@@ -943,12 +1041,12 @@
     t.plan_ms = t.sweep_small_ms = t.sweep_medium_ms = t.sweep_general_ms = t.compact_ms = 0.f;
     t.total_ms = 0.f;
     if (full) {
-        t.plan_ms = ev_ms(e->ev[EV_START], e->ev[EV_PLAN]);
+        t.plan_ms = ev_ms(e->ev[R.direct ? EV_PLAN0 : EV_START], e->ev[EV_PLAN]);
         t.sweep_small_ms = ev_ms(e->ev[EV_S0], e->ev[EV_SMALL]);
         t.sweep_medium_ms = ev_ms(e->ev[EV_SMALL], e->ev[EV_MED]);
         t.sweep_general_ms = ev_ms(e->ev[EV_MED], e->ev[EV_GEN]);
         t.compact_ms = ev_ms(e->ev[EV_GEN], e->ev[EV_COMPACT]);
-        t.total_ms = (predicted ? ev_ms(e->ev[EV_START], e->ev[EV_COMPACT])
+        t.total_ms = ((predicted || R.direct) ? ev_ms(e->ev[EV_START], e->ev[EV_COMPACT])
                                 : t.plan_ms + ev_ms(e->ev[EV_S0], e->ev[EV_COMPACT])) + extra_ms;
     }
     t.n_small = 0;
@@ -1188,6 +1286,8 @@
     HIP_TRY(hipStreamSynchronize(e->stream));
     return YACRD_OK;
 }
+
+uint64_t yacrd_debug_direct_runs(const yacrd_engine *e) { return e ? e->direct_runs : 0; }
 
 void yacrd_debug_live_bytes(uint64_t out[2])
 {
diff --git a/yacrd_amd/csrc/engine_internal.h b/yacrd_amd/csrc/engine_internal.h
--- a/yacrd_amd/csrc/engine_internal.h
+++ b/yacrd_amd/csrc/engine_internal.h
@@ -153,7 +153,7 @@
     return e != hipSuccess ? e : hipErrorUnknown;
 }
 
-enum { EV_START = 0, EV_PLAN, EV_S0, EV_SMALL, EV_MED, EV_GEN, EV_COMPACT, EV_X0, EV_X1, EV_H2D0, EV_H2D1, EV_D2H0, EV_D2H1, EV_COUNT };
+enum { EV_START = 0, EV_PLAN, EV_S0, EV_SMALL, EV_MED, EV_GEN, EV_COMPACT, EV_X0, EV_X1, EV_H2D0, EV_H2D1, EV_D2H0, EV_D2H1, EV_PLAN0, EV_COUNT };
 enum { EVS_DONE = 0, EVS_FORK, EVS_JOIN, EVS_COUNT };
 
 struct DeviceGuard {
@@ -221,8 +221,10 @@
     u32 big_n = 0;
     u64 big_iv = 0;
     bool big_beside = false;
+    bool direct = false;
     int cls_b[12], cls_e[12];
     int n_cls_ev = 0, dom_cls = -1;
+    hipStream_t cls_ev_stream = nullptr;
     bool timing_on = false;
     bool fused_marked = false, screened = false, big_screened = false;
 };
@@ -275,6 +277,7 @@
     bool one_launch_off = false;
     int last_build = -1, prev_build = -1;
     bool miss_pending = false;
+    uint64_t direct_runs = 0;
     uint32_t nodefer_left = 0;
     static constexpr int kBounce = 12;
     static constexpr size_t kBounceBytes = (size_t)4 << 20;
diff --git a/yacrd_amd/csrc/plan_compact.h b/yacrd_amd/csrc/plan_compact.h
--- a/yacrd_amd/csrc/plan_compact.h
+++ b/yacrd_amd/csrc/plan_compact.h
@@ -10,12 +10,16 @@
 #endif
 constexpr int kPlanSmallBlock = YK_PLAN_SMALL_BLOCK;
 
+constexpr u32 kPlanDirect = 8u, kPlanModeMask = 7u;
+constexpr int kPlanSideBlock = 256, kPlanSidePer = 8;
 template <int PER, int BLK = kPlanBlock>
 __global__ __launch_bounds__(BLK) void plan_kernel(const u64 *off, u32 n_reads, u32 *lists,
-                                                   Counters *ctr, u32 mode, u32 *zero,
+                                                   Counters *ctr, u32 mode_bits, u32 *zero,
                                                    u32 zero_words, u32 *counts, uint4 *mrec, u32 mrec_cap1, u32 mrec_cap2)
 {
     constexpr int kPlanBlock = BLK;
+    const u32 mode = mode_bits & kPlanModeMask;
+    const bool direct = (mode_bits & kPlanDirect) != 0u;
     for (u32 i = blockIdx.x * kPlanBlock + threadIdx.x; i < zero_words; i += gridDim.x * kPlanBlock)
         zero[i] = 0;
     __shared__ u32 s_cnt[CLS_COUNT];
@@ -85,7 +89,7 @@
 #pragma unroll
     for (int k = 0; k < kPlanPer; k++) {
         const u32 r = blockIdx.x * (u32)kPlanReads + (u32)k * kPlanBlock + threadIdx.x;
-        if (cls[k] != CLS_COUNT) {
+        if (cls[k] != CLS_COUNT && !(direct && cls[k] == CLS_H16)) {
             const u64 pos = s_base[cls[k]] + local[k];
             lists[(u64)cls[k] * n_reads + pos] = r;
             counts[r] = kClosedForm;
diff --git a/yacrd_amd/csrc/screen_reg.h b/yacrd_amd/csrc/screen_reg.h
--- a/yacrd_amd/csrc/screen_reg.h
+++ b/yacrd_amd/csrc/screen_reg.h
@@ -132,10 +132,13 @@
 
 struct VerdictsToGlobal {
     const SweepArgs &a;
+    bool own_count = false;
     __device__ __forceinline__ void closed(u32 r, u32 ra, u32 rb, u32 len) const
     {
-        if (ra != 0 || rb != len) a.closed[r] = make_uint2(ra, rb);
-        else a.counts[r] = 0;
+        if (ra != 0 || rb != len) {
+            a.closed[r] = make_uint2(ra, rb);
+            if (own_count) a.counts[r] = kClosedForm;
+        } else a.counts[r] = 0;
         if (a.prefilter == 2) atomicAdd(&a.ctr->prefiltered, 1u);
     }
     __device__ __forceinline__ void deferred(u32 r) const { a.counts[r] = kDeferredMark; }
@@ -277,4 +280,41 @@
     screen_reads<LANES, ITEMS, WIDE, 1, K, NB, NT, TABW>(a, r, active, VerdictsToGlobal{a});
 }
 
-}
+constexpr u32 kH16MinIntervals = 129, kH16MaxIntervals = 256;
+__device__ __forceinline__ bool is_h16(u64 n) { return n >= (u64)kH16MinIntervals && n <= (u64)kH16MaxIntervals; }
+
+template <int TABW>
+__device__ __forceinline__ void screen_block_rows(const SweepArgs &a, u32 block, bool direct, u32 n_reads)
+{
+    const u32 grp = lane_id() / 16u;
+    u32 r[1] = {0u};
+    bool active[1] = {false};
+    ReadsKnown<1> k;
+    k.o[0] = 0, k.n[0] = 0, k.len[0] = 0;
+    if (direct) {
+        const u32 r0 = a.first + block * 4u;
+        if (r0 >= n_reads) return;
+        r[0] = r0 + grp;
+        if (r[0] < n_reads) {
+            const ulonglong2 oo = load_extent(a.off + r[0]);
+            k.len[0] = a.len[r[0]];
+            active[0] = is_h16(oo.y - oo.x);
+            k.o[0] = oo.x, k.n[0] = (u32)(oo.y - oo.x);
+        }
+        if (__builtin_amdgcn_ballot_w64(active[0]) == 0) return;
+    } else {
+        const u32 list_n = *a.list_n;
+        const u32 idx0 = a.first + block * 4u;
+        if (idx0 >= list_n) return;
+        active[0] = idx0 + grp < list_n;
+        if (active[0]) {
+            r[0] = a.list[idx0 + grp];
+            const ulonglong2 oo = load_extent(a.off + r[0]);
+            k.len[0] = a.len[r[0]];
+            k.o[0] = oo.x, k.n[0] = (u32)(oo.y - oo.x);
+        }
+    }
+    screen_reads<16, 1, false, 1, 32, 32, true, TABW>(a, r, active, VerdictsToGlobal{a, direct}, &k);
+}
+
+}
diff --git a/yacrd_amd/csrc/sweep_wave.h b/yacrd_amd/csrc/sweep_wave.h
--- a/yacrd_amd/csrc/sweep_wave.h
+++ b/yacrd_amd/csrc/sweep_wave.h
@@ -337,6 +337,8 @@
     u32 first[5];
     const u32 *list[5];
     const u32 *list_n[5];
+    u32 direct;
+    u32 n_reads;
 };
 
 template <bool DEFER, int WPB, int ITEMS = 1, bool WIDE = false>
@@ -368,7 +370,7 @@
         else sweep_group_block<16, 16, WPB>(a, b);
         break;
     default:
-        if constexpr (ROWS) screen_block<16, 1, false, 32, 32, true, TABW>(a, b);
+        if constexpr (ROWS) screen_block_rows<TABW>(a, b, f.direct != 0u, f.n_reads);
         else if constexpr (DEFER) screen_block<32, ITEMS, WIDE>(a, b);
         else sweep_group_block<32, 16, WPB>(a, b);
         break;
diff --git a/yacrd_amd/engine.py b/yacrd_amd/engine.py
--- a/yacrd_amd/engine.py
+++ b/yacrd_amd/engine.py
@@ -28,6 +28,12 @@
 F_SCREEN_ITEMS_2 = 524288
 F_NO_FUSED_SCREEN = 1048576
 F_SCREEN_WIDE = 2097152
+F_SCREEN_DIRECT = 8388608
+F_NO_SCREEN_DIRECT = 16777216
+DEBUG_SYMBOLS = [
+    "yacrd_debug_sort_pairs", "yacrd_debug_last_counters", "yacrd_debug_last_input_csr", "yacrd_debug_peer_copy_counts",
+    "yacrd_debug_live_bytes", "yacrd_debug_direct_runs",
+]
 F_ONE_LAUNCH = 4194304
 
 EXPORTED_SYMBOLS = [
@@ -671,6 +677,11 @@
             out[n] = list(v) if hasattr(v, "__len__") else int(v)
         return out
 
+    def direct_runs(self):
+        self._lib.yacrd_debug_direct_runs.restype = ctypes.c_uint64
+        self._lib.yacrd_debug_direct_runs.argtypes = [ctypes.c_void_p]
+        return int(self._lib.yacrd_debug_direct_runs(self._h))
+
     def _type_table(self, names, read_type):
         blobs = [n if isinstance(n, bytes) else n.encode("utf-8", "surrogateescape") for n in names]
         off = np.zeros(len(blobs) + 1, np.uint64)
```

Measured after the change: 3.406 billion (median of 6 runs). 9.0% higher.
